# kngwyu/rogue-gym

Hardware: AMD Instinct MI355X
Metric: env-steps/sec (whole node) at 65 536 envs, 32x16 mini-dungeon (higher is better)
Workload: dtype u8/u16 integer state, f32 observation; 1 GPU; config-mini.json 32x16, 65536 envs per GPU (65536 total), gray-image obs [N,1,16,32] f32, max_steps 1000, auto-reset; envs_per_gpu=65536, parallelism=env-sharded x1, no data-path collective

## Files before the change

### include/rogue_gym_hip.h

```cpp
#ifndef ROGUE_GYM_HIP_H
#define ROGUE_GYM_HIP_H
#include <stddef.h>
#include <stdint.h>

#ifdef __cplusplus
extern "C" {
#endif

typedef struct rg_handle rg_t;

#define RG_FLAG_TERMINAL   0x00000001u
#define RG_FLAG_DEAD       0x00000002u
#define RG_FLAG_REDRAW     0x00000004u
#define RG_FLAG_HIST_STALE 0x00000008u
#define RG_FLAG_HIST_LAG   0x00000010u
#define RG_FLAG_HIST_DIRTY 0x00000020u
#define RG_FLAG_SCR_CHANGED 0x00000040u
#define RG_FLAG_MSG_SHIFT  8
#define RG_FLAG_MSG_MASK   0x00007f00u
#define RG_FLAG_ERR_KEY    0x00010000u
#define RG_FLAG_ERR_DEAD   0x00020000u
#define RG_FLAG_ERR_TILE   0x00040000u
#define RG_FLAG_ERR_INTERNAL 0x00080000u
#define RG_FLAG_ERR_STATE  0x00100000u
#define RG_FLAG_ERR_MASK   0x00ff0000u

int rg_create(const char *const *cfg_json, int n_env, uint64_t max_steps, int device, int auto_reset, rg_t **out);
void rg_destroy(rg_t *h);
const char *rg_last_error(const rg_t *h);

const char *rg_build_id(void);

int rg_dims(const rg_t *h, int *height, int *width, int *symbols, int *n_env);
int rg_env_dims(const rg_t *h, int32_t *heights, int32_t *widths);
int rg_env_symbols(const rg_t *h, int32_t *out_host);
int rg_set_stream(rg_t *h, void *hip_stream);

int rg_seed(rg_t *h, const uint64_t *seed_lo, const uint64_t *seed_hi, int n);
int rg_reset(rg_t *h);
int rg_reset_envs(rg_t *h, const int32_t *env_ids, int k, int ids_on_device);
int rg_reset_mask(rg_t *h, const uint8_t *mask_dev);
int rg_seed_envs(rg_t *h, const int32_t *env_ids, const uint64_t *seed_lo, const uint64_t *seed_hi, int k);
int rg_step(rg_t *h, const uint8_t *keys, int keys_on_device);
int rg_step_prefix(rg_t *h, const uint8_t *keys, int n_keys, int keys_on_device);
int rg_step_obs_gray(rg_t *h, const uint8_t *keys, int keys_on_device, uint32_t status_flag, int with_hist, float *out_dev);
int rg_obs_bind(rg_t *h, int kind, uint32_t status_flag, int with_hist, float *out_dev);
int rg_sync(rg_t *h);

int rg_screen(rg_t *h, uint8_t **dev);
int rg_hist(rg_t *h, uint8_t **dev);
int rg_status(rg_t *h, int32_t **dev);
int rg_flags(rg_t *h, uint32_t **dev);
int rg_reward(rg_t *h, float **dev);
int rg_done(rg_t *h, uint8_t **dev);

int rg_set_stair_reward(rg_t *h, float bonus);

int rg_obs_gray(rg_t *h, uint32_t status_flag, int with_hist, float *out_dev);
int rg_obs_symbol(rg_t *h, uint32_t status_flag, int with_hist, float *out_dev);
int rg_obs_channels(const rg_t *h, int symbol, uint32_t status_flag, int with_hist);

int rg_obs_crop(rg_t *h, int kind, int radius_y, int radius_x, uint32_t status_flag, int with_hist, float *out_dev, int32_t *centers_dev);

#define RG_OBS_F32  0
#define RG_OBS_F16  1
#define RG_OBS_BF16 2
#define RG_OBS_U8   3
int rg_obs_dtype_bytes(int dtype);
int rg_obs_typed(rg_t *h, int kind, int dtype, uint32_t status_flag, int with_hist, void *out_dev);
int rg_step_obs_typed(rg_t *h, const uint8_t *keys, int keys_on_device, int kind, int dtype, uint32_t status_flag, int with_hist, void *out_dev);

int rg_status_vec(rg_t *h, uint32_t status_flag, int32_t *out_host);

int rg_fetch_states(rg_t *h, uint8_t *screen, uint8_t *hist, int32_t *status, uint32_t *flags);
int rg_step_fetch(rg_t *h, const uint8_t *keys_host, int n_keys, uint8_t *screen, uint8_t *hist, int32_t *status, uint32_t *flags);

int rg_dev_alloc(int device, size_t bytes, void **out);
void rg_dev_free(int device, void *p);
int rg_snapshot_take(rg_t *h, void *dev);
int rg_dev_read(rg_t *h, const void *dev_src, void *host_dst, size_t bytes);
int rg_dev_read_rows(rg_t *h, const void *dev_src, size_t src_pitch, void *host_dst, size_t row_bytes, int rows);

int rg_encode_host(int device, const uint8_t *screen, const uint8_t *hist, const int32_t *status, int height, int width,
                   int symbols, uint32_t status_flag, int with_hist, int kind, float *out_host);

int rg_encode_host_batch(int device, int n, const uint8_t *screen, const uint8_t *hist, const int32_t *status, int height, int width,
                         int symbols, uint32_t status_flag, int with_hist, int kind, float *out_host);
int rg_obs_host(rg_t *h, int kind, uint32_t status_flag, int with_hist, float *out_host);
int rg_host_alloc(size_t bytes, void **out);
void rg_host_free(void *p);

#define RG_COMPACT_FIXED_BYTES 48
#define RG_COMPACT_STATUS_OFFSET(hw) (hw)
#define RG_COMPACT_REWARD_OFFSET(hw) ((hw) + 40)
#define RG_COMPACT_FLAGS_OFFSET(hw) ((hw) + 44)
#define RG_COMPACT_HIST_OFFSET(hw) ((hw) + RG_COMPACT_FIXED_BYTES)
int rg_compact_record_bytes(const rg_t *h, int with_hist);
int rg_pack_compact(rg_t *h, int with_hist, uint8_t *out_dev);
int rg_comm_unique_id(uint8_t id[128]);
int rg_comm_init(rg_t *h, const uint8_t id[128], int rank, int world);
int rg_comm_destroy(rg_t *h);
int rg_comm_count(rg_t *h, int *count, int *rank);
int rg_allgather_compact(rg_t *h, int with_hist, uint8_t *out_dev);
int rg_expand_compact(rg_t *h, const uint8_t *packed_dev, int n, int packed_has_hist, int kind, uint32_t status_flag, int with_hist, float *out_dev);

int rg_history_enable(rg_t *h, int cap_per_env);
int rg_history_keys(rg_t *h, int env, int which, uint8_t *keys, size_t cap, uint32_t *len);
int rg_dump_history(rg_t *h, int env, int which, char *buf, size_t cap, size_t *needed);

int rg_counters(rg_t *h, uint64_t out[8], int reset);
int rg_counters_ex(rg_t *h, uint64_t *out, int n_out, int reset);
int rg_probe_sclk(rg_t *h, double *mhz);

int rg_timing_enable(rg_t *h, int on);
int rg_timing_read(rg_t *h, double ms[4], uint64_t launches[4]);
int rg_timing_read_all(rg_t *h, int n, double *ms, uint64_t *sampled, uint64_t *launches);
int rg_timing_read_samples(rg_t *h, int kernel, float *ms, int cap, int *n);

int rg_dump_config(const rg_t *h, int env, char *buf, size_t cap);

int rg_config_canonical(const char *cfg_json, char *buf, size_t cap);

int rg_config_resolved(const char *cfg_json, char *buf, size_t cap);

int rg_config_schema(char *buf, size_t cap, size_t *needed);

int rg_state_record_bytes(const rg_t *h);
int rg_state_save(rg_t *h, const int32_t *env_ids, int k, int ids_on_device, uint8_t *out_dev);
int rg_state_load(rg_t *h, const uint8_t *rec_dev, size_t rec_bytes, const int32_t *env_ids, int k, int ids_on_device);

typedef struct rg_debug_state {
    int32_t px, py, dungeon_level, hp, hp_max, player_level, n_monsters, n_gold;
    uint32_t exp, food_left, quiet, pack_gold, steps;
    uint32_t rng[12];
    int32_t mon_x[384], mon_y[384], mon_type[384], mon_active[384], mon_hp[384];
    uint32_t mon_exp[384];
    int32_t gold_x[384], gold_y[384], gold_amount[384];
    int32_t n_rooms;
    uint32_t room_rect[384];
    int32_t room_meta[384];
} rg_debug_state;
int rg_debug_fetch(rg_t *h, int env, rg_debug_state *out, uint16_t *cells);
int rg_debug_descend(rg_t *h);

#ifdef __cplusplus
}
#endif
#endif
```

### rogue-gym_amd/csrc/rg_api.cpp

```cpp
#include <hip/hip_runtime.h>
#include <dlfcn.h>

#include <cstdio>
#include <cstdlib>
#include <cstring>
#include <mutex>
#include <random>
#include <string>
#include <vector>

#include "../../include/rogue_gym_hip.h"
#include "rg_state.h"
#include "rg_state_io.h"

extern "C" {
typedef struct ncclComm *ncclComm_t;
typedef struct { char internal[128]; } ncclUniqueId;
typedef int ncclResult_t;
typedef int ncclDataType_t;
}
static const ncclResult_t ncclSuccess = 0;
static const ncclDataType_t ncclUint8 = 1;

extern "C" {
void rgk_build(const RgState *S, const RgConfig *c, hipStream_t st);
int rgk_step(const RgState *S, const RgState *SP_dev, const RgConfig *c, const uint8_t *keys, int use_spares, int parity, hipStream_t st, hipEvent_t ev0, hipEvent_t ev1);
void rgk_probe_clock(unsigned long long *out, int spin, hipStream_t st);
void rgk_regen(const RgState *SP, const RgConfig *c, int bulk, int spares, const uint32_t *mark, uint32_t target, uint32_t *err_any, hipStream_t st, hipEvent_t ev0, hipEvent_t ev1);
void rgk_regen_gate(const uint32_t *mark, uint32_t target, uint32_t *err_any, hipStream_t st);
void rgk_export(const RgState *S, uint32_t *err_any, void *o_screen, void *o_hist, void *o_status, void *o_flags, uint32_t *o_err, hipStream_t st);
int rgk_regen_lanes_supported(const RgConfig *c, int maze_cap);
int rgk_step_bound_capable(const RgConfig *c);
int rgk_regen_lanes(const RgState *SP, const RgConfig *c, uint32_t *q, int32_t *list, int bulk, int waves, int slots, hipStream_t st, hipEvent_t ev0, hipEvent_t ev1);
void rgk_debug_descend(const RgState *S, const RgConfig *c, hipStream_t st);
void rgk_render(const RgState *S, const RgConfig *c, hipStream_t st);
void rgk_encode(const uint8_t *screen, const uint8_t *hist, const int32_t *status, uint32_t *flags, uint32_t *err_any, int n, int hw, size_t rs, size_t rst,
                int symbols, int planes_sym, uint32_t sflag, int with_hist, int kind, float *out, const int32_t *ext, hipStream_t st);
void rgk_pack(const RgState *S, int with_hist, uint8_t *out, hipStream_t st);
void rgk_scatter_rows(const void *src, void *dst, const int32_t *ext, int n, int row_bytes, hipStream_t st);
void rgk_gather_keys(const uint8_t *keys, const int32_t *ext, uint8_t *dst, int n, hipStream_t st);
int rgk_obs(const RgState *S, const RgConfig *c, uint32_t sflag, int with_hist, int kind, float *out, uint32_t *err_any, int planes_sym, int bound, hipStream_t st, hipEvent_t ev0, hipEvent_t ev1);
int rgk_redraw(const RgState *S, const RgConfig *c, hipStream_t st);
int rgk_obs_typed(const RgState *S, const RgConfig *c, int kind, int dtype, uint32_t sflag, int with_hist, int planes_sym, void *out, uint32_t *err_any, hipStream_t st, hipEvent_t ev0,
                  hipEvent_t ev1);
int rgk_obs_crop(const RgState *S, const RgConfig *c, int kind, int ry, int rx, uint32_t sflag, int with_hist, int planes_sym, float *out, int32_t *centers,
                 uint32_t *err_any, hipStream_t st);
void rgk_state_save(const RgState *S, const RgIoLayout *L, const uint64_t *desc, const uint32_t *guard, const int32_t *ids, int k, uint8_t *out, hipStream_t st);
void rgk_state_load(const RgState *S, const RgIoLayout *L, const uint64_t *desc, const uint32_t *guard, const int32_t *ids, int k, const uint8_t *recs, uint32_t rec_bytes, uint8_t *ok,
                    uint8_t *mark, hipStream_t st);
void rgk_state_stairs(const RgState *S, const RgIoLayout *L, uint8_t *mark, hipStream_t st);
void rgk_reset_compact(const uint8_t *mask, int n, int32_t *list, uint32_t *cnt, hipStream_t st);
void rgk_build_list(const RgState *S, const RgConfig *c, const int32_t *list, const uint32_t *cnt, uint8_t *mark, hipStream_t st);
}

#define RG_TIMED_KERNELS 5
struct rg_handle {
    RgParsed parsed;
    RgConfig cfg;
    RgState S;
    RgState SP;
    bool spares = false;
    uint32_t *lane_q = nullptr; int32_t *lane_list = nullptr;
    hipStream_t side3 = nullptr;
    hipStream_t side2 = nullptr;
    int lane_flip = 0;
    uint64_t lane_last = 0;
    uint8_t *pin_keys = nullptr;
    uint32_t *pin_err = nullptr;
    bool lane_regen = false;
    uint64_t step_count = 0;
    hipStream_t side = nullptr;
    int regen_idle_after = -1;
    int regen_bulk = 0;
    int device = 0;
    hipStream_t stream = nullptr;
    std::vector<void *> allocs;
    uint32_t *d_err = nullptr;
    uint8_t *d_keys = nullptr;
    bool render_pending = false;
    float *bound_out = nullptr; int bound_kind = 0; bool bound_valid = false;
    int32_t *obs_list_mem = nullptr; uint32_t *obs_cnt_mem = nullptr; float *gray_lut_mem = nullptr;
    int bound_steps = 0;
    int stair_gen = 0;
    float *obs_scratch = nullptr;
    size_t obs_scratch_cap = 0;
    std::vector<uint64_t> seed_lo, seed_hi;
    std::vector<uint8_t> reseed;
    std::vector<uint64_t> range_lo, range_span;
    unsigned long long *d_probe = nullptr;
    std::vector<rg_handle *> sub;
    std::vector<int> g_of, l_of;
    int32_t *d_ext = nullptr;
    std::vector<int32_t> ext;
    uint8_t *d_keys_sub = nullptr;
    int planes_sym = 0;
    bool screens_stale = true;
    bool mixed = false;
    std::vector<size_t> ragged_off;
    size_t stat_rows = 0;
    RgState *d_SP = nullptr;
    ncclComm_t comm = nullptr;
    int comm_rank = 0, comm_world = 1;
    std::string err;
    bool timing = false;
    std::vector<hipEvent_t> ev[RG_TIMED_KERNELS];
    size_t ev_used[RG_TIMED_KERNELS] = {0, 0, 0, 0, 0};
    uint64_t timing_seq[RG_TIMED_KERNELS] = {0, 0, 0, 0, 0};
    uint64_t timing_stride = 1;
    uint64_t state_fp = 0;
    uint64_t *io_desc = nullptr;
    uint32_t *io_guard = nullptr;
    uint32_t io_words = 0;
    int32_t *io_ids = nullptr; size_t io_ids_cap = 0;
    uint8_t *io_ok = nullptr; size_t io_ok_cap = 0;
    uint8_t *io_mark = nullptr;
    int32_t *reset_list = nullptr;
    uint32_t *reset_cnt = nullptr;
};

#define RG_TIMING_MAX 4096
struct TimedLaunch {
    rg_handle *h; int k; bool on, ext_;
    TimedLaunch(rg_handle *h_, int k_, bool ext = false) : h(h_), k(k_), on(false), ext_(ext) {
        if (h->timing && (h->timing_seq[k]++ % h->timing_stride) == h->timing_stride / 2 && h->ev_used[k] + 2 <= h->ev[k].size()) {
            on = true;
            if (!ext_) (void)hipEventRecord(h->ev[k][h->ev_used[k]], h->stream);
        }
    }
    hipEvent_t start_ev() const { return on && ext_ ? h->ev[k][h->ev_used[k]] : nullptr; }
    hipEvent_t stop_ev() const { return on && ext_ ? h->ev[k][h->ev_used[k] + 1] : nullptr; }
    void cancel() { on = false; }
    void stop() { if (on) { if (!ext_) (void)hipEventRecord(h->ev[k][h->ev_used[k] + 1], h->stream); h->ev_used[k] += 2; on = false; } }
    ~TimedLaunch() { stop(); }
};

static thread_local std::string g_create_err;

#ifdef RG_DEV_KNOBS
#define RG_DEV_ENV(name) getenv(name)
#else
#define RG_DEV_ENV(name) ((const char *)nullptr)
#endif

#define HIPCHK(h, call)                                                                                  \
    do {                                                                                                 \
        hipError_t e_ = (call);                                                                          \
        if (e_ != hipSuccess) {                                                                          \
            (h)->err = std::string(#call) + ": " + hipGetErrorString(e_);                                \
            return 1;                                                                                    \
        }                                                                                                \
    } while (0)

template <typename T>
static bool dev_alloc(rg_handle *h, T **p, size_t count) {
    void *q = nullptr;
    size_t bytes = count * sizeof(T);
    if (bytes == 0) bytes = 16;
    if (hipMalloc(&q, bytes) != hipSuccess) { h->err = "hipMalloc failed (" + std::to_string(bytes) + " bytes)"; return false; }
    if (hipMemset(q, 0, bytes) != hipSuccess) { h->err = "hipMemset failed"; return false; }
    h->allocs.push_back(q);
    *p = (T *)q;
    return true;
}

static void free_all(rg_handle *h) {
    for (void *p : h->allocs) (void)hipFree(p);
    h->allocs.clear();
}

static int flush_render(rg_handle *h) {
    if (h->render_pending) {
        { TimedLaunch t(h, 1); rgk_render(&h->S, &h->cfg, h->stream); }
        HIPCHK(h, hipGetLastError());
        h->render_pending = false;
        h->bound_valid = false;
    }
    return 0;
}

static int upload_seeds(rg_handle *h, size_t n) {
    HIPCHK(h, hipMemcpyAsync(h->S.seed_lo, h->seed_lo.data(), n * 8, hipMemcpyHostToDevice, h->stream));
    HIPCHK(h, hipMemcpyAsync(h->S.seed_hi, h->seed_hi.data(), n * 8, hipMemcpyHostToDevice, h->stream));
    HIPCHK(h, hipMemcpyAsync(h->S.reseed, h->reseed.data(), n, hipMemcpyHostToDevice, h->stream));
    return 0;
}

extern "C" {

const char *rg_last_error(const rg_t *h) { return h ? h->err.c_str() : g_create_err.c_str(); }

#ifndef RG_BUILD_ID
#define RG_BUILD_ID "unstamped"
#endif
const char *rg_build_id(void) { static const char id[] = "RGBUILDID:" RG_BUILD_ID; return id + 10; }

static void destroy_handle(rg_handle *h);
struct EnvSeed { bool has_seed, has_range; uint64_t lo, hi; unsigned __int128 r0, r1; };

static int create_homog(const RgParsed &parsed, const EnvSeed *seeds, int n_env, uint64_t max_steps, int device, int auto_reset, rg_handle **out) {
    *out = nullptr;
    rg_handle *h = new rg_handle();
    std::random_device rd;
    std::mt19937_64 gen(((uint64_t)rd() << 32) ^ rd());
    h->seed_lo.resize(n_env); h->seed_hi.resize(n_env); h->reseed.resize(n_env);
    h->parsed = parsed;
    for (int i = 0; i < n_env; i++) {
        const EnvSeed &p = seeds[i];
        if (p.has_seed) { h->seed_lo[i] = p.lo; h->seed_hi[i] = p.hi; h->reseed[i] = 0; }
        else { h->seed_lo[i] = gen(); h->seed_hi[i] = gen(); h->reseed[i] = 1; }
        if (p.has_range) {
            if (!(p.r1 > p.r0)) {
                if (!p.has_seed) { g_create_err = "Invalid Setting: seed_range must satisfy start < end"; delete h; return 1; }
                continue;
            }
            if (h->range_lo.empty()) { h->range_lo.assign(2 * (size_t)n_env, 0); h->range_span.assign(2 * (size_t)n_env, 0); }
            const unsigned __int128 span = p.r1 - p.r0;
            h->range_lo[i] = (uint64_t)p.r0; h->range_lo[n_env + i] = (uint64_t)(p.r0 >> 64);
            h->range_span[i] = (uint64_t)span; h->range_span[n_env + i] = (uint64_t)(span >> 64);
            if (!p.has_seed) h->reseed[i] = 2;
        }
    }
    h->cfg = h->parsed.cfg;
    {
        RgParsed q = h->parsed;
        q.has_seed_range = false;
        const std::string js = rg_dump_config_json(q, 0, 0, false);
        uint64_t f = 0xcbf29ce484222325ull;
        for (unsigned char ch : js) { f ^= ch; f *= 0x100000001b3ull; }
        h->state_fp = f;
    }
    h->planes_sym = h->cfg.symbols;
    h->cfg.max_steps = max_steps > 0xfffffff0ull ? 0xfffffff0u : (uint32_t)max_steps;
    h->cfg.auto_reset = auto_reset ? 1 : 0;
    h->device = device;
    int ndev = 0;
    if (hipGetDeviceCount(&ndev) != hipSuccess || ndev <= 0) {
        g_create_err = "no HIP device available (librogue_gym_hip has no CPU fallback)"; delete h; return 1;
    }
    if (device < 0 || device >= ndev || hipSetDevice(device) != hipSuccess) { g_create_err = "invalid HIP device " + std::to_string(device); delete h; return 1; }

    RgState &S = h->S;
    memset(&S, 0, sizeof S);
    const size_t n = (size_t)n_env, hw = (size_t)h->cfg.width * h->cfg.height;
    S.n = n_env; S.hw = (int)hw; S.n_keys = n_env;
    const int maze_cap = ((h->cfg.width / h->cfg.room_num_x + 1) / 2) * ((h->cfg.height / h->cfg.room_num_y + 1) / 2) + 1;
    S.maze_cap = maze_cap;
    const size_t nr = (size_t)h->cfg.room_num_x * h->cfg.room_num_y, ne = 2 * nr;
    h->stat_rows = 2048 + (n + 15) / 16;
    bool ok = dev_alloc(h, &S.cell, n * hw) && dev_alloc(h, &S.screen, n * hw) && dev_alloc(h, &S.hist, n * hw) &&
              dev_alloc(h, &S.p_pos, n) && dev_alloc(h, &S.p_hp, n) && dev_alloc(h, &S.p_hpmax, n) && dev_alloc(h, &S.p_lvl, n) &&
              dev_alloc(h, &S.p_exp, n) && dev_alloc(h, &S.food, n) && dev_alloc(h, &S.quiet, n) && dev_alloc(h, &S.pack_gold, n) &&
              dev_alloc(h, &S.dlevel, n) && dev_alloc(h, &S.steps, n) && dev_alloc(h, &S.flags, n) && dev_alloc(h, &S.reward, n) && dev_alloc(h, &S.done, n) &&
              dev_alloc(h, &S.rng, 12 * n) && dev_alloc(h, &S.seed_lo, n) && dev_alloc(h, &S.seed_hi, n) && dev_alloc(h, &S.reseed, n) &&
              dev_alloc(h, &S.room_rect, nr * n) && dev_alloc(h, &S.room_meta, nr * n) &&
              dev_alloc(h, &S.mon_w0, nr * n) && dev_alloc(h, &S.mon_hp, nr * n) && dev_alloc(h, &S.mon_exp, nr * n) &&
              dev_alloc(h, &S.mon_cnt, n) && dev_alloc(h, &S.gold_pos, nr * n) && dev_alloc(h, &S.gold_amt, nr * n) &&
              dev_alloc(h, &S.edge_a, ne * n) && dev_alloc(h, &S.edge_b, ne * n) &&
              dev_alloc(h, &S.maze_stack, (size_t)maze_cap * n) && dev_alloc(h, &S.build_ctr, n) && dev_alloc(h, &S.stats, RG_STAT_COLS * h->stat_rows) && dev_alloc(h, &S.stair_list, 2 * n) && dev_alloc(h, &S.stair_cnt, 8) && dev_alloc(h, &S.stair_mark, 2 * n) &&
              dev_alloc(h, &S.dc_map, h->cfg.n_enemies > 0 ? n * RG_DIST_SLOTS * hw : 16) && dev_alloc(h, &S.dc_key, RG_DIST_SLOTS * n) &&
              dev_alloc(h, &S.dc_head, n) && dev_alloc(h, &S.dc_len, n) && dev_alloc(h, &S.dc_part, n) && dev_alloc(h, &S.dc_own, n) && dev_alloc(h, &S.status, n * 10) &&
              dev_alloc(h, &h->d_err, 4) && dev_alloc(h, &h->d_keys, n);
    if (ok && nr <= RG_OBS_MAX_ROOMS) ok = dev_alloc(h, &S.obs_rec, n * (size_t)RG_OBS_REC_WORDS(nr));
    if (ok && nr <= RG_OVL_MAX && getenv("ROGUE_GYM_HIP_NO_MIRROR_UPDATE") == nullptr)
        ok = dev_alloc(h, &S.ovl, (nr + 1) * n) && hipMemset(S.ovl, 0xff, (nr + 1) * n * 2) == hipSuccess;
    h->spares = auto_reset != 0 && getenv("ROGUE_GYM_HIP_NO_SPARES") == nullptr;
    h->lane_regen = h->spares && getenv("ROGUE_GYM_HIP_WAVE_REGEN") == nullptr && rgk_regen_lanes_supported(&h->cfg, maze_cap) > 0;
    const char *slots_env = getenv("ROGUE_GYM_HIP_SP_SLOTS");
    S.sp_slots = h->lane_regen ? (slots_env ? atoi(slots_env) : 4) : 1;
    if (S.sp_slots < 1 || S.sp_slots > 8) S.sp_slots = 4;
    const size_t ns = n * (size_t)S.sp_slots;
    ok = ok && dev_alloc(h, &S.sp_ready, ns) && dev_alloc(h, &h->d_probe, 4) && dev_alloc(h, &S.launch_mark, 4);
    if (ok && h->cfg.n_enemies > 0 && RG_PARTIAL_MAPS(h->cfg.width, h->cfg.height, (int)nr))
        ok = dev_alloc(h, &S.dc_walk, n * RG_DIST_SLOTS * h->cfg.height * RG_WALK_WORDS(h->cfg.width));
    S.full_bfs = getenv("ROGUE_GYM_HIP_FULL_BFS") != nullptr;
    S.keep_spares = getenv("ROGUE_GYM_HIP_KEEP_SPARES") != nullptr;
    S.err_any = h->d_err;
    if (ok && !h->range_lo.empty()) {
        ok = dev_alloc(h, &S.range_lo, 2 * n) && dev_alloc(h, &S.range_span, 2 * n) &&
             hipMemcpy(S.range_lo, h->range_lo.data(), 2 * n * 8, hipMemcpyHostToDevice) == hipSuccess &&
             hipMemcpy(S.range_span, h->range_span.data(), 2 * n * 8, hipMemcpyHostToDevice) == hipSuccess;
        if (!ok && h->err.empty()) h->err = "hipMemcpy failed";
    }
    if (ok && !h->parsed.init_draws.empty()) {
        uint32_t *d = nullptr;
        ok = dev_alloc(h, &d, h->parsed.init_draws.size()) &&
             hipMemcpy(d, h->parsed.init_draws.data(), h->parsed.init_draws.size() * 4, hipMemcpyHostToDevice) == hipSuccess;
        if (!ok && h->err.empty()) h->err = "hipMemcpy failed";
        S.init_draws = d;
    }
    if (ok && h->spares && nr <= 64 && getenv("ROGUE_GYM_HIP_NO_NEXT_LEVELS") == nullptr) {
        RgNext nx;
        memset(&nx, 0, sizeof nx);
        RgNext *d_nx = nullptr;
        ok = dev_alloc(h, &nx.cell, n * hw) && dev_alloc(h, &nx.room_rect, nr * n) && dev_alloc(h, &nx.room_meta, nr * n) &&
             dev_alloc(h, &nx.gold_pos, nr * n) && dev_alloc(h, &nx.gold_amt, nr * n) && dev_alloc(h, &nx.level, n) &&
             dev_alloc(h, &S.nx_rng, 12 * n) && dev_alloc(h, &S.nx_state, n) && dev_alloc(h, &d_nx, 1);
        ok = ok && hipMemcpy(d_nx, &nx, sizeof nx, hipMemcpyHostToDevice) == hipSuccess;
        S.nx = d_nx;
    }
    h->SP = S;
    if (ok && h->spares) {
        RgState &P = h->SP;
        ok = dev_alloc(h, &P.cell, ns * hw) && dev_alloc(h, &P.p_pos, ns) && dev_alloc(h, &P.p_hp, ns) && dev_alloc(h, &P.p_hpmax, ns) && dev_alloc(h, &P.p_lvl, ns) &&
             dev_alloc(h, &P.p_exp, ns) && dev_alloc(h, &P.food, ns) && dev_alloc(h, &P.quiet, ns) && dev_alloc(h, &P.pack_gold, ns) && dev_alloc(h, &P.dlevel, ns) &&
             dev_alloc(h, &P.rng, 12 * ns) && dev_alloc(h, &P.room_rect, nr * ns) && dev_alloc(h, &P.room_meta, nr * ns) &&
             dev_alloc(h, &P.mon_w0, nr * ns) && dev_alloc(h, &P.mon_hp, nr * ns) && dev_alloc(h, &P.mon_exp, nr * ns) &&
             dev_alloc(h, &P.mon_cnt, ns) && dev_alloc(h, &P.gold_pos, nr * ns) && dev_alloc(h, &P.gold_amt, nr * ns) &&
             dev_alloc(h, &P.edge_a, ne * n) && dev_alloc(h, &P.edge_b, ne * n) && dev_alloc(h, &P.maze_stack, (size_t)maze_cap * n) &&
             dev_alloc(h, &P.on_stairs, ns);
        P.prof = nullptr;
        int lo = 0, hi = 0;
        if (ok && (hipDeviceGetStreamPriorityRange(&lo, &hi) != hipSuccess || hipStreamCreateWithPriority(&h->side, hipStreamNonBlocking, RG_DEV_ENV("ROGUE_GYM_HIP_SIDE_HIPRIO") ? hi : lo) != hipSuccess)) {
            h->err = "failed to create the background generation stream"; ok = false;
        }
        static const bool lanes_low = RG_DEV_ENV("ROGUE_GYM_HIP_LANES_LOWPRIO") != nullptr;
        if (ok && (hipStreamCreateWithPriority(&h->side2, hipStreamNonBlocking, lanes_low ? lo : (lo + hi) / 2) != hipSuccess || hipStreamCreateWithPriority(&h->side3, hipStreamNonBlocking, lanes_low ? lo : (lo + hi) / 2) != hipSuccess)) { h->err = "failed to create the background generation stream"; ok = false; }
    }
    ok = ok && dev_alloc(h, &h->d_SP, 1) && hipMemcpy(h->d_SP, &h->SP, sizeof(RgState), hipMemcpyHostToDevice) == hipSuccess;
    if (!ok) { g_create_err = h->err.empty() ? "device allocation failed" : h->err; destroy_handle(h); return 1; }
    if (hipMemset(S.screen, ' ', n * hw) != hipSuccess) { g_create_err = "hipMemset failed"; destroy_handle(h); return 1; }
    if (upload_seeds(h, n)) { g_create_err = h->err; destroy_handle(h); return 1; }
    h->S.stair_gen = h->stair_gen++;
    rgk_build(&h->S, &h->cfg, h->stream);
    hipError_t e = hipGetLastError();
    if (e == hipSuccess) e = hipStreamSynchronize(h->stream);
    if (e != hipSuccess) { g_create_err = std::string("k_build: ") + hipGetErrorString(e); destroy_handle(h); return 1; }
    h->render_pending = true;
    if (h->spares) {
        if (h->lane_regen && !(dev_alloc(h, &h->lane_q, 8) && dev_alloc(h, &h->lane_list, 2 * ns))) { g_create_err = h->err; destroy_handle(h); return 1; }
        if (h->lane_regen) (void)rgk_regen_lanes(&h->SP, &h->cfg, h->lane_q, h->lane_list, 1, 0, h->S.sp_slots, h->side2, nullptr, nullptr);
        else rgk_regen(&h->SP, &h->cfg, 1, 1, nullptr, 0, h->d_err, h->side, nullptr, nullptr);
        e = hipGetLastError();
        if (e == hipSuccess && !RG_DEV_ENV("ROGUE_GYM_HIP_ASYNC_FIRST_SPARES")) { e = hipStreamSynchronize(h->side); if (e == hipSuccess) e = hipStreamSynchronize(h->side2); if (e == hipSuccess) e = hipStreamSynchronize(h->side3); }
        if (e != hipSuccess) { g_create_err = std::string("k_regen: ") + hipGetErrorString(e); destroy_handle(h); return 1; }
        h->regen_bulk = 1;
        bool all_fixed = true;
        for (uint8_t m : h->reseed) all_fixed = all_fixed && m == 0;
        if (h->S.keep_spares && all_fixed && !h->S.nx_state) h->regen_idle_after = 1;
    }
    *out = h;
    return 0;
}

#define SUBCHK(h, sh, call) do { if (call) { (h)->err = (sh)->err; return 1; } } while (0)

static void destroy_handle(rg_handle *h);
static int comm_release(rg_handle *h, bool teardown);

static int assemble_small(rg_handle *h) {
    for (rg_handle *sh : h->sub) {
        const int m = sh->S.n;
        rgk_scatter_rows(sh->S.status, h->S.status, sh->d_ext, m, 40, h->stream);
        rgk_scatter_rows(sh->S.reward, h->S.reward, sh->d_ext, m, 4, h->stream);
        rgk_scatter_rows(sh->S.done, h->S.done, sh->d_ext, m, 1, h->stream);
        rgk_scatter_rows(sh->S.flags, h->S.flags, sh->d_ext, m, 4, h->stream);
    }
    HIPCHK(h, hipGetLastError());
    return 0;
}
static int assemble_screens(rg_handle *h) {
    if (!h->screens_stale) return 0;
    for (rg_handle *sh : h->sub) {
        SUBCHK(h, sh, flush_render(sh));
        const int m = sh->S.n;
        if (!h->mixed) {
            rgk_scatter_rows(sh->S.screen, h->S.screen, sh->d_ext, m, h->S.hw, h->stream);
            rgk_scatter_rows(sh->S.hist, h->S.hist, sh->d_ext, m, h->S.hw, h->stream);
        }
        rgk_scatter_rows(sh->S.flags, h->S.flags, sh->d_ext, m, 4, h->stream);
    }
    HIPCHK(h, hipGetLastError());
    h->screens_stale = false;
    return 0;
}

int rg_create(const char *const *cfg_json, int n_env, uint64_t max_steps, int device, int auto_reset, rg_t **out) {
    if (!out || n_env <= 0) { g_create_err = "rg_create: invalid arguments"; return 1; }
    *out = nullptr;
    std::vector<RgParsed> reps;
    std::vector<EnvSeed> seeds(n_env);
    std::vector<int> g_of(n_env), l_of(n_env);
    std::vector<std::vector<int>> members;
    {
        const char *prev = nullptr; int prev_g = -1;
        RgParsed p;
        for (int i = 0; i < n_env; i++) {
            const char *js = cfg_json ? cfg_json[i] : nullptr;
            const bool same_text = i > 0 && ((js == nullptr && prev == nullptr) || (js && prev && strcmp(js, prev) == 0));
            int g = prev_g;
            if (!same_text) {
                std::string e = rg_parse_config(js, &p);
                if (!e.empty()) { g_create_err = "Failed to parse config: " + e; return 1; }
                g = -1;
                for (size_t k = 0; k < reps.size(); k++) if (rg_config_equal(reps[k], p)) { g = (int)k; break; }
                if (g < 0) { g = (int)reps.size(); reps.push_back(p); members.emplace_back(); }
                prev = js; prev_g = g;
            }
            seeds[i] = EnvSeed{p.has_seed, p.has_seed_range, p.seed_lo, p.seed_hi, p.seed_range[0], p.seed_range[1]};
            g_of[i] = g; l_of[i] = (int)members[g].size(); members[g].push_back(i);
        }
    }
    if (reps.size() == 1) return create_homog(reps[0], seeds.data(), n_env, max_steps, device, auto_reset, out);
    bool mixed = false;
    for (size_t k = 1; k < reps.size(); k++) mixed = mixed || reps[k].cfg.width != reps[0].cfg.width || reps[k].cfg.height != reps[0].cfg.height;
    rg_handle *h = new rg_handle();
    h->device = device;
    h->mixed = mixed;
    h->g_of = g_of; h->l_of = l_of;
    for (size_t k = 0; k < reps.size(); k++) {
        std::vector<EnvSeed> gs(members[k].size());
        for (size_t j = 0; j < members[k].size(); j++) gs[j] = seeds[members[k][j]];
        rg_handle *sh = nullptr;
        if (create_homog(reps[k], gs.data(), (int)gs.size(), max_steps, device, auto_reset, &sh)) { destroy_handle(h); return 1; }
        h->sub.push_back(sh);
        sh->ext.assign(members[k].begin(), members[k].end());
        bool ok = dev_alloc(sh, &sh->d_ext, gs.size()) && dev_alloc(sh, &sh->d_keys_sub, gs.size()) &&
                  hipMemcpy(sh->d_ext, sh->ext.data(), gs.size() * 4, hipMemcpyHostToDevice) == hipSuccess;
        if (!ok) { g_create_err = "device allocation failed"; destroy_handle(h); return 1; }
        sh->S.ext = sh->d_ext;
    }
    if (mixed) {
        h->ragged_off.assign((size_t)n_env + 1, 0);
        for (int i = 0; i < n_env; i++) h->ragged_off[i + 1] = h->ragged_off[i] + (size_t)reps[g_of[i]].cfg.width * reps[g_of[i]].cfg.height;
    }
    rg_handle *first = h->sub[g_of[0]];
    h->parsed = first->parsed; h->cfg = first->cfg;
    h->planes_sym = first->cfg.symbols;
    for (rg_handle *sh : h->sub) sh->planes_sym = h->planes_sym;
    RgState &S = h->S;
    memset(&S, 0, sizeof S);
    const size_t n = (size_t)n_env, hw = (size_t)h->cfg.width * h->cfg.height;
    S.n = n_env; S.hw = (int)hw; S.n_keys = n_env;
    bool ok = (mixed || (dev_alloc(h, &S.screen, n * hw) && dev_alloc(h, &S.hist, n * hw))) && dev_alloc(h, &S.status, n * 10) && dev_alloc(h, &S.flags, n) &&
              dev_alloc(h, &S.reward, n) && dev_alloc(h, &S.done, n) && dev_alloc(h, &h->d_err, 4) && dev_alloc(h, &h->d_probe, 4);
    if (!ok) { g_create_err = h->err; destroy_handle(h); return 1; }
    S.err_any = h->d_err;
    if (assemble_small(h) || hipStreamSynchronize(h->stream) != hipSuccess) { g_create_err = h->err.empty() ? "assemble failed" : h->err; destroy_handle(h); return 1; }
    *out = h;
    return 0;
}

static void destroy_handle(rg_handle *h) {
    if (!h) return;
    (void)hipSetDevice(h->device);
    for (rg_handle *sh : h->sub) destroy_handle(sh);
    h->sub.clear();
    (void)hipStreamSynchronize(h->stream);
    if (h->comm) (void)comm_release(h, true);
    if (h->side) { (void)hipStreamSynchronize(h->side); (void)hipStreamDestroy(h->side); }
    if (h->side2) { (void)hipStreamSynchronize(h->side2); (void)hipStreamDestroy(h->side2); }
    if (h->side3) { (void)hipStreamSynchronize(h->side3); (void)hipStreamDestroy(h->side3); }
    for (int k = 0; k < RG_TIMED_KERNELS; k++) for (auto &e : h->ev[k]) (void)hipEventDestroy(e);
    if (h->obs_scratch) (void)hipFree(h->obs_scratch);
    if (h->pin_keys) (void)hipHostFree(h->pin_keys);
    if (h->pin_err) (void)hipHostFree(h->pin_err);
    free_all(h);
    delete h;
}

void rg_destroy(rg_t *h) { destroy_handle(h); }

int rg_dims(const rg_t *h, int *height, int *width, int *symbols, int *n_env) {
    if (height) *height = h->cfg.height;
    if (width) *width = h->cfg.width;
    if (symbols) *symbols = h->planes_sym;
    if (n_env) *n_env = h->S.n;
    return 0;
}

int rg_env_dims(const rg_t *h, int32_t *heights, int32_t *widths) {
    for (int i = 0; i < h->S.n; i++) {
        const RgConfig &c = h->sub.empty() ? h->cfg : h->sub[h->g_of[i]]->cfg;
        if (heights) heights[i] = c.height;
        if (widths) widths[i] = c.width;
    }
    return 0;
}
static bool refuse_mixed(rg_handle *h, const char *what) {
    if (!h->mixed) return false;
    h->err = std::string(what) + ": the envs of this batch differ in width / height, so there is no [n_env][H][W] tensor (per-env sizes: rg_env_dims; "
             "ragged host copies: rg_fetch_states; or one handle per size)";
    return true;
}

int rg_env_symbols(const rg_t *h, int32_t *out_host) {
    if (h->sub.empty()) { for (int i = 0; i < h->S.n; i++) out_host[i] = h->cfg.symbols; return 0; }
    for (int i = 0; i < h->S.n; i++) out_host[i] = h->sub[h->g_of[i]]->cfg.symbols;
    return 0;
}

int rg_set_stream(rg_t *h, void *hip_stream) {
    for (rg_handle *sh : h->sub) SUBCHK(h, sh, rg_set_stream(sh, hip_stream));
    HIPCHK(h, hipStreamSynchronize(h->stream));
    if (h->side) { HIPCHK(h, hipStreamSynchronize(h->side)); HIPCHK(h, hipStreamSynchronize(h->side2)); HIPCHK(h, hipStreamSynchronize(h->side3)); }
    h->stream = (hipStream_t)hip_stream;
    return 0;
}

int rg_seed(rg_t *h, const uint64_t *seed_lo, const uint64_t *seed_hi, int n) {
    if (n > h->S.n) n = h->S.n;
    if (n <= 0) return 0;
    HIPCHK(h, hipSetDevice(h->device));
    if (!h->sub.empty()) {
        for (rg_handle *sh : h->sub) {
            std::vector<uint64_t> lo, hi;
            for (int l = 0; l < sh->S.n && sh->ext[l] < n; l++) { lo.push_back(seed_lo[sh->ext[l]]); hi.push_back(seed_hi ? seed_hi[sh->ext[l]] : 0); }
            if (!lo.empty()) SUBCHK(h, sh, rg_seed(sh, lo.data(), hi.data(), (int)lo.size()));
        }
        return 0;
    }
    for (int i = 0; i < n; i++) { h->seed_lo[i] = seed_lo[i]; h->seed_hi[i] = seed_hi ? seed_hi[i] : 0; h->reseed[i] = 0; }
    if (h->spares) {
        HIPCHK(h, hipStreamSynchronize(h->side));
        HIPCHK(h, hipStreamSynchronize(h->side2));
        HIPCHK(h, hipStreamSynchronize(h->side3));
        for (int sl = 0; sl < h->S.sp_slots; sl++) HIPCHK(h, hipMemsetAsync(h->S.sp_ready + (size_t)sl * h->S.n, 0, (size_t)n * 4, h->stream));
        if (h->regen_idle_after >= 0) h->regen_idle_after = 2;
        h->regen_bulk = 2;
    }
    return upload_seeds(h, (size_t)n);
}

int rg_reset(rg_t *h) {
    HIPCHK(h, hipSetDevice(h->device));
    if (!h->sub.empty()) {
        for (rg_handle *sh : h->sub) SUBCHK(h, sh, rg_reset(sh));
        h->screens_stale = true;
        return assemble_small(h);
    }
    h->S.stair_gen = h->stair_gen++;
    { TimedLaunch t(h, 3); rgk_build(&h->S, &h->cfg, h->stream); }
    HIPCHK(h, hipGetLastError());
    h->render_pending = true;
    h->bound_valid = false;
    return 0;
}

static int obs_common(rg_t *h, uint32_t status_flag, int with_hist, int kind, float *out_dev);
int rg_step(rg_t *h, const uint8_t *keys, int keys_on_device) { return rg_step_prefix(h, keys, h->S.n, keys_on_device); }
int rg_step_obs_gray(rg_t *h, const uint8_t *keys, int keys_on_device, uint32_t status_flag, int with_hist, float *out_dev) {
    return rg_step_prefix(h, keys, h->S.n, keys_on_device) ? 1 : obs_common(h, status_flag, with_hist, 0, out_dev);
}

int rg_step_prefix(rg_t *h, const uint8_t *keys, int n_keys, int keys_on_device) {
    HIPCHK(h, hipSetDevice(h->device));
    if (n_keys < 0) { h->err = "rg_step_prefix: negative key count"; return 1; }
    if (n_keys > h->S.n) n_keys = h->S.n;
    if (!h->sub.empty()) {
        const uint8_t *dkeys = keys;
        if (!keys_on_device) {
            if (!h->d_keys && !dev_alloc(h, &h->d_keys, (size_t)h->S.n)) return 1;
            HIPCHK(h, hipMemcpyAsync(h->d_keys, keys, (size_t)n_keys, hipMemcpyHostToDevice, h->stream));
            dkeys = h->d_keys;
        }
        for (rg_handle *sh : h->sub) {
            int m = 0;
            while (m < sh->S.n && sh->ext[m] < n_keys) m++;
            if (m) rgk_gather_keys(dkeys, sh->d_ext, sh->d_keys_sub, m, h->stream);
            SUBCHK(h, sh, rg_step_prefix(sh, sh->d_keys_sub, m, 1));
        }
        HIPCHK(h, hipGetLastError());
        h->screens_stale = true;
        return assemble_small(h);
    }
    if (flush_render(h)) return 1;
    const uint8_t *dk = keys;
    if (!keys_on_device) {
        HIPCHK(h, hipMemcpyAsync(h->d_keys, keys, (size_t)n_keys, hipMemcpyHostToDevice, h->stream));
        dk = h->d_keys;
    }
    h->S.n_keys = n_keys;
    static const int regen_every = RG_DEV_ENV("ROGUE_GYM_HIP_REGEN_EVERY") ? atoi(RG_DEV_ENV("ROGUE_GYM_HIP_REGEN_EVERY")) : 1;
    h->step_count++;
    bool regen = h->spares && (regen_every <= 1 || h->step_count % (uint64_t)regen_every == 0);
    if (regen && h->regen_idle_after >= 0) { if (h->regen_idle_after == 0) regen = false; else h->regen_idle_after--; }
    static const bool no_stair_waves = getenv("ROGUE_GYM_HIP_NO_STAIR_WAVES") != nullptr;
    {
        TimedLaunch t(h, 0, true);
        h->S.stair_gen = h->stair_gen++;
        h->S.obs_par = (int32_t)(h->step_count & 1); h->bound_steps++;
        (void)rgk_step(&h->S, h->d_SP, &h->cfg, dk, h->spares ? 1 : 0, no_stair_waves ? -1 : 0, h->stream, t.start_ev(), t.stop_ev());
    }
    HIPCHK(h, hipGetLastError());
    if (regen) {
        TimedLaunch t(h, 4, true);
        if (h->lane_regen) {
            static const int lane_waves = RG_DEV_ENV("ROGUE_GYM_HIP_LANE_WAVES") ? atoi(RG_DEV_ENV("ROGUE_GYM_HIP_LANE_WAVES")) : 256;
            static const int lane_every = RG_DEV_ENV("ROGUE_GYM_HIP_LANE_EVERY") ? atoi(RG_DEV_ENV("ROGUE_GYM_HIP_LANE_EVERY")) : 16;
            static const bool time_lanes = RG_DEV_ENV("ROGUE_GYM_HIP_TIME_LANES") != nullptr;
            const bool lanes_now = h->regen_bulk > 0 || h->step_count - h->lane_last >= (uint64_t)(lane_every > 0 ? lane_every : 1);
            static const int urgent_mode = RG_DEV_ENV("ROGUE_GYM_HIP_URGENT_AT0") ? 3 : 2;
            rgk_regen(&h->SP, &h->cfg, 0, urgent_mode, h->S.launch_mark, (uint32_t)h->S.stair_gen + 1u, h->d_err, h->side, time_lanes ? nullptr : t.start_ev(), time_lanes ? nullptr : t.stop_ev());
            if (time_lanes && !lanes_now) t.cancel();
            if (lanes_now) {
                h->lane_last = h->step_count;
                h->lane_flip ^= 1;
                rgk_regen_gate(h->S.launch_mark, (uint32_t)h->S.stair_gen + 1u, h->d_err, h->lane_flip ? h->side3 : h->side2);
                (void)rgk_regen_lanes(&h->SP, &h->cfg, h->lane_q + 4 * h->lane_flip, h->lane_list + (size_t)h->S.n * h->S.sp_slots * h->lane_flip, h->regen_bulk > 0 ? 1 : 0, lane_waves, h->S.sp_slots,
                                      h->lane_flip ? h->side3 : h->side2, time_lanes ? t.start_ev() : nullptr, time_lanes ? t.stop_ev() : nullptr);
            }
        } else rgk_regen(&h->SP, &h->cfg, h->regen_bulk > 0 ? 1 : 0, 1, h->S.launch_mark, (uint32_t)h->S.stair_gen + 1u, h->d_err, h->side, t.start_ev(), t.stop_ev());
        if (h->regen_bulk > 0) h->regen_bulk--;
    }
    HIPCHK(h, hipGetLastError());
    h->render_pending = true;
    return 0;
}

int rg_sync(rg_t *h) {
    HIPCHK(h, hipSetDevice(h->device));
    if (!h->sub.empty()) {
        int rc = 0;
        for (rg_handle *sh : h->sub)
            if (rg_sync(sh) && !rc) { rc = 1; h->err = sh->err; }
        if (rc) return rc;
    }
    uint32_t err = 0;
    HIPCHK(h, hipMemcpyAsync(&err, h->d_err, 4, hipMemcpyDeviceToHost, h->stream));
    HIPCHK(h, hipStreamSynchronize(h->stream));
    if (h->side) { HIPCHK(h, hipStreamSynchronize(h->side)); HIPCHK(h, hipStreamSynchronize(h->side2)); HIPCHK(h, hipStreamSynchronize(h->side3)); }
    if (err) {
        HIPCHK(h, hipMemsetAsync(h->d_err, 0, 4, h->stream));
        if (err & RG_FLAG_ERR_INTERNAL) h->err = "internal capacity guard of the HIP stepper tripped (please report the config), or rg_reset_envs was given a device-side env id out of range";
        else if (err & RG_FLAG_ERR_STATE) h->err = "state record refused: it does not fit this env (magic / version / config fingerprint / geometry), the env is unchanged";
        else if (err & RG_FLAG_ERR_KEY) h->err = "Invalid input (key is not in the ai keymap)";
        else if (err & RG_FLAG_ERR_DEAD) h->err = "Ignored input (action while the player is dead)";
        else h->err = "Invalid tile in symbol image (symbol >= symbols - 1)";
        return 1;
    }
    return 0;
}

static int flush_mirrors(rg_handle *h) { return h->sub.empty() ? flush_render(h) : assemble_screens(h); }
int rg_screen(rg_t *h, uint8_t **dev) { if (refuse_mixed(h, "rg_screen")) return 1; HIPCHK(h, hipSetDevice(h->device)); if (flush_mirrors(h)) return 1; *dev = h->S.screen; return 0; }
int rg_hist(rg_t *h, uint8_t **dev) { if (refuse_mixed(h, "rg_hist")) return 1; HIPCHK(h, hipSetDevice(h->device)); if (flush_mirrors(h)) return 1; *dev = h->S.hist; return 0; }
int rg_status(rg_t *h, int32_t **dev) { *dev = h->S.status; return 0; }
int rg_flags(rg_t *h, uint32_t **dev) { HIPCHK(h, hipSetDevice(h->device)); if (flush_mirrors(h)) return 1; *dev = h->S.flags; return 0; }
int rg_reward(rg_t *h, float **dev) { *dev = h->S.reward; return 0; }
int rg_done(rg_t *h, uint8_t **dev) { *dev = h->S.done; return 0; }
int rg_set_stair_reward(rg_t *h, float bonus) {
    if (!(bonus == bonus) || bonus < 0.f) { h->err = "rg_set_stair_reward: the bonus must be a number >= 0"; return 1; }
    h->S.stair_reward = bonus;
    for (rg_handle *sh : h->sub) sh->S.stair_reward = bonus;
    return 0;
}

int rg_obs_channels(const rg_t *h, int symbol, uint32_t status_flag, int with_hist) {
    return (symbol ? h->planes_sym : 1) + __builtin_popcount(status_flag & 0x1ffu) + (with_hist ? 1 : 0);
}

static int obs_common(rg_t *h, uint32_t status_flag, int with_hist, int kind, float *out_dev) {
    if (refuse_mixed(h, kind ? "rg_obs_symbol" : "rg_obs_gray")) return 1;
    HIPCHK(h, hipSetDevice(h->device));
    if (!h->sub.empty()) {
        for (rg_handle *sh : h->sub) {
            if (kind && sh->cfg.symbols > h->planes_sym) {
                h->err = "symbol image: a config of the batch has more symbols (" + std::to_string(sh->cfg.symbols) + ") than env 0's (" + std::to_string(h->planes_sym) +
                         "), which sets the channel count (python/src/lib.rs:281-285)";
                return 1;
            }
            SUBCHK(h, sh, obs_common(sh, status_flag, with_hist, kind, out_dev));
        }
        return 0;
    }
    {
        TimedLaunch t(h, 2, true);
        const bool bound = h->bound_out && out_dev == h->bound_out && kind == h->bound_kind && (status_flag & 0x1ffu) == 0 && !with_hist;
        if (rgk_obs(&h->S, &h->cfg, status_flag & 0x1ffu, with_hist ? 1 : 0, kind, out_dev, h->d_err, h->planes_sym, bound && h->S.obs_list && h->bound_valid && h->bound_steps == 1, h->stream, t.start_ev(), t.stop_ev())) {
            HIPCHK(h, hipGetLastError());
            h->render_pending = false;
            h->bound_valid = bound;
            h->bound_steps = 0;
            return 0;
        }
        t.cancel();
    }
    h->bound_valid = false;
    if (flush_render(h)) return 1;
    {
        TimedLaunch t(h, 2);
        rgk_encode(h->S.screen, h->S.hist, h->S.status, h->S.flags, h->d_err, h->S.n, h->S.hw, (size_t)h->S.hw, 10, h->cfg.symbols, h->planes_sym,
                   status_flag & 0x1ffu, with_hist ? 1 : 0, kind, out_dev, h->S.ext, h->stream);
    }
    HIPCHK(h, hipGetLastError());
    return 0;
}
static uint32_t host_tile_to_sym(uint32_t t) {
    switch (t) {
    case ' ': return 0; case '@': return 1; case '#': return 2; case '.': return 3; case '-': case '|': return 4;
    case '%': return 5; case '+': return 6; case '^': return 7; case '!': return 8; case '?': return 9; case ']': return 10;
    case ')': return 11; case '/': return 12; case '*': return 13; case ':': return 14; case '=': return 15; case ',': return 16;
    default: return (t >= 'A' && t <= 'Z') ? t - 'A' + 17 : 255u;
    }
}
int rg_obs_bind(rg_t *h, int kind, uint32_t status_flag, int with_hist, float *out_dev) {
    if (!h->sub.empty()) { h->err = "rg_obs_bind: not for a handle with config groups"; return 1; }
    if (out_dev && ((status_flag & 0x1ffu) || with_hist || (kind != 0 && kind != 1))) { h->err = "rg_obs_bind: gray or symbol image without status planes and history plane"; return 1; }
    HIPCHK(h, hipSetDevice(h->device));
    const bool capable = rgk_step_bound_capable(&h->cfg) != 0;
    if (!capable) { h->S.obs_list = nullptr; h->S.obs_cnt = nullptr; h->S.bound_gray = nullptr; h->bound_out = out_dev; h->bound_kind = kind; h->bound_valid = false; h->bound_steps = 0; return 0; }
    if (out_dev && !h->obs_list_mem) {
        if (!dev_alloc(h, &h->obs_list_mem, 2 * (size_t)h->S.n) || !dev_alloc(h, &h->obs_cnt_mem, 2)) return 1;
    }
    if (out_dev) HIPCHK(h, hipMemsetAsync(h->obs_cnt_mem, 0, 8, h->stream));
    h->S.obs_list = out_dev ? h->obs_list_mem : nullptr; h->S.obs_cnt = out_dev ? h->obs_cnt_mem : nullptr;
    h->S.bound_gray = (out_dev && kind == 0) ? out_dev : nullptr;
    if (h->S.bound_gray && !h->gray_lut_mem) {
        float lut[128];
        for (uint32_t g = 0; g < 128; g++) lut[g] = (float)(uint8_t)host_tile_to_sym(g) / (float)(uint8_t)h->cfg.symbols;
        if (!dev_alloc(h, &h->gray_lut_mem, 128)) return 1;
        HIPCHK(h, hipMemcpy(h->gray_lut_mem, lut, sizeof lut, hipMemcpyHostToDevice));
    }
    h->S.gray_lut = h->gray_lut_mem;
    h->bound_out = out_dev; h->bound_kind = kind; h->bound_valid = false; h->bound_steps = 0;
    return 0;
}
int rg_obs_crop(rg_t *h, int kind, int radius_y, int radius_x, uint32_t status_flag, int with_hist, float *out_dev, int32_t *centers_dev) {
    if (kind != 0 && kind != 1) { h->err = "rg_obs_crop: kind must be 0 (gray) or 1 (symbol), got " + std::to_string(kind); return 1; }
    if (radius_y < 0 || radius_y > RG_MAX_H - 1 || radius_x < 0 || radius_x > RG_MAX_W - 1) {
        h->err = "rg_obs_crop: radii must satisfy 0 <= radius_y <= " + std::to_string(RG_MAX_H - 1) + " and 0 <= radius_x <= " + std::to_string(RG_MAX_W - 1) +
                 ", got (" + std::to_string(radius_y) + ", " + std::to_string(radius_x) + ")";
        return 1;
    }
    if (!out_dev || ((uintptr_t)out_dev & 15)) { h->err = "rg_obs_crop: out_dev must be a non-null, 16-byte aligned device pointer"; return 1; }
    HIPCHK(h, hipSetDevice(h->device));
    if (!h->sub.empty()) {
        for (rg_handle *sh : h->sub)
            if (kind && sh->cfg.symbols > h->planes_sym) {
                h->err = "symbol image: a config of the batch has more symbols (" + std::to_string(sh->cfg.symbols) + ") than env 0's (" + std::to_string(h->planes_sym) +
                         "), which sets the channel count (python/src/lib.rs:281-285)";
                return 1;
            }
        for (rg_handle *sh : h->sub) SUBCHK(h, sh, rg_obs_crop(sh, kind, radius_y, radius_x, status_flag, with_hist, out_dev, centers_dev));
        return 0;
    }
    if (flush_render(h)) return 1;
    if (!rgk_obs_crop(&h->S, &h->cfg, kind, radius_y, radius_x, status_flag & 0x1ffu, with_hist ? 1 : 0, h->planes_sym, out_dev, centers_dev, h->d_err, h->stream)) {
        h->err = "rg_obs_crop: window too large";
        return 1;
    }
    HIPCHK(h, hipGetLastError());
    return 0;
}
int rg_obs_dtype_bytes(int dtype) { return dtype == RG_OBS_F32 ? 4 : (dtype == RG_OBS_F16 || dtype == RG_OBS_BF16) ? 2 : dtype == RG_OBS_U8 ? 1 : -1; }
static int typed_check(rg_t *h, const char *what, int kind, int dtype, uint32_t status_flag, const void *out_dev) {
    const std::string w = std::string(what) + ": ";
    if (kind < 0 || kind > 2) { h->err = w + "kind must be 0 (gray), 1 (symbol) or 2 (symbol ids), got " + std::to_string(kind); return 1; }
    if (rg_obs_dtype_bytes(dtype) < 0) { h->err = w + "dtype must be RG_OBS_F32 (0), RG_OBS_F16 (1), RG_OBS_BF16 (2) or RG_OBS_U8 (3), got " + std::to_string(dtype); return 1; }
    if (kind == 2 && dtype != RG_OBS_U8) { h->err = w + "kind 2 (symbol ids) takes dtype RG_OBS_U8 only, got dtype " + std::to_string(dtype); return 1; }
    if (kind != 2 && dtype == RG_OBS_U8) { h->err = w + "dtype RG_OBS_U8 is for kind 2 (symbol ids) only, got kind " + std::to_string(kind); return 1; }
    if (kind == 2 && (status_flag & 0x1ffu)) { h->err = w + "status_flag must be 0 for kind 2 (status values do not fit a byte; read the status mirror)"; return 1; }
    if (!out_dev || ((uintptr_t)out_dev & 15)) { h->err = w + "out_dev must be a non-null, 16-byte aligned device pointer"; return 1; }
    if (dtype == RG_OBS_F32) return 0;
    if (!h->sub.empty() || h->mixed) { h->err = w + "not for a handle with config groups or mixed sizes"; return 1; }
    const int cells = dtype == RG_OBS_U8 ? 16 : 8;
    if (h->S.hw % cells) {
        h->err = w + "H*W must be a multiple of " + std::to_string(cells) + " for this dtype (a lane writes whole 16-byte pieces of a plane), got " + std::to_string(h->cfg.height) +
                 " x " + std::to_string(h->cfg.width);
        return 1;
    }
    return 0;
}
static int obs_typed_checked(rg_t *h, int kind, int dtype, uint32_t status_flag, int with_hist, void *out_dev) {
    if (dtype == RG_OBS_F32) return obs_common(h, status_flag, with_hist, kind, static_cast<float *>(out_dev));
    HIPCHK(h, hipSetDevice(h->device));
    if (h->render_pending) {
        bool swept;
        { TimedLaunch t(h, 1); swept = rgk_redraw(&h->S, &h->cfg, h->stream) != 0; if (!swept) t.cancel(); }
        if (swept) {
            HIPCHK(h, hipGetLastError());
            h->render_pending = false;
            h->bound_valid = false;
        } else if (flush_render(h)) return 1;
    }
    {
        TimedLaunch t(h, 2, true);
        if (!rgk_obs_typed(&h->S, &h->cfg, kind, dtype, status_flag & 0x1ffu, with_hist ? 1 : 0, h->planes_sym, out_dev, h->d_err, h->stream, t.start_ev(), t.stop_ev())) {
            t.cancel();
            h->err = "rg_obs_typed: grid not supported";
            return 1;
        }
    }
    HIPCHK(h, hipGetLastError());
    return 0;
}
int rg_obs_typed(rg_t *h, int kind, int dtype, uint32_t status_flag, int with_hist, void *out_dev) {
    return typed_check(h, "rg_obs_typed", kind, dtype, status_flag, out_dev) ? 1 : obs_typed_checked(h, kind, dtype, status_flag, with_hist, out_dev);
}
int rg_step_obs_typed(rg_t *h, const uint8_t *keys, int keys_on_device, int kind, int dtype, uint32_t status_flag, int with_hist, void *out_dev) {
    if (typed_check(h, "rg_step_obs_typed", kind, dtype, status_flag, out_dev)) return 1;
    return rg_step_prefix(h, keys, h->S.n, keys_on_device) ? 1 : obs_typed_checked(h, kind, dtype, status_flag, with_hist, out_dev);
}
int rg_obs_gray(rg_t *h, uint32_t status_flag, int with_hist, float *out_dev) { return obs_common(h, status_flag, with_hist, 0, out_dev); }
int rg_obs_symbol(rg_t *h, uint32_t status_flag, int with_hist, float *out_dev) { return obs_common(h, status_flag, with_hist, 1, out_dev); }

int rg_fetch_states(rg_t *h, uint8_t *screen, uint8_t *hist, int32_t *status, uint32_t *flags) {
    HIPCHK(h, hipSetDevice(h->device));
    if (flush_mirrors(h)) return 1;
    size_t n = (size_t)h->S.n, hw = (size_t)h->S.hw;
    if (h->mixed) {
        std::vector<uint8_t> tmp;
        for (rg_handle *sh : h->sub) {
            const size_t m = (size_t)sh->S.n, ghw = (size_t)sh->S.hw;
            for (int which = 0; which < 2; which++) {
                uint8_t *dst = which ? hist : screen;
                if (!dst) continue;
                tmp.resize(m * ghw);
                HIPCHK(h, hipMemcpyAsync(tmp.data(), which ? sh->S.hist : sh->S.screen, m * ghw, hipMemcpyDeviceToHost, h->stream));
                HIPCHK(h, hipStreamSynchronize(h->stream));
                for (size_t l = 0; l < m; l++) memcpy(dst + h->ragged_off[sh->ext[l]], tmp.data() + l * ghw, ghw);
            }
        }
        screen = hist = nullptr;
    }
    if (screen) HIPCHK(h, hipMemcpyAsync(screen, h->S.screen, n * hw, hipMemcpyDeviceToHost, h->stream));
    if (hist) HIPCHK(h, hipMemcpyAsync(hist, h->S.hist, n * hw, hipMemcpyDeviceToHost, h->stream));
    if (status) HIPCHK(h, hipMemcpyAsync(status, h->S.status, n * 40, hipMemcpyDeviceToHost, h->stream));
    if (flags) HIPCHK(h, hipMemcpyAsync(flags, h->S.flags, n * 4, hipMemcpyDeviceToHost, h->stream));
    HIPCHK(h, hipStreamSynchronize(h->stream));
    return 0;
}

int rg_step_fetch(rg_t *h, const uint8_t *keys_host, int n_keys, uint8_t *screen, uint8_t *hist, int32_t *status, uint32_t *flags) {
    if (refuse_mixed(h, "rg_step_fetch")) return 1;
    if (!h->sub.empty()) { h->err = "rg_step_fetch: not for a handle with config groups (rg_step_prefix + rg_fetch_states)"; return 1; }
    if (!status || !flags || (screen == nullptr) != (hist == nullptr)) { h->err = "rg_step_fetch: status and flags are required, screen and hist come together"; return 1; }
    if (h->S.hw & 3) { h->err = "rg_step_fetch needs H*W divisible by 4"; return 1; }
    HIPCHK(h, hipSetDevice(h->device));
    if (n_keys < 0) { h->err = "rg_step_fetch: negative key count"; return 1; }
    if (n_keys > h->S.n) n_keys = h->S.n;
    if (!h->pin_keys) HIPCHK(h, hipHostMalloc((void **)&h->pin_keys, (size_t)h->S.n + 16, hipHostMallocDefault));
    if (!h->pin_err) HIPCHK(h, hipHostMalloc((void **)&h->pin_err, 16, hipHostMallocDefault));
    memcpy(h->pin_keys, keys_host, (size_t)n_keys);
    if (rg_step_prefix(h, h->pin_keys, n_keys, 1)) return 1;
    if (flush_render(h)) return 1;
    rgk_export(&h->S, h->d_err, screen, hist, status, flags, h->pin_err, h->stream);
    HIPCHK(h, hipGetLastError());
    HIPCHK(h, hipStreamSynchronize(h->stream));
    const uint32_t err = h->pin_err[0];
    if (err) {
        if (err & RG_FLAG_ERR_INTERNAL) h->err = "internal capacity guard of the HIP stepper tripped (please report the config), or rg_reset_envs was given a device-side env id out of range";
        else if (err & RG_FLAG_ERR_STATE) h->err = "state record refused: it does not fit this env (magic / version / config fingerprint / geometry), the env is unchanged";
        else if (err & RG_FLAG_ERR_KEY) h->err = "Invalid input (key is not in the ai keymap)";
        else if (err & RG_FLAG_ERR_DEAD) h->err = "Ignored input (action while the player is dead)";
        else h->err = "Invalid tile in symbol image (symbol >= symbols - 1)";
        return 1;
    }
    return 0;
}

int rg_dev_alloc(int device, size_t bytes, void **out) {
    if (hipSetDevice(device) != hipSuccess || hipMalloc(out, bytes ? bytes : 16) != hipSuccess) { g_create_err = "hipMalloc failed (" + std::to_string(bytes) + " bytes)"; return 1; }
    return 0;
}
void rg_dev_free(int device, void *p) { if (p && hipSetDevice(device) == hipSuccess) (void)hipFree(p); }
int rg_snapshot_take(rg_t *h, void *dev) {
    if (refuse_mixed(h, "rg_snapshot_take")) return 1;
    HIPCHK(h, hipSetDevice(h->device));
    if (flush_mirrors(h)) return 1;
    const size_t bytes = (size_t)h->S.n * (size_t)h->S.hw;
    HIPCHK(h, hipMemcpyAsync(dev, h->S.screen, bytes, hipMemcpyDeviceToDevice, h->stream));
    HIPCHK(h, hipMemcpyAsync(static_cast<uint8_t *>(dev) + bytes, h->S.hist, bytes, hipMemcpyDeviceToDevice, h->stream));
    return 0;
}
int rg_dev_read_rows(rg_t *h, const void *dev_src, size_t src_pitch, void *host_dst, size_t row_bytes, int rows) {
    HIPCHK(h, hipSetDevice(h->device));
// ... 746 lines not shown
```

### rogue-gym_amd/csrc/rg_kernels.hip

```cpp


#include "rg_device.h"


#include "rg_gen.h"


#ifdef RG_FINE_PROF
#define PFM(id) pf.mark(id)
#else
#define PFM(id) ((void)0)
#endif
struct Prof {
    unsigned long long *p; unsigned long long t, t0, r0; int k;
    __device__ __forceinline__ void start(unsigned long long *pp) { p = pp ? pp + (size_t)blockIdx.x * 64 : nullptr; k = 0; if (p) { r0 = __builtin_amdgcn_s_memrealtime(); t = t0 = __builtin_amdgcn_s_memtime(); } }
    __device__ __forceinline__ void rec(int phase, unsigned long long v) {
        if (p && threadIdx.x == 0 && k < 61) p[1 + k++] = ((unsigned long long)phase << 48) | (v & 0xffffffffffffull);
    }
    __device__ __forceinline__ void mark(int phase) {
        if (!p) return;
        unsigned long long now = __builtin_amdgcn_s_memtime();
        rec(phase, now - t);
        t = now;
    }
// ... 2073 lines not shown
    const __attribute__((address_space(3))) uint8_t *mt = (const __attribute__((address_space(3))) uint8_t *)(ovl_l - ln + (RG_OVL_MAX + 6) * WAVE);
    uint32_t actp = 0;
    bool far = false;
#pragma nounroll
    for (int s0 = 0; s0 < nrooms; s0++) {
        const uint32_t p = ovl_l[(1 + s0) * WAVE], m = mc[s0 * WAVE];
        const bool alive = (m >> 24) & MF_ALIVE, had = p != OVL_NONE;
        const uint32_t pp = p & 0xff3fu, pn = m & 0xffffu;
        bool show = false;
        if (alive) {
            const int x = POS_X(pn), y = POS_Y(pn), dx = px - x, dy = py - y;
            show = dx * dx + dy * dy <= 2;
            if (!show && rid >= 0 && room_id_of(c, x, y) == rid) {
                if ((r_meta & RM_KIND_MASK) == RK_EMPTY) show = true;
                else {
                    int x0, y0, x1, y1;
                    unpack_rect(r_rect, x0, y0, x1, y1);
                    const bool ina = px >= x0 && px < x1 && py >= y0 && py < y1, inb = x >= x0 && x < x1 && y >= y0 && y < y1;
                    show = ina == inb;
                }
            }
        }
        const bool unknown = had && (p & OVL_UNKNOWN), showed = had && (p & OVL_SHOW);
        const bool same = had && alive && pp == pn && !unknown && !dirty_at(POS_X(pn), POS_Y(pn));
        uint32_t a = 0;
        if (same) { if (showed && !show) a = 1u; else if (!showed && show) a = 2u; }
        else { if (had && (showed || unknown)) a |= 1u; if (show) a |= 2u; }
        a |= show ? 4u : 0u;
        actp |= a << (3 * s0);
        if (((a & 1u) && !in_win(POS_X(pp), POS_Y(pp))) || ((a & 2u) && !in_win(POS_X(pn), POS_Y(pn)))) far = true;
        const uint32_t now = alive ? (pn | (show ? OVL_SHOW : 0u)) : OVL_NONE;
        if (now != p) S.ovl[(size_t)s0 * n + e] = (uint16_t)now;
    }
    const uint32_t pl = ovl_l[(1 + nrooms) * WAVE];
    const uint32_t plp = pl & 0xff3fu;
    const bool pl_moved = pl == OVL_NONE || (pl & OVL_UNKNOWN) || plp != POS(px, py) || dirty_at(px, py);
    if (pl_moved) S.ovl[(size_t)nrooms * n + e] = (uint16_t)POS(px, py);
    if (far || (pl_moved && pl != OVL_NONE && !in_win(POS_X(plp), POS_Y(plp)))) return false;
    for (uint32_t d = ds; d;) {
        const int k = __ffs((int)d) - 1;
        d &= d - 1;
        const int j = k / 5, i = k - j * 5, x = w.ox + i - 2, y = w.oy + j - 2;
        put(y * W + x, base_glyph(c, WV(w, k), y) & 0x7fu);
    }
    if (react & R_HIST_CHANGED) S.hist[(size_t)e * S.hw + py * W + px] = 1;
    if (pl_moved && pl != OVL_NONE) {
        const int x = POS_X(plp), y = POS_Y(plp);
        put(y * W + x, base_glyph(c, WV(w, WIN_K(x - w.ox, y - w.oy)), y) & 0x7fu);
    }
#pragma nounroll
    for (int s0 = 0; s0 < nrooms; s0++)
        if ((actp >> (3 * s0)) & 1u) {
            const uint32_t pp = ovl_l[(1 + s0) * WAVE] & 0xff3fu;
            const int x = POS_X(pp), y = POS_Y(pp);
            put(y * W + x, base_glyph(c, WV(w, WIN_K(x - w.ox, y - w.oy)), y) & 0x7fu);
        }
#pragma nounroll
    for (int s0 = 0; s0 < nrooms; s0++)
        if ((actp >> (3 * s0)) & 2u) {
            const uint32_t m = mc[s0 * WAVE];
            const int x = POS_X(m), y = POS_Y(m);
            const uint32_t under = base_glyph(c, WV(w, WIN_K(x - w.ox, y - w.oy)), y);
            if ((under & 0x80u) && under != (0x80u | '*')) put(y * W + x, mt[(m >> 16) & 0xff]);
        }
    if (pl_moved && (base_glyph(c, WV(w, WIN_K(px - w.ox, py - w.oy)), py) & 0x80u)) put(py * W + px, '@');
    return true;
}

__device__ __forceinline__ void take_spares(const RgState &S, const RgState *__restrict__ SPd, const RgConfig &c, int lane, int e, bool taken, bool &on_stairs) {
    const uint64_t tm = __ballot(taken);
    if (!tm) return;
    const RgState &SP = *SPd;
    const int HW = S.hw, n = S.n, nrooms = c.room_num_x * c.room_num_y;
    const size_t ns = (size_t)n * S.sp_slots;
    int es = e;
    if (taken)
        for (int sl = S.sp_slots - 1; sl >= 0; sl--)
            if (__hip_atomic_load(&S.sp_ready[(size_t)sl * n + e], __ATOMIC_RELAXED, __HIP_MEMORY_SCOPE_AGENT) == 1u) es = sl * n + e;
    __builtin_amdgcn_fence(__ATOMIC_ACQUIRE, "agent");
    if ((HW & 7) == 0) {
        const int q = HW / 8;
        uint64_t mm = tm;
        while (mm) {
            const int s0 = __ffsll((long long)mm) - 1; mm &= mm - 1;
            const int s1 = mm ? __ffsll((long long)mm) - 1 : -1; if (mm) mm &= mm - 1;
            const int s2 = mm ? __ffsll((long long)mm) - 1 : -1; if (mm) mm &= mm - 1;
            const int s3 = mm ? __ffsll((long long)mm) - 1 : -1; if (mm) mm &= mm - 1;
            const int e0 = __shfl(e, s0), e1 = __shfl(e, s1 >= 0 ? s1 : s0), e2 = __shfl(e, s2 >= 0 ? s2 : s0), e3 = __shfl(e, s3 >= 0 ? s3 : s0);
            const int q0 = __shfl(es, s0), q1 = __shfl(es, s1 >= 0 ? s1 : s0), q2 = __shfl(es, s2 >= 0 ? s2 : s0), q3 = __shfl(es, s3 >= 0 ? s3 : s0);
            const uint4 *a0 = reinterpret_cast<const uint4 *>(SP.cell + (size_t)q0 * HW), *a1 = reinterpret_cast<const uint4 *>(SP.cell + (size_t)q1 * HW);
            const uint4 *a2 = reinterpret_cast<const uint4 *>(SP.cell + (size_t)q2 * HW), *a3 = reinterpret_cast<const uint4 *>(SP.cell + (size_t)q3 * HW);
            uint4 *d0 = reinterpret_cast<uint4 *>(S.cell + (size_t)e0 * HW), *d1 = reinterpret_cast<uint4 *>(S.cell + (size_t)e1 * HW);
            uint4 *d2 = reinterpret_cast<uint4 *>(S.cell + (size_t)e2 * HW), *d3 = reinterpret_cast<uint4 *>(S.cell + (size_t)e3 * HW);
            for (int i = lane; i < q; i += WAVE) {
                const uint4 v0 = a0[i];
                uint4 v1 = v0, v2 = v0, v3 = v0;
                if (s1 >= 0) v1 = a1[i];
                if (s2 >= 0) v2 = a2[i];
                if (s3 >= 0) v3 = a3[i];
                d0[i] = v0;
                if (s1 >= 0) d1[i] = v1;
                if (s2 >= 0) d2[i] = v2;
                if (s3 >= 0) d3[i] = v3;
            }
        }
    } else {
        uint64_t mm = tm;
        while (mm) {
            const int src = __ffsll((long long)mm) - 1; mm &= mm - 1;
            const int env_s = __shfl(e, src);
            const uint16_t *sp = SP.cell + (size_t)__shfl(es, src) * HW;
            uint16_t *dp = S.cell + (size_t)env_s * HW;
            for (int i = lane; i < HW; i += WAVE) dp[i] = sp[i];
        }
    }
    if (taken) {
        uint32_t r[12];
#pragma unroll
        for (int k = 0; k < 12; k++) r[k] = SP.rng[k * ns + es];
        const uint16_t pp = SP.p_pos[es];
        const int32_t hp = SP.p_hp[es], hpm = SP.p_hpmax[es], lv = SP.p_lvl[es];
        const uint32_t ex = SP.p_exp[es], fd = SP.food[es], qu = SP.quiet[es], pg = SP.pack_gold[es], dl = SP.dlevel[es], mc = SP.mon_cnt[es];
        on_stairs = SP.on_stairs[es] != 0;
#pragma unroll
        for (int k = 0; k < 12; k++) S.rng[k * n + e] = r[k];
        S.p_pos[e] = pp; S.p_hp[e] = hp; S.p_hpmax[e] = hpm; S.p_lvl[e] = lv;
        if (S.obs_rec) S.obs_rec[(size_t)e * RG_OBS_REC_WORDS(nrooms) + nrooms] = pp;
        if (S.ovl) S.ovl[(size_t)nrooms * n + e] = (uint16_t)(pp | 0x40u);
        S.p_exp[e] = ex; S.food[e] = fd; S.quiet[e] = qu; S.pack_gold[e] = pg; S.dlevel[e] = dl; S.mon_cnt[e] = mc;
        for (int s0 = 0; s0 < nrooms; s0 += 4) {
            uint32_t rr[4], mw[4], me[4], gp[4], ga[4]; int32_t mh[4]; uint8_t rm[4];
#pragma unroll
            for (int k = 0; k < 4; k++) {
                const size_t g = (size_t)(s0 + k < nrooms ? s0 + k : s0) * ns + es;
                rr[k] = SP.room_rect[g]; rm[k] = SP.room_meta[g]; mw[k] = SP.mon_w0[g]; mh[k] = SP.mon_hp[g]; me[k] = SP.mon_exp[g]; gp[k] = SP.gold_pos[g]; ga[k] = SP.gold_amt[g];
            }
#pragma unroll
            for (int k = 0; k < 4; k++)
                if (s0 + k < nrooms) {
                    const size_t g = (size_t)(s0 + k) * n + e;
                    S.room_rect[g] = rr[k]; S.room_meta[g] = rm[k]; S.mon_w0[g] = mw[k]; S.mon_hp[g] = mh[k]; S.mon_exp[g] = me[k]; S.gold_pos[g] = gp[k]; S.gold_amt[g] = ga[k];
                    if (S.obs_rec) {
                        uint32_t *rec = S.obs_rec + (size_t)e * RG_OBS_REC_WORDS(nrooms);
                        rec[s0 + k] = mw[k]; rec[nrooms + 1 + s0 + k] = rr[k]; reinterpret_cast<uint8_t *>(&rec[2 * nrooms + 1])[s0 + k] = rm[k];
                    }
                    if (S.ovl) S.ovl[(size_t)(s0 + k) * n + e] = (uint16_t)(((mw[k] >> 24) & MF_ALIVE) ? ((mw[k] & 0xffffu) | 0x40u) : 0xffffu);
                }
        }
    }
    __syncthreads();
    if (taken && !(S.keep_spares && S.reseed[e] == 0)) __hip_atomic_store(&S.sp_ready[es], 0u, __ATOMIC_RELAXED, __HIP_MEMORY_SCOPE_AGENT);
}

template <int BW, int GM, bool BND = false>
__device__ __forceinline__ void step_wave(const RgState &S, const RgState *__restrict__ SPd, const RgConfig &c, const uint8_t *__restrict__ keys, int use_spares, int stage_off,
                                          const int e, const bool valid_in, const int stair_role) {
    uint16_t *lds_grid = reinterpret_cast<uint16_t *>(g_smem + stage_off);
    const int lane = threadIdx.x;
    Prof pf; pf.start(S.prof);
    Env E;
    E.err = 0; E.on_stairs = 0;
    uint32_t react = 0, err = 0, old_flags = 0, steps = 0, flags = 0;
    int act = ACT_NOOP, dir = 0;
    int gold0 = 0;
    bool live = false;
    bool ui_dead = false, terminal = false;
    bool inc_done = false;
    bool taken = false;
    uint32_t n_bfs = 0, n_inline = 0, n_taken = 0, n_cont = 0;
    uint32_t key = 0, nxs = RG_NX_NONE;
    bool listed = false;
    const int nrooms_k = c.room_num_x * c.room_num_y;
    E.mc = (lds_u32 *)(g_smem + STEP_LDS_MC) + lane;
    const uint32_t glyph_r = S.ovl ? c.mon[lane & 31].tile : 0u;
    if (valid_in) {
        listed = S.stair_mark[(size_t)(S.stair_gen & 1) * S.n + e] != 0;
        uint32_t nxk = 0;
        if (S.nx_state) {
            nxs = __hip_atomic_load(&S.nx_state[e], __ATOMIC_RELAXED, __HIP_MEMORY_SCOPE_AGENT);
            nxk = __hip_atomic_load(&S.nx_rng[(size_t)3 * S.n + e], __ATOMIC_RELAXED, __HIP_MEMORY_SCOPE_AGENT);
        }
        old_flags = S.flags[e];
        steps = S.steps[e];
        gold0 = S.status[(size_t)e * 10 + 1];
        if (e < S.n_keys) key = keys[e];
        load_env(S, E, e);
        if (nxs == RG_NX_READY && nxk != E.rd.w) nxs = RG_NX_STALE;
        for (int s0 = 0; s0 < nrooms_k; s0 += 4) {
            uint32_t m4[4];
#pragma unroll
            for (int k = 0; k < 4; k++) m4[k] = S.mon_w0[(size_t)(s0 + k < nrooms_k ? s0 + k : s0) * S.n + e];
#pragma unroll
            for (int k = 0; k < 4; k++)
                if (s0 + k < nrooms_k) E.mc[(s0 + k) * WAVE] = m4[k];
        }
    }
    const bool to_stair_wave = listed && key == '>';
    const bool valid = valid_in && (stair_role == 0 || (stair_role == 1) == to_stair_wave);
    const bool has_key = valid && e < S.n_keys;
    if (valid) {
        if (has_key && !(steps > c.max_steps)) {
            act = decode_key(key, dir);
            if (act == ACT_INVALID) err = RG_FLAG_ERR_KEY;
            else {
                klog_push(S, e, key);
                if (old_flags & RG_FLAG_DEAD) err = RG_FLAG_ERR_DEAD;
                else live = true;
            }
        }
    }
    pf.mark(0);
    bool need_gen = false, descends = false;
    Win w;
    w.v = (lds_u16 *)(g_smem + STEP_LDS_WIN) + lane;
    lds_u32 *ovl_l = (lds_u32 *)(g_smem + STEP_LDS_OVL) + lane;
    ovl_l[0] = 0;
    if (BND && S.bound_gray) {
        typedef const __attribute__((address_space(1))) void *gptr;
        typedef __attribute__((address_space(3))) void *lptr;
        __builtin_amdgcn_global_load_lds((gptr)(S.gray_lut + lane), (lptr)(g_smem + STEP_LDS_LUT), 4, 0, 0);
        __builtin_amdgcn_global_load_lds((gptr)(S.gray_lut + 64 + lane), (lptr)(g_smem + STEP_LDS_LUT + 256), 4, 0, 0);
    }
    if (S.ovl && lane < RG_MAX_ENEMY_KINDS + 6)
        ((__attribute__((address_space(3))) uint8_t *)(g_smem + STEP_LDS_OVL + (RG_OVL_MAX + 6) * WAVE * 4))[lane] = (uint8_t)glyph_r;
    if (S.ovl) {
        typedef const __attribute__((address_space(1))) void *gptr;
        typedef __attribute__((address_space(3))) void *lptr;
        lds_u32 *base = (lds_u32 *)(g_smem + STEP_LDS_OVL);
        const size_t es = valid_in ? (size_t)e : 0;
#pragma unroll
        for (int s0 = 0; s0 <= RG_OVL_MAX; s0++)
            __builtin_amdgcn_global_load_lds((gptr)(S.ovl + (size_t)(s0 <= nrooms_k ? s0 : 0) * S.n + es), (lptr)(base + (1 + s0) * WAVE), 2, 0, 0);
    }
    w.inb = 0;
    if (S.ovl) {
        typedef const __attribute__((address_space(1))) void *gptr;
        typedef __attribute__((address_space(3))) void *lptr;
        lds_u32 *base = (lds_u32 *)(g_smem + STEP_LDS_OVL);
        const size_t es = valid_in ? (size_t)e : 0;
        const bool mv = live && (act == ACT_MOVE || act == ACT_MOVE_UNTIL);
        const int ra = room_id_of(c, E.px, E.py), rb = mv ? room_id_of(c, E.px + dir_dx(dir), E.py + dir_dy(dir)) : ra;
        const size_t aa = (size_t)(ra >= 0 ? ra : 0) * S.n + es, ab = (size_t)(rb >= 0 ? rb : 0) * S.n + es;
        __builtin_amdgcn_global_load_lds((gptr)(S.room_rect + aa), (lptr)(base + (RG_OVL_MAX + 2) * WAVE), 4, 0, 0);
        __builtin_amdgcn_global_load_lds((gptr)(S.room_meta + aa), (lptr)(base + (RG_OVL_MAX + 3) * WAVE), 1, 0, 0);
        __builtin_amdgcn_global_load_lds((gptr)(S.room_rect + ab), (lptr)(base + (RG_OVL_MAX + 4) * WAVE), 4, 0, 0);
        __builtin_amdgcn_global_load_lds((gptr)(S.room_meta + ab), (lptr)(base + (RG_OVL_MAX + 5) * WAVE), 1, 0, 0);
    }
    if (live && stair_role != 1) win_load(c, E.cell, w, E.px, E.py);
    else { w.inb = 0; w.dirty = 0; w.ox = w.oy = 0; }
    pf.mark(26);
    if (live && act == ACT_DOWNSTAIR) {
        if (stair_role == 1 || (WV(w, WIN_K(0, 0)) & C_SURF_MASK) == S_STAIR) {
            need_gen = descends = true;
            react |= R_REDRAW | R_STATUS | R_HIST_STALE;
        } else react |= MSG_NO_DOWNSTAIR;
    }
    if (S.nx_state) {
        if (descends && nxs == RG_NX_READY) {
            const uint32_t *q = S.nx_rng + e;
            const size_t n = (size_t)S.n;
            const uint32_t k0 = q[0], k1 = q[n], k2 = q[2 * n], kl = S.nx->level[e];
            if (k0 == E.rd.x && k1 == E.rd.y && k2 == E.rd.z && kl == E.dlevel) nxs = RG_NX_HIT;
        }
        if (__any(nxs == RG_NX_HIT)) __builtin_amdgcn_fence(__ATOMIC_ACQUIRE, "agent");
    }
    {
        uint64_t lag = __ballot(descends && ((old_flags & RG_FLAG_HIST_LAG) || ((old_flags & RG_FLAG_REDRAW) && (old_flags & RG_FLAG_HIST_STALE))));
        while (lag) {
            const int src = __ffsll((long long)lag) - 1;
            lag &= lag - 1;
            const int env_s = __shfl(e, src);
            const uint16_t *cp = S.cell + (size_t)env_s * S.hw;
            uint8_t *hp = S.hist + (size_t)env_s * S.hw;
            for (int i = lane; i < S.hw; i += WAVE) hp[i] = (cp[i] & C_VISITED) ? 1 : 0;
        }
    }
#pragma nounroll
    for (int pass = 0; pass < 2; ++pass) {
        pf.mark(1);
        if (pass == 1 && use_spares) {
            if (need_gen) {
                bool rdy = false;
                for (int sl = 0; sl < S.sp_slots; sl++) rdy = rdy || __hip_atomic_load(&S.sp_ready[(size_t)sl * S.n + e], __ATOMIC_RELAXED, __HIP_MEMORY_SCOPE_AGENT) == 1u;
                if (rdy) { taken = true; need_gen = false; n_taken++; }
            }
        }
        const bool regenerated = descends && pass == 0;
        if constexpr (BW == 1 || BW == 2) { if (pass == 0 && S.dc_walk) snapshot_walk_service(S, c, lane, e, descends); }
        const uint64_t nx_now = pass == 0 ? __ballot(need_gen && nxs == RG_NX_HIT) : 0ull;
        if (need_gen) n_inline++;
        gen_service<GM>(S, c, E, lane, e, need_gen, pass == 1, lds_grid, pf, nx_now);
        (void)regenerated;
        pf.mark(2);
        need_gen = false;
        if (pass == 1) break;

        bool running = live && act != ACT_NOOP;
        int iter = 0;
        while (__any(running)) {
            bool do_turn = false, need_bfs = false, opened = false, own_req = false;
            int map_slot = -1;
            FillReq fr; fr.leave = fr.enter = 0;
            if (running) {
                switch (act) {
                case ACT_DOWNSTAIR:
                    do_turn = true; running = false;
                    break;
                case ACT_MOVE:
                case ACT_MOVE_UNTIL: {
                    bool done = move_player(S, c, E, w, dir, react, fr, (S.ovl && iter == 0) ? (const lds_u32 *)ovl_l : nullptr);
                    if (act == ACT_MOVE) { do_turn = true; running = false; break; }
                    uint32_t v = win_get(w, WIN_K(E.px - w.ox, E.py - w.oy));
                    uint32_t tile = (v & C_VISIBLE) ? glyph_of(v) : ' ';
                    if (done || (tile != '.' && tile != '#')) running = false;
                    else do_turn = true;
                    break;
                }
                case ACT_SEARCH:
                    opened = do_search(c, E, w, react);
                    do_turn = true; running = false;
                    break;
                }
            }
            if constexpr (BW == 1 || BW == 2) { if (__any(opened) && S.dc_walk) snapshot_walk_service(S, c, lane, e, opened); }
            pf.mark(28);
            if (do_turn) turn_passed(c, E, react);
            pf.mark(29);
            bool need_map = false;
            if (do_turn && E.mon_active > 0) need_map = monsters_prepass(S, c, E);
            pf.mark(30);
            if (need_map) {
                uint32_t part_bits = 0, own_bits = 0;
                if constexpr (BW == 1 || BW == 2) { part_bits = S.dc_part[e]; own_bits = S.dc_own[e]; }
                need_bfs = !dist_cache_lookup(S, E, POS(E.px, E.py), map_slot);
                if constexpr (BW == 1 || BW == 2) {
                    if (!need_bfs && ((part_bits >> map_slot) & 1u) && !dist_map_sufficient(S, c, E, map_slot)) {
                        need_bfs = true;
                        own_req = (own_bits >> map_slot) & 1u;
                        if (own_req) n_cont++;
                    }
                }
            }
            pf.mark(3);
            if (iter == 0) ovl_l[0] = w.dirty | ((fr.leave | fr.enter) ? 0x80000000u : 0u);
            fill_service(S, c, lane, e, fr);
            win_flush(c, E.cell, w);
            pf.mark(27);
#ifdef RG_EXP_NO_BFS
            need_bfs = false;
#endif
            uint64_t m = __ballot(need_bfs);
            if (need_bfs) n_bfs++;
            if (m) {
                unsigned long long tb0 = pf.p ? __builtin_amdgcn_s_memtime() : 0;
                const bool complete = bfs_service<BW>(S, c, reinterpret_cast<uint64_t *>(lds_grid), m, e, E.px, E.py, map_slot, lane, E.mc - lane, __ballot(own_req));
                if constexpr (BW == 1 || BW == 2) {
                    if (need_bfs) {
                        const uint32_t bit = 1u << map_slot;
                        const uint32_t part = S.dc_part[e], own = S.dc_own[e];
                        S.dc_part[e] = (uint16_t)(complete ? part & ~bit : part | bit);
                        S.dc_own[e] = (uint16_t)((own_req && !complete) ? own : own & ~bit);
                    }
                } else (void)complete;
                if (pf.p) { pf.rec(24, __builtin_amdgcn_s_memtime() - tb0); pf.rec(25, (unsigned long long)__popcll(m)); }
            }
            pf.mark(4);
            if (do_turn && E.mon_active > 0) ui_dead = monsters_move(S, c, E, map_slot, react);
            else if (do_turn) ui_dead = false;
            pf.mark(5);
            if (++iter > RG_MAX_W + RG_MAX_H && running) { running = false; E.err |= RG_FLAG_ERR_INTERNAL; }
            if (running) win_load(c, E.cell, w, E.px, E.py);
        }
        if (live) {
            flags = (react & 0x7f00u);
            if (react & R_REDRAW) flags |= RG_FLAG_REDRAW | ((react & R_HIST_STALE) ? RG_FLAG_HIST_STALE : 0);
            else flags |= old_flags & (RG_FLAG_REDRAW | RG_FLAG_HIST_STALE);
            flags |= old_flags & (RG_FLAG_HIST_LAG | RG_FLAG_HIST_DIRTY | (BND ? RG_FLAG_SCR_CHANGED : 0u));
            if ((react & R_HIST_CHANGED) || descends) flags |= RG_FLAG_HIST_DIRTY;
            if (react & R_STATUS) write_status(S, c, E);
            if (ui_dead) flags |= RG_FLAG_DEAD;
            steps += 1;
            terminal = (react & R_GRAVE) || steps >= c.max_steps;
            need_gen = terminal && c.auto_reset;
            if (S.ovl && (react & R_REDRAW) && !descends && !need_gen && act != ACT_MOVE_UNTIL &&
                !(old_flags & (RG_FLAG_REDRAW | RG_FLAG_HIST_STALE | RG_FLAG_HIST_LAG | RG_FLAG_HIST_DIRTY)) && !(ovl_l[0] >> 31)) {
                if (mirror_update<BND>(S, c, E, w, react, room_id_of(c, w.ox, w.oy))) flags = (flags & ~(RG_FLAG_REDRAW | RG_FLAG_HIST_DIRTY)) | ((!BND || S.bound_gray) ? 0u : RG_FLAG_SCR_CHANGED);
                inc_done = true;
            }
        }
    }
    pf.mark(6);
    int et = e;
    asm volatile("" : "+v"(et));
    E.e = et;
    bool pend = false; uint64_t pm = 0; uint32_t lbase = 0;
    if (BND && S.obs_list) {
        const uint32_t fw = (live ? ((terminal && c.auto_reset) ? RG_FLAG_REDRAW : flags) : old_flags);
        pend = valid && (fw & (RG_FLAG_REDRAW | RG_FLAG_SCR_CHANGED));
        pm = __ballot(pend);
        if (pm && lane == 0) lbase = atomicAdd(&S.obs_cnt[S.obs_par], (uint32_t)__popcll(pm));
    }
    if (S.stats) {
        const uint32_t cnt[8] = {(uint32_t)__popcll(__ballot(live && terminal && c.auto_reset)), (uint32_t)__popcll(__ballot(descends)),
                                 wave_sum(n_bfs), wave_sum(n_inline), wave_sum(n_taken), (uint32_t)__popcll(__ballot(live && (react & R_REDRAW))),
                                 (uint32_t)__popcll(__ballot(live)), (BW == 1 || BW == 2) ? wave_sum(n_cont) : 0u};
        const uint32_t n_nx = (uint32_t)__popcll(__ballot(descends && nxs == RG_NX_HIT));
        int ln = threadIdx.x;
        asm volatile("" : "+v"(ln));
        if (ln < RG_STAT_COLS) {
            uint32_t mine = ln == 8 ? n_nx : 0u;
#pragma unroll
            for (int k = 0; k < 8; k++) mine = ln == k ? cnt[k] : mine;
            if (mine) atomicAdd(&S.stats[(size_t)blockIdx.x * RG_STAT_COLS + ln], (unsigned long long)mine);
        }
    }
    if (valid && err) {
        S.flags[et] = (old_flags & ~RG_FLAG_ERR_MASK) | err;
        S.reward[et] = 0.f;
        S.done[et] = (old_flags & RG_FLAG_TERMINAL) ? 1 : 0;
        atomicOr(S.err_any, err);
    } else if (valid && !live) {
        S.reward[et] = 0.f; S.done[et] = (old_flags & RG_FLAG_TERMINAL) ? 1 : 0;
    } else if (valid) {
        if (terminal && c.auto_reset) {
            if (taken) {
                E.dlevel = 1; E.gold = c.init_gold; E.hp = E.hpmax = c.init_hp; E.plvl = 1; E.exp = 0; E.food = c.hunger_time;
            }
            write_status(S, c, E);
            S.dc_len[et] = 0; S.dc_head[et] = 0; S.dc_part[et] = 0; S.dc_own[et] = 0;
            steps = 0;
            flags = RG_FLAG_REDRAW | RG_FLAG_HIST_DIRTY;
            klog_new_episode(S, et);
        }
        if (E.err) { flags |= E.err; atomicOr(S.err_any, E.err); }
        if (terminal) flags |= RG_FLAG_TERMINAL;
        if (!taken) store_env(S, E);
        S.steps[et] = steps;
        S.flags[et] = flags;
        S.done[et] = terminal ? 1 : 0;
        if (S.ovl && !taken && !inc_done && ((react & R_REDRAW) || descends || (terminal && c.auto_reset))) {
            for (int s0 = 0; s0 < nrooms_k; s0++) {
                const uint32_t mw = E.mc[s0 * WAVE];
                S.ovl[(size_t)s0 * S.n + et] = (uint16_t)(((mw >> 24) & MF_ALIVE) ? ((mw & 0xffffu) | OVL_UNKNOWN) : OVL_NONE);
            }
            S.ovl[(size_t)nrooms_k * S.n + et] = (uint16_t)(POS(E.px, E.py) | OVL_UNKNOWN);
        }
        if (S.obs_rec && (flags & RG_FLAG_REDRAW) && !taken) {
            uint32_t *rec = S.obs_rec + (size_t)et * RG_OBS_REC_WORDS(nrooms_k);
            for (int s0 = 0; s0 < nrooms_k; s0 += 4) {
                uint32_t m4[4];
#pragma unroll
                for (int k = 0; k < 4; k++) m4[k] = E.mc[(s0 + k < nrooms_k ? s0 + k : s0) * WAVE];
                if (s0 + 4 <= nrooms_k) *reinterpret_cast<uint4 *>(rec + s0) = make_uint4(m4[0], m4[1], m4[2], m4[3]);
                else
                    for (int k = 0; k < 4 && s0 + k < nrooms_k; k++) rec[s0 + k] = m4[k];
            }
            rec[nrooms_k] = POS(E.px, E.py);
        }
        const int gold_before = gold0;
        const int gold_after = ((terminal && c.auto_reset) || (react & R_STATUS)) ? (int)E.gold : gold_before;
        const float bonus = (descends && !(terminal && c.auto_reset)) ? S.stair_reward : 0.f;
        S.reward[et] = (float)(gold_after - gold_before > 0 ? gold_after - gold_before : 0) + bonus;
    }
    bool on_next = false;
    if (valid && !live) on_next = S.stair_mark[(size_t)(S.stair_gen & 1) * S.n + et] != 0;
    if (live) on_next = ((descends || (terminal && c.auto_reset && !taken)) ? E.on_stairs != 0
                                                                              : (win_get(w, WIN_K(E.px - w.ox, E.py - w.oy)) & C_SURF_MASK) == S_STAIR);
    if (S.nx_state) {
        const bool fresh = live && (descends || (terminal && c.auto_reset));
        const bool ask = live && !fresh && (w.inb & WIN_STAIR) && (nxs == RG_NX_NONE || nxs == RG_NX_STALE);
        if (fresh && nxs != RG_NX_NONE) (void)__hip_atomic_fetch_and(&S.nx_state[et], RG_NX_DROP, __ATOMIC_RELAXED, __HIP_MEMORY_SCOPE_AGENT);
        if (__any(ask)) {
            if (ask) {
                uint32_t *q = S.nx_rng + et;
                const size_t n = (size_t)S.n;
                st_pub<true>(&q[0], E.rd.x); st_pub<true>(&q[n], E.rd.y); st_pub<true>(&q[2 * n], E.rd.z); st_pub<true>(&q[3 * n], E.rd.w);
                st_pub<true>(&q[8 * n], E.ri.x); st_pub<true>(&q[9 * n], E.ri.y); st_pub<true>(&q[10 * n], E.ri.z); st_pub<true>(&q[11 * n], E.ri.w);
                st_pub<true>(&S.nx->level[et], E.dlevel);
            }
            asm volatile("s_waitcnt vmcnt(0)" ::: "memory");
            if (ask) __hip_atomic_store(&S.nx_state[et], RG_NX_ASKED, __ATOMIC_RELAXED, __HIP_MEMORY_SCOPE_AGENT);
        }
    }
    if (BND && pm) {
        const uint32_t lb = uni(lbase);
        if (pend) S.obs_list[(size_t)S.obs_par * S.n + lb + lanes_below(pm)] = et;
    }
    take_spares(S, SPd, c, lane, et, taken, on_next);
    stair_publish(S, lane, et, valid, on_next);
    pf.mark(7);
    pf.finish();
}

#define STAIR_BLOCKS 256

#define RG_STEP_BLOCK_BODY(BWV, GMV, BNDV) \
    __builtin_amdgcn_s_setprio(3); \
    const int lane = threadIdx.x; \
    if (blockIdx.x == 0 && lane == 0) { \
        stair_recycle(S); \
        if (BNDV && S.obs_cnt) S.obs_cnt[S.obs_par ^ 1] = 0;   \
        __hip_atomic_store(S.launch_mark, (uint32_t)S.stair_gen + 1u, __ATOMIC_RELAXED, __HIP_MEMORY_SCOPE_AGENT);   \
    } \
    const bool stair = parity >= 0 && (int)blockIdx.x < STAIR_BLOCKS; \
    const int32_t *list = S.stair_list + (size_t)(S.stair_gen & 1) * S.n; \
    const int items = stair ? (int)S.stair_cnt[S.stair_gen % 3] : S.n; \
    const int first = stair ? (int)blockIdx.x : ((int)blockIdx.x - (parity >= 0 ? STAIR_BLOCKS : 0)) * epw; \
    uint32_t *next = S.stair_cnt + 4 + S.stair_gen % 3; \
    for (int i0 = first; i0 < items;) { \
        bool v; int e; \
        if (stair) { e = list[i0]; v = lane == 0 && e < S.n_keys && keys[e] == '>'; } \
        else { v = lane < epw && i0 + lane < items; e = v ? i0 + lane : 0; } \
        if (!stair || __any(v)) step_wave<BWV, GMV, BNDV>(S, SPd, c, keys, use_spares, stage_off, e, v, parity >= 0 ? (stair ? 1 : 2) : 0); \
        if (!stair || items <= STAIR_BLOCKS) break; \
        __syncthreads(); \
        uint32_t t = 0; \
        if (lane == 0) t = atomicAdd(next, 1u); \
        i0 = STAIR_BLOCKS + (int)uni(t); \
    }
template <int BW, bool BND = false>
__global__ void __launch_bounds__(WAVE) k_step(RgState S, const RgState *__restrict__ SPd, RgConfig c, const uint8_t *__restrict__ keys, int use_spares, int stage_off, int epw,
                                               int parity) {
    RG_STEP_BLOCK_BODY(BW, (BW != 0 ? 1 : 0), BND)
}
template <bool BND>
__global__ void __launch_bounds__(WAVE) __attribute__((amdgpu_waves_per_eu(2, 2)))
k_step_w32(RgState S, const RgState *__restrict__ SPd, RgConfig c, const uint8_t *__restrict__ keys, int use_spares, int stage_off, int epw, int parity) {
    RG_STEP_BLOCK_BODY(0, 0, BND)
}
__global__ void __launch_bounds__(WAVE) k_step_huge(RgState S, const RgState *__restrict__ SPd, RgConfig c, const uint8_t *__restrict__ keys, int use_spares, int stage_off,
                                                    int epw, int parity) {
    RG_STEP_BLOCK_BODY(4, 2, false)
}
#undef RG_STEP_BLOCK_BODY

static int gen_mode_of(const RgConfig *c) { const int nr = c->room_num_x * c->room_num_y; return nr <= 32 ? 0 : (nr <= 64 ? 1 : 2); }
extern "C" {
void rgk_build(const RgState *S, const RgConfig *c, hipStream_t st) {
    int hw = c->width * c->height;
    size_t smem = GEN_SLOT_BYTES(hw, c->room_num_x * c->room_num_y);
    const dim3 grid((S->n + BUILD_EPB - 1) / BUILD_EPB);
    switch (gen_mode_of(c)) {
    case 0: hipLaunchKernelGGL(k_build<0>, grid, dim3(WAVE), smem, st, *S, *c); break;
    case 1: hipLaunchKernelGGL(k_build<1>, grid, dim3(WAVE), smem, st, *S, *c); break;
    default: hipLaunchKernelGGL(k_build<2>, grid, dim3(WAVE), smem, st, *S, *c);
    }
}
void rgk_reset_compact(const uint8_t *mask, int n, int32_t *list, uint32_t *cnt, hipStream_t st) {
    (void)hipMemsetAsync(cnt, 0, 4, st);
    hipLaunchKernelGGL(k_reset_compact, dim3((n + COMPACT_THREADS - 1) / COMPACT_THREADS), dim3(COMPACT_THREADS), 0, st, mask, n, list, cnt);
}
void rgk_build_list(const RgState *S, const RgConfig *c, const int32_t *list, const uint32_t *cnt, uint8_t *mark, hipStream_t st) {
    int hw = c->width * c->height;
    size_t smem = GEN_SLOT_BYTES(hw, c->room_num_x * c->room_num_y);
    const dim3 grid((S->n + BUILD_EPB - 1) / BUILD_EPB);
    switch (gen_mode_of(c)) {
    case 0: hipLaunchKernelGGL(k_build_list<0>, grid, dim3(WAVE), smem, st, *S, *c, list, cnt, mark); break;
    case 1: hipLaunchKernelGGL(k_build_list<1>, grid, dim3(WAVE), smem, st, *S, *c, list, cnt, mark); break;
    default: hipLaunchKernelGGL(k_build_list<2>, grid, dim3(WAVE), smem, st, *S, *c, list, cnt, mark);
    }
}
int rgk_step_epw(int n, int slots_per_simd) {
    static const int epw_env = getenv("ROGUE_GYM_HIP_EPW") ? atoi(getenv("ROGUE_GYM_HIP_EPW")) : 0;
    int epw = WAVE;
    while (epw > 16 && (n + epw - 1) / epw < 1024) epw >>= 1;
    if (slots_per_simd < 2 && epw < WAVE && (n + epw - 1) / epw > 1008) { epw = (n + 1007) / 1008; if (epw > WAVE) epw = WAVE; }
    if (epw_env >= 16 && epw_env <= 64) epw = epw_env;
    return epw;
}
static size_t step_lds(const RgConfig *c, int *stage_off_out) {
    const int hw = c->width * c->height;
    size_t stage = GEN_SLOT_BYTES(hw, c->room_num_x * c->room_num_y);
    const bool n32 = c->width <= 96 && hw <= 4096;
    const size_t bfs_hi = n32 ? 0 : (size_t)10 * ((c->width + 63) / 64) * WAVE * 8;
    if (bfs_hi > stage) stage = bfs_hi;
    stage = (stage + 15) & ~(size_t)15;
    const int stage_off = STEP_LDS_MC + c->room_num_x * c->room_num_y * WAVE * 4;
    if (stage_off_out) *stage_off_out = stage_off;
    return (size_t)stage_off + stage;
}
size_t rgk_step_lds_per_cu(const RgConfig *c) { return step_lds(c, nullptr) * ((c->width <= 32 && gen_mode_of(c) == 0) ? 8 : 4); }
int rgk_step_bound_capable(const RgConfig *c) {
    const int hw = c->width * c->height;
    if (gen_mode_of(c) == 2) return 0;
    if (c->width <= 32 && gen_mode_of(c) == 0) return 1;
    return (c->width <= 96 && hw <= 4096 && c->width > 64) ? 1 : 0;
}
int rgk_step(const RgState *S, const RgState *SP_dev, const RgConfig *c, const uint8_t *keys, int use_spares, int parity, hipStream_t st, hipEvent_t ev0, hipEvent_t ev1) {
    const bool bnd = S->obs_list != nullptr && rgk_step_bound_capable(c);
    int hw = c->width * c->height;
    const bool n32 = c->width <= 96 && hw <= 4096;
    int stage_off = 0;
    const size_t smem = step_lds(c, &stage_off);
    const int epw = rgk_step_epw(S->n, (c->width <= 32 && gen_mode_of(c) == 0) ? 2 : 1);
    const int nb = (S->n + epw - 1) / epw;
    const dim3 grid(parity >= 0 ? STAIR_BLOCKS + nb : nb), block(WAVE);
#define RG_LAUNCH_STEP(K) do { if (ev0 || ev1) hipExtLaunchKernelGGL(K, grid, block, (uint32_t)smem, st, ev0, ev1, 0, *S, SP_dev, *c, keys, use_spares, stage_off, epw, parity); \
                               else hipLaunchKernelGGL(K, grid, block, smem, st, *S, SP_dev, *c, keys, use_spares, stage_off, epw, parity); } while (0)
    if (gen_mode_of(c) == 2) {
        static size_t raised[64] = {0};
        int dev = 0;
        (void)hipGetDevice(&dev);
        if (dev < 0 || dev >= 64 || smem > raised[dev]) {
            if (hipFuncSetAttribute(reinterpret_cast<const void *>(k_step_huge), hipFuncAttributeMaxDynamicSharedMemorySize, (int)smem) == hipSuccess && dev >= 0 && dev < 64) raised[dev] = smem;
        }
        RG_LAUNCH_STEP(k_step_huge);
    } else if (c->width <= 32 && gen_mode_of(c) == 0) { if (bnd) RG_LAUNCH_STEP(k_step_w32<true>); else RG_LAUNCH_STEP(k_step_w32<false>); }
    else if (n32 && c->width <= 64) RG_LAUNCH_STEP(k_step<1>);
    else if (n32) { if (bnd) RG_LAUNCH_STEP((k_step<2, true>)); else RG_LAUNCH_STEP(k_step<2>); }
    else if (c->width <= 128) RG_LAUNCH_STEP(k_step<3>);
    else RG_LAUNCH_STEP(k_step<4>);
#undef RG_LAUNCH_STEP
    return (int)grid.x;
}
void rgk_debug_descend(const RgState *S, const RgConfig *c, hipStream_t st) {
    int hw = c->width * c->height;
    const size_t smem = GEN_SLOT_BYTES(hw, c->room_num_x * c->room_num_y);
    const dim3 grid((S->n + BUILD_EPB - 1) / BUILD_EPB);
    switch (gen_mode_of(c)) {
    case 0: hipLaunchKernelGGL(k_debug_descend<0>, grid, dim3(WAVE), smem, st, *S, *c); break;
    case 1: hipLaunchKernelGGL(k_debug_descend<1>, grid, dim3(WAVE), smem, st, *S, *c); break;
    default: hipLaunchKernelGGL(k_debug_descend<2>, grid, dim3(WAVE), smem, st, *S, *c);
    }
}
void rgk_regen_gate(const uint32_t *mark, uint32_t target, uint32_t *err_any, hipStream_t st) { hipLaunchKernelGGL(k_regen_gate, dim3(1), dim3(WAVE), 0, st, mark, target, err_any); }
void rgk_regen(const RgState *SP, const RgConfig *c, int bulk, int spares, const uint32_t *mark, uint32_t target, uint32_t *err_any, hipStream_t st, hipEvent_t ev0, hipEvent_t ev1) {
    if (mark) rgk_regen_gate(mark, target, err_any, st);
    int hw = c->width * c->height;
    size_t smem = GEN_SLOT_BYTES(hw, c->room_num_x * c->room_num_y);
#ifdef RG_DEV_KNOBS
    static const int epb_env = getenv("ROGUE_GYM_HIP_REGEN_EPB") ? atoi(getenv("ROGUE_GYM_HIP_REGEN_EPB")) : 0;
    const int epb = (epb_env >= 4 && epb_env <= WAVE) ? epb_env : (spares == 1 ? 8 : WAVE);
    static const int claims_env = getenv("ROGUE_GYM_HIP_REGEN_CLAIMS") ? atoi(getenv("ROGUE_GYM_HIP_REGEN_CLAIMS")) : 1;
    const int max_claims = bulk ? WAVE : claims_env;
#else
    const int epb = spares == 1 ? 8 : WAVE, max_claims = bulk ? WAVE : 1;
#endif
    const dim3 grid((SP->n + epb - 1) / epb);
#define RG_LAUNCH_REGEN(K) do { if (ev0 || ev1) hipExtLaunchKernelGGL(K, grid, dim3(WAVE), (uint32_t)smem, st, ev0, ev1, 0, *SP, *c, epb, max_claims, spares); \
                                else hipLaunchKernelGGL(K, grid, dim3(WAVE), smem, st, *SP, *c, epb, max_claims, spares); } while (0)
    switch (gen_mode_of(c)) {
    case 0: RG_LAUNCH_REGEN(k_regen<0>); break;
    case 1: RG_LAUNCH_REGEN(k_regen<1>); break;
    default: RG_LAUNCH_REGEN(k_regen_huge);
    }
#undef RG_LAUNCH_REGEN
}
}
```

### rogue-gym_amd/csrc/rg_obs.hip

```cpp
#include <cstdlib>
#include "rg_device.h"

#define RENDER_THREADS 256
__device__ __forceinline__ bool in_same_room(const RgState &S, const RgConfig &c, int e, int ax, int ay, int bx, int by) {
    int id = room_id_of(c, ax, ay);
    if (id < 0 || room_id_of(c, bx, by) != id) return false;
    uint8_t meta = S.room_meta[id * S.n + e];
    if ((meta & RM_KIND_MASK) == RK_EMPTY) return true;
    int x0, y0, x1, y1;
    unpack_rect(S.room_rect[id * S.n + e], x0, y0, x1, y1);
    bool ina = ax >= x0 && ax < x1 && ay >= y0 && ay < y1, inb = bx >= x0 && bx < x1 && by >= y0 && by < y1;
    return ina == inb;
}

__global__ void __launch_bounds__(RENDER_THREADS) k_render(RgState S, RgConfig c) {
    __shared__ uint8_t s_scr[RG_MAX_W * RG_MAX_H];
    const int tid = threadIdx.x, W = c.width, H = c.height, HW = W * H, n = S.n;
    const int nrooms = c.room_num_x * c.room_num_y;
    for (int e = blockIdx.x; e < n; e += gridDim.x) {
        const uint32_t fl = S.flags[e];
        if (!(fl & RG_FLAG_REDRAW)) continue;
        const uint16_t *cell = S.cell + (size_t)e * HW;
        const bool upd_hist = !(fl & RG_FLAG_HIST_STALE);
        uint8_t *hist = S.hist + (size_t)e * HW;
// ... 206 lines not shown
    auto load_flag = [&](int base, int e) -> uint32_t {
        return (le < epb && base + le < n) ? S.flags[e] : 0u;
    };
    auto prefetch = [&](int base, int e, uint32_t fl) {
        Pre p; p.v0 = make_uint4(0, 0, 0, 0); p.rec = 0;
        if (le < epb && base + le < n) {
            if (fl & RG_FLAG_REDRAW) {
                if (lt < Q8) p.v0 = reinterpret_cast<const uint4 *>(S.cell + (size_t)e * HW)[lt];
                if (lt < rec_words) p.rec = rec_all[(size_t)e * rec_words + lt];
            } else if (fast_ok) {
                const uint32_t *m4 = reinterpret_cast<const uint32_t *>(S.screen + (size_t)e * HW);
                if (lt < Q4) p.v0.x = m4[lt];
                if (lt + tpe < Q4) p.v0.y = m4[lt + tpe];
                if (lt + 2 * tpe < Q4) p.v0.z = m4[lt + 2 * tpe];
                if (lt + 3 * tpe < Q4) p.v0.w = m4[lt + 3 * tpe];
            } else if (lt < Q8) {
                const uint2 m = reinterpret_cast<const uint2 *>(S.screen + (size_t)e * HW)[lt];
                p.v0.x = m.x; p.v0.y = m.y;
            }
        }
        return p;
    };
    const uint32_t smax = (uint32_t)symbols - 1;
    auto emit_glyphs = [&](float4 *o, int q, uint32_t g, bool &bad) {
        const int q4 = Q4;
        const uint32_t b0 = g & 0x7f, b1 = (g >> 8) & 0x7f, b2 = (g >> 16) & 0x7f, b3 = g >> 24;
        if (KIND == 0) {
            float4 v; v.x = lutf[b0]; v.y = lutf[b1]; v.z = lutf[b2]; v.w = lutf[b3];
            store_obs(&o[q], v);
        } else {
            const uint32_t s0 = luts[b0], s1 = luts[b1], s2 = luts[b2], s3 = luts[b3];
            bad = bad || s0 >= smax || s1 >= smax || s2 >= smax || s3 >= smax;
            for (uint32_t ch = 0; ch < smax; ch++) {
                float4 v;
                v.x = s0 == ch ? 1.f : 0.f; v.y = s1 == ch ? 1.f : 0.f; v.z = s2 == ch ? 1.f : 0.f; v.w = s3 == ch ? 1.f : 0.f;
                store_obs(&o[(size_t)ch * q4 + q], v);
            }
            float4 z; z.x = z.y = z.z = z.w = 0.f;
            for (uint32_t ch = smax; ch < (uint32_t)base_planes; ch++) store_obs(&o[(size_t)ch * q4 + q], z);
        }
    };
    auto emit = [&](float4 *o, int q, uint32_t g, const float *stf, int nst, const uint32_t *hist4, bool &bad) {
        const int q4 = Q4;
        emit_glyphs(o, q, g, bad);
        int p = base_planes;
        for (int b = 0; b < nst; b++, p++) {
            float4 sv; sv.x = sv.y = sv.z = sv.w = stf[b];
            store_obs(&o[(size_t)p * q4 + q], sv);
        }
        if (with_hist) {
            const uint32_t h4 = hist4[q];
            float4 a;
            a.x = (h4 & 0xff) ? 1.f : 0.f; a.y = (h4 & 0xff00) ? 1.f : 0.f; a.z = (h4 & 0xff0000) ? 1.f : 0.f; a.w = (h4 >> 24) ? 1.f : 0.f;
            store_obs(&o[(size_t)p * q4 + q], a);
        }
    };
    lds_barrier();
    const int base0 = blockIdx.x * epb;
    int e_cur = load_env(base0), e_nxt = load_env(base0 + stride), e_nn = load_env(base0 + 2 * stride);
    uint32_t fl_cur = load_flag(base0, e_cur), fl_nxt = load_flag(base0 + stride, e_nxt);
    Pre nxt = prefetch(base0, e_cur, fl_cur);
    for (int base = base0; base < n; base += stride) {
        const int e = e_cur;
        const bool valid = le < epb && base + le < n;
        const Pre cur = nxt;
        const uint32_t fl = fl_cur;
        e_cur = e_nxt; e_nxt = e_nn;
        fl_cur = fl_nxt;
        fl_nxt = load_flag(base + 2 * stride, e_nxt);
        e_nn = load_env(base + 3 * stride);
        if (base + stride < n) nxt = prefetch(base + stride, e_cur, fl_cur);
        const uint4 *cell4 = reinterpret_cast<const uint4 *>(S.cell + (size_t)e * HW);
        const uint4 v0 = cur.v0;
        const uint32_t t_rec = cur.rec;
        const bool my_fast = fast_ok && valid && !(fl & RG_FLAG_REDRAW);
        if (my_fast) {
            const int xe = GROUPS ? __builtin_amdgcn_readfirstlane(S.ext[e]) : e;
            float4 *o = reinterpret_cast<float4 *>(out + (size_t)xe * nplanes * HW);
            bool bad = false;
            if (lt < Q4) emit_glyphs(o, lt, v0.x & 0x7f7f7f7fu, bad);
            if (lt + tpe < Q4) emit_glyphs(o, lt + tpe, v0.y & 0x7f7f7f7fu, bad);
            if (lt + 2 * tpe < Q4) emit_glyphs(o, lt + 2 * tpe, v0.z & 0x7f7f7f7fu, bad);
            if (lt + 3 * tpe < Q4) emit_glyphs(o, lt + 3 * tpe, v0.w & 0x7f7f7f7fu, bad);
            if (KIND == 1 && bad) { atomicOr(&S.flags[e], RG_FLAG_ERR_TILE); atomicOr(err_any, RG_FLAG_ERR_TILE); }
            if (BOUND && lt == 0) atomicAnd(&S.flags[e], ~RG_FLAG_SCR_CHANGED);
        }
        const bool staged = valid && !my_fast;
        if (fast_ok && !(one_wave ? __any(staged) : staged)) continue;
        const bool redraw = staged && (fl & RG_FLAG_REDRAW);
        lds_barrier();
        if (staged) {
            if (redraw) {
                if (lt < rec_words) tb->w[lt] = t_rec;
                const bool upd_hist = !(fl & RG_FLAG_HIST_STALE) && (fl & RG_FLAG_HIST_DIRTY);
                uint2 *hist8 = reinterpret_cast<uint2 *>(S.hist + (size_t)e * HW);
                for (int i = lt; i < Q8; i += tpe) {
                    uint4 v = i == lt ? v0 : cell4[i];
                    uint32_t g[2], hb[2];
                    draw_cells8(v, i, W, HW, g, hb);
                    reinterpret_cast<uint2 *>(scr)[i] = make_uint2(g[0], g[1]);
                    if (upd_hist) hist8[i] = make_uint2(hb[0], hb[1]);
                }
            } else {
                const uint2 *m8 = reinterpret_cast<const uint2 *>(S.screen + (size_t)e * HW);
                for (int i = lt; i < Q8; i += tpe) reinterpret_cast<uint2 *>(scr)[i] = i == lt ? make_uint2(v0.x, v0.y) : m8[i];
            }
        }
        lds_barrier();
        const uint32_t ppos = redraw ? tb->w[nrooms] : 0;
        const int px = POS_X(ppos), py = POS_Y(ppos);
        if (redraw && lt < nrooms) {
            uint32_t w = tb->w[lt];
            if ((w >> 24) & MF_ALIVE) {
                int x = POS_X(w), y = POS_Y(w);
                const bool show = monster_shown(c, tb, nrooms, px, py, x, y);
                const uint32_t under = scr[y * W + x];
                if (show && (under & 0x80u) && under != (0x80u | '*')) scr[y * W + x] = (uint8_t)(0x80u | mtile[(w >> 16) & 0xff]);
            }
        }
        lds_barrier();
        if (redraw && lt == 0 && (scr[py * W + px] & 0x80u)) scr[py * W + px] = (uint8_t)(0x80u | '@');
        lds_barrier();
        if (with_hist) __syncthreads();
        if (staged) {
            uint32_t *m4 = reinterpret_cast<uint32_t *>(S.screen + (size_t)e * HW);
            const uint32_t *scr4 = reinterpret_cast<const uint32_t *>(scr);
            const uint32_t *hist4 = reinterpret_cast<const uint32_t *>(S.hist + (size_t)e * HW);
            const int xe = GROUPS ? __builtin_amdgcn_readfirstlane(S.ext[e]) : e;
            float4 *o = reinterpret_cast<float4 *>(out + (size_t)xe * nplanes * HW);
            float stf[9];
            int nst = 0;
            for (int b = 0; b < 9; b++)
                if (sflag & (1u << b)) stf[nst++] = (float)S.status[(size_t)e * 10 + kStatusIdx[b]];
            bool bad = false;
            for (int q = lt; q < Q4; q += tpe) {
                const uint32_t g = scr4[q] & 0x7f7f7f7fu;
                if (redraw) m4[q] = g;
                emit(o, q, g, stf, nst, hist4, bad);
            }
            if (KIND == 1 && bad) { atomicOr(&S.flags[e], RG_FLAG_ERR_TILE); atomicOr(err_any, RG_FLAG_ERR_TILE); }
            const uint32_t seen = BOUND ? RG_FLAG_SCR_CHANGED : 0u;
            if (redraw && lt == 0) {
                const uint32_t clr = seen | RG_FLAG_REDRAW | RG_FLAG_HIST_STALE | RG_FLAG_HIST_LAG | ((fl & RG_FLAG_HIST_STALE) ? 0u : RG_FLAG_HIST_DIRTY);
                const uint32_t set = (fl & RG_FLAG_HIST_STALE) ? RG_FLAG_HIST_LAG : 0u;
                if (KIND == 1) {
                    atomicAnd(&S.flags[e], ~clr);
                    if (set) atomicOr(&S.flags[e], set);
                } else S.flags[e] = (fl & ~clr) | set;
            } else if (BOUND && !redraw && lt == 0) atomicAnd(&S.flags[e], ~RG_FLAG_SCR_CHANGED);
        }
    }
}

#ifndef OBS_RUN
#define OBS_RUN 4
#endif
#ifndef OBS_STREAM_WAVES
#define OBS_STREAM_WAVES 16384
#endif
__global__ void __launch_bounds__(WAVE) k_obs_stream(RgState S, RgConfig c, float *__restrict__ out, int hi_prio) {
    if (hi_prio) __builtin_amdgcn_s_setprio(3);
    __shared__ float lutf[128];
    __shared__ uint8_t mtile[RG_MAX_ENEMY_KINDS + 6];
    __shared__ __align__(16) uint8_t scr[512];
    __shared__ ObsTabs tb;
    const int lane = threadIdx.x, W = c.width, HW = W * c.height, Q4 = HW >> 2, Q8 = HW >> 3, n = S.n;
    const int nrooms = c.room_num_x * c.room_num_y, rec_words = RG_OBS_REC_WORDS(nrooms);
    for (int g = lane; g < 128; g += WAVE) lutf[g] = (float)(uint8_t)tile_to_sym((uint32_t)g) / (float)(uint8_t)c.symbols;
    for (int g = lane; g < RG_MAX_ENEMY_KINDS + 6; g += WAVE) mtile[g] = c.mon[g].tile;
    lds_barrier();
    auto gray4 = [&](uint32_t w) {
        w &= 0x7f7f7f7fu;
        float4 v; v.x = lutf[w & 0xff]; v.y = lutf[(w >> 8) & 0xff]; v.z = lutf[(w >> 16) & 0xff]; v.w = lutf[w >> 24];
        return v;
    };
    struct Run { uint32_t fl, w0[OBS_RUN], w1[OBS_RUN]; };
    auto load_run = [&](int r, Run &R) {
        const int base = r * OBS_RUN, cnt = n - base;
        R.fl = lane < cnt && lane < OBS_RUN ? S.flags[base + lane] : 0u;
        const uint32_t *m = reinterpret_cast<const uint32_t *>(S.screen) + (size_t)base * Q4;
#pragma unroll
        for (int i = 0; i < OBS_RUN; i++) {
            R.w0[i] = i < cnt && lane < Q4 ? m[i * Q4 + lane] : 0u;
            R.w1[i] = i < cnt && lane + WAVE < Q4 ? m[i * Q4 + lane + WAVE] : 0u;
        }
    };
    const int nruns = (n + OBS_RUN - 1) / OBS_RUN;
    Run cur;
    load_run(blockIdx.x, cur);
    for (int r = blockIdx.x; r < nruns; r += gridDim.x) {
        const int base = r * OBS_RUN, cnt = n - base < OBS_RUN ? n - base : OBS_RUN;
        Run nxt;
        load_run(r + gridDim.x, nxt);
        const uint32_t fl = cur.fl;
#ifdef RG_EXP_OBS_STREAM_BOUND
        uint64_t rmask = 0;
#else
        uint64_t rmask = __ballot(fl & RG_FLAG_REDRAW);
#endif
        auto load_tiles = [&](int e, uint4 &v, uint32_t &rec) {
            v = lane < Q8 ? reinterpret_cast<const uint4 *>(S.cell + (size_t)e * HW)[lane] : make_uint4(0, 0, 0, 0);
            rec = lane < rec_words ? S.obs_rec[(size_t)e * rec_words + lane] : 0u;
        };
        uint4 tv = make_uint4(0, 0, 0, 0);
        uint32_t trec = 0;
        if (rmask) load_tiles(base + __builtin_ctzll(rmask), tv, trec);
        float4 *o = reinterpret_cast<float4 *>(out) + (size_t)base * Q4;
#pragma unroll
        for (int i = 0; i < OBS_RUN; i++) {
            if (i >= cnt || ((rmask >> i) & 1)) continue;
            if (lane < Q4) store_obs(&o[i * Q4 + lane], gray4(cur.w0[i]));
            if (lane + WAVE < Q4) store_obs(&o[i * Q4 + lane + WAVE], gray4(cur.w1[i]));
        }
        while (rmask) {
            const int i = __builtin_ctzll(rmask);
            rmask &= rmask - 1;
            const int e = base + i;
            const uint32_t fle = __builtin_amdgcn_readlane(fl, i);
            const uint4 v = tv;
            const uint32_t t_rec = trec;
            if (rmask) load_tiles(base + __builtin_ctzll(rmask), tv, trec);
            lds_barrier();
            if (lane < rec_words) tb.w[lane] = t_rec;
            const bool upd_hist = !(fle & RG_FLAG_HIST_STALE) && (fle & RG_FLAG_HIST_DIRTY);
            if (lane < Q8) {
                uint32_t g[2], hb[2];
                draw_cells8(v, lane, W, HW, g, hb);
                reinterpret_cast<uint2 *>(scr)[lane] = make_uint2(g[0], g[1]);
                if (upd_hist) reinterpret_cast<uint2 *>(S.hist + (size_t)e * HW)[lane] = make_uint2(hb[0], hb[1]);
            }
            lds_barrier();
            const uint32_t ppos = tb.w[nrooms];
            const int px = POS_X(ppos), py = POS_Y(ppos);
            if (lane < nrooms) {
                const uint32_t mw = tb.w[lane];
                if ((mw >> 24) & MF_ALIVE) {
                    const int x = POS_X(mw), y = POS_Y(mw);
                    const uint32_t under = scr[y * W + x];
                    if (monster_shown(c, &tb, nrooms, px, py, x, y) && (under & 0x80u) && under != (0x80u | '*')) scr[y * W + x] = (uint8_t)(0x80u | mtile[(mw >> 16) & 0xff]);
                }
            }
            lds_barrier();
            if (lane == 0 && (scr[py * W + px] & 0x80u)) scr[py * W + px] = (uint8_t)(0x80u | '@');
            lds_barrier();
            uint32_t *m4 = reinterpret_cast<uint32_t *>(S.screen + (size_t)e * HW);
            float4 *oe = reinterpret_cast<float4 *>(out) + (size_t)e * Q4;
            for (int q = lane; q < Q4; q += WAVE) {
                const uint32_t g = reinterpret_cast<const uint32_t *>(scr)[q] & 0x7f7f7f7fu;
                m4[q] = g;
                store_obs(&oe[q], gray4(g));
            }
            if (lane == 0)
                S.flags[e] = (fle & ~(RG_FLAG_REDRAW | RG_FLAG_HIST_STALE | RG_FLAG_HIST_LAG | ((fle & RG_FLAG_HIST_STALE) ? 0u : RG_FLAG_HIST_DIRTY))) |
                             ((fle & RG_FLAG_HIST_STALE) ? RG_FLAG_HIST_LAG : 0u);
        }
        cur = nxt;
    }
}

#define RG_PUBLIC_FLAGS (RG_FLAG_TERMINAL | RG_FLAG_DEAD | RG_FLAG_MSG_MASK | RG_FLAG_ERR_MASK)
__global__ void __launch_bounds__(256) k_pack(const uint8_t *__restrict__ screen, const uint8_t *__restrict__ hist, const int32_t *__restrict__ status,
                                              const float *__restrict__ reward, const uint32_t *__restrict__ flags, int n, int hw, int with_hist, uint32_t *__restrict__ out) {
    const int qs = hw >> 2, qr = qs + 12 + (with_hist ? qs : 0);
    const size_t total = (size_t)n * qr;
    for (size_t g = (size_t)blockIdx.x * blockDim.x + threadIdx.x; g < total; g += (size_t)gridDim.x * blockDim.x) {
        const int e = (int)(g / qr), i = (int)(g - (size_t)e * qr);
        uint32_t v;
        if (i < qs) v = reinterpret_cast<const uint32_t *>(screen + (size_t)e * hw)[i];
        else if (i < qs + 10) v = (uint32_t)status[(size_t)e * 10 + (i - qs)];
        else if (i == qs + 10) v = __float_as_uint(reward[e]);
        else if (i == qs + 11) v = flags[e] & RG_PUBLIC_FLAGS;
        else v = reinterpret_cast<const uint32_t *>(hist + (size_t)e * hw)[i - qs - 12];
        out[g] = v;
    }
}

__global__ void __launch_bounds__(256) k_export(const uint32_t *__restrict__ screen, const uint32_t *__restrict__ hist, const uint32_t *__restrict__ status,
                                                const uint32_t *__restrict__ flags, uint32_t *__restrict__ err_any, size_t w_scr, size_t w_status, size_t w_flags,
                                                uint32_t *__restrict__ o_screen, uint32_t *__restrict__ o_hist, uint32_t *__restrict__ o_status,
                                                uint32_t *__restrict__ o_flags, uint32_t *__restrict__ o_err) {
    const size_t total = (o_screen ? 2 * w_scr : 0) + w_status + w_flags;
    const size_t base = o_screen ? 2 * w_scr : 0;
    for (size_t g = (size_t)blockIdx.x * blockDim.x + threadIdx.x; g < total; g += (size_t)gridDim.x * blockDim.x) {
        if (g < base) { if (g < w_scr) o_screen[g] = screen[g]; else o_hist[g - w_scr] = hist[g - w_scr]; }
        else if (g < base + w_status) o_status[g - base] = status[g - base];
        else o_flags[g - base - w_status] = flags[g - base - w_status];
    }
    if (blockIdx.x == 0 && threadIdx.x == 0) {
        const uint32_t e = atomicExch(err_any, 0u);
        *o_err = e;
    }
}
__global__ void __launch_bounds__(256) k_scatter_rows(const uint8_t *__restrict__ src, uint8_t *__restrict__ dst, const int32_t *__restrict__ ext, int n, int row_bytes) {
    if ((row_bytes & 3) == 0) {
        const int rw = row_bytes >> 2;
        const size_t total = (size_t)n * rw;
        for (size_t g = (size_t)blockIdx.x * blockDim.x + threadIdx.x; g < total; g += (size_t)gridDim.x * blockDim.x) {
            const int e = (int)(g / rw), i = (int)(g - (size_t)e * rw);
            reinterpret_cast<uint32_t *>(dst)[(size_t)ext[e] * rw + i] = reinterpret_cast<const uint32_t *>(src)[g];
        }
    } else {
        const size_t total = (size_t)n * row_bytes;
        for (size_t g = (size_t)blockIdx.x * blockDim.x + threadIdx.x; g < total; g += (size_t)gridDim.x * blockDim.x) {
            const int e = (int)(g / row_bytes), i = (int)(g - (size_t)e * row_bytes);
            dst[(size_t)ext[e] * row_bytes + i] = src[g];
        }
    }
}
__global__ void __launch_bounds__(256) k_gather_keys(const uint8_t *__restrict__ keys, const int32_t *__restrict__ ext, uint8_t *__restrict__ dst, int n) {
    const int e = blockIdx.x * 256 + threadIdx.x;
    if (e < n) dst[e] = keys[ext[e]];
}

__global__ void k_probe_clock(unsigned long long *out, int spin) {
    const unsigned long long c0 = __builtin_amdgcn_s_memtime(), r0 = __builtin_amdgcn_s_memrealtime();
    uint32_t x = threadIdx.x + 1u;
    for (int i = 0; i < spin; i++) x = x * 1664525u + 1013904223u;
    const unsigned long long c1 = __builtin_amdgcn_s_memtime(), r1 = __builtin_amdgcn_s_memrealtime();
    if (threadIdx.x == 0) { out[0] = c1 - c0; out[1] = r1 - r0; out[2] = x; out[3] = (unsigned long long)spin; }
}

__global__ void __launch_bounds__(256) k_encode_scalar(const uint8_t *__restrict__ screen, const uint8_t *__restrict__ hist, const int32_t *__restrict__ status,
                                                       uint32_t *__restrict__ flags, uint32_t *__restrict__ err_any, int n, int hw, size_t rs, size_t rst, int symbols,
                                                       int planes_sym, uint32_t sflag, int with_hist, int kind, float *__restrict__ out, const int32_t *__restrict__ ext) {
    const size_t total = (size_t)n * hw;
    const int base = kind ? planes_sym : 1;
    const int nplanes = base + __popc(sflag) + (with_hist ? 1 : 0);
    for (size_t g = (size_t)blockIdx.x * blockDim.x + threadIdx.x; g < total; g += (size_t)gridDim.x * blockDim.x) {
        int e = (int)(g / hw), i = (int)(g - (size_t)e * hw);
        uint32_t sym = tile_to_sym(screen[(size_t)e * rs + i]);
        float *o = out + (size_t)(ext ? ext[e] : e) * nplanes * hw + i;
        if (!kind) o[0] = (float)(uint8_t)sym / (float)(uint8_t)symbols;
        else {
            if (sym >= (uint32_t)symbols - 1) { if (flags) atomicOr(&flags[e], RG_FLAG_ERR_TILE); atomicOr(err_any, RG_FLAG_ERR_TILE); }
            for (int ch = 0; ch < planes_sym; ch++) o[(size_t)ch * hw] = (sym == (uint32_t)ch && ch < symbols - 1) ? 1.f : 0.f;
        }
        int p = base;
        for (int b = 0; b < 9; b++)
            if (sflag & (1u << b)) { o[(size_t)p * hw] = (float)status[(size_t)e * rst + kStatusIdx[b]]; p++; }
        if (with_hist) o[(size_t)p * hw] = hist[(size_t)e * rs + i] ? 1.f : 0.f;
    }
}

enum { CROP_D_CA, CROP_D_AREA, CROP_D_WC, CROP_D_BB, CROP_D_BW };
__device__ __forceinline__ uint32_t mdiv(uint32_t x, uint32_t m, uint32_t shifts, int which) {
    return (uint32_t)(((uint64_t)x * m) >> ((shifts >> (6 * which)) & 63));
}
struct RgCropArgs {
    int ry, rx, hc, wc, area, ca;
    int run, bh, bw, bb;
    int planes, nst, with_hist, nplanes;
    uint32_t sflag;
    uint32_t m[5], shifts;
};
#define CROP_UNROLL 8
template <int KIND>
__global__ void __launch_bounds__(WAVE) k_obs_crop(const uint16_t *__restrict__ p_pos, const int32_t *__restrict__ status, const uint8_t *__restrict__ screen,
                                                  const uint8_t *__restrict__ hist, uint32_t *__restrict__ flags, const int32_t *__restrict__ ext, int n, int W, int H,
                                                  int symbols, RgCropArgs a, float *__restrict__ out, int32_t *__restrict__ centers, uint32_t *__restrict__ err_any) {
    extern __shared__ __align__(16) uint8_t smem[];
    float *lutf = reinterpret_cast<float *>(smem);
    uint8_t *luts = smem + 512;
    int4 *geo = reinterpret_cast<int4 *>(smem + 640);
    float *stf = reinterpret_cast<float *>(smem + 640 + 16 * a.run);
    uint8_t *box = smem + 640 + 52 * a.run;
    uint8_t *hbox = box + (size_t)a.run * a.bb;
    const int lane = threadIdx.x, HW = W * H, R = a.run;
    for (int g = lane; g < 128; g += WAVE) {
        const uint32_t sy = tile_to_sym((uint32_t)g);
        luts[g] = (uint8_t)sy;
        lutf[g] = (float)(uint8_t)sy / (float)(uint8_t)symbols;
    }
    const uint32_t smax = (uint32_t)symbols - 1;
    const int nruns = (n + R - 1) / R;
    for (int run = blockIdx.x; run < nruns; run += gridDim.x) {
        const int base = run * R, cnt = n - base < R ? n - base : R;
        lds_barrier();
        if (lane < cnt) {
            const int e = base + lane;
            const uint32_t pos = p_pos[e];
            const int cx = POS_X(pos), cy = POS_Y(pos);
            const int oy = min(max(cy - a.ry, 0), H - a.bh), ox = min(max(cx - a.rx, 0), W - a.bw);
            geo[lane] = make_int4(cy, cx, oy, ox);
            int p = 0;
            for (int b = 0; b < 9; b++)
                if (a.sflag & (1u << b)) stf[lane * 9 + p++] = (float)status[(size_t)e * 10 + kStatusIdx[b]];
            if (centers) {
                const int xe = ext ? ext[e] : e;
                centers[2 * (size_t)xe] = cy;
                centers[2 * (size_t)xe + 1] = cx;
            }
        }
        lds_barrier();
        const int tot = cnt * a.bb;
        auto box_cell = [&](int k, int &r, int &y, int &x) {
            r = (int)mdiv((uint32_t)k, a.m[CROP_D_BB], a.shifts, CROP_D_BB);
            const int t = k - r * a.bb, j = (int)mdiv((uint32_t)t, a.m[CROP_D_BW], a.shifts, CROP_D_BW);
            const int4 gg = geo[r];
            y = gg.z + j; x = gg.w + (t - j * a.bw);
        };
        for (int k0 = 0; k0 < tot; k0 += WAVE * CROP_UNROLL) {
            uint32_t gv[CROP_UNROLL], hv[CROP_UNROLL];
#pragma unroll
            for (int u = 0; u < CROP_UNROLL; u++) {
                const int kk = k0 + u * WAVE + lane;
                gv[u] = hv[u] = 0;
                if (KIND == 0 || kk < tot) {
                    int r, y, x;
                    box_cell(min(kk, tot - 1), r, y, x);
// ... 157 lines not shown
    typedef uint32_t wv __attribute__((ext_vector_type(CW)));
    constexpr uint32_t ONE = DT == RG_OBS_F16 ? 0x3C00u : 0x3F80u;
    __shared__ uint16_t lut16[128];
    __shared__ uint8_t luts[128];
    const int tid = threadIdx.x, B = blockDim.x, Q = hw / (4 * CW);
    for (int g = tid; g < 128; g += B) {
        const uint32_t sy = tile_to_sym((uint32_t)g);
        luts[g] = (uint8_t)sy;
        if (KIND == 0) lut16[g] = (uint16_t)cvt16<DT>((float)(uint8_t)sy / (float)(uint8_t)symbols);
    }
    const int nplanes = planes + __popc(sflag) + (with_hist ? 1 : 0);
    const uint32_t smax = (uint32_t)symbols - 1;
    const int per_run = run * Q;
    int el[OBS_T_ITEMS], ql[OBS_T_ITEMS];
#pragma unroll
    for (int k = 0; k < OBS_T_ITEMS; k++) {
        const int j = tid + k * B;
        el[k] = j < per_run ? j / Q : -1;
        ql[k] = el[k] < 0 ? 0 : j - el[k] * Q;
    }
    struct Run { wv w[OBS_T_ITEMS], h[OBS_T_ITEMS]; };
    auto load_run = [&](int r, Run &R) {
        const int base = r * run;
        const wv *m = reinterpret_cast<const wv *>(screen + (size_t)base * hw), *hm = reinterpret_cast<const wv *>(hist + (size_t)base * hw);
#pragma unroll
        for (int k = 0; k < OBS_T_ITEMS; k++) {
            const bool ok = el[k] >= 0 && base + el[k] < n;
            R.w[k] = ok ? m[tid + k * B] : (wv)0u;
            R.h[k] = ok && with_hist ? hm[tid + k * B] : (wv)0u;
        }
    };
    auto gray2 = [&](uint32_t w, int hi) -> uint32_t {
        return (uint32_t)lut16[(w >> (16 * hi)) & 0x7f] | ((uint32_t)lut16[(w >> (16 * hi + 8)) & 0x7f] << 16);
    };
    auto one2 = [&](bool a, bool b) -> uint32_t { return (a ? ONE : 0u) | (b ? ONE << 16 : 0u); };
    lds_barrier();
    const int nruns = (n + run - 1) / run;
    Run cur;
    load_run(blockIdx.x, cur);
    for (int r = blockIdx.x; r < nruns; r += gridDim.x) {
        Run nxt;
        load_run(r + gridDim.x, nxt);
        const int base = r * run;
#pragma unroll
        for (int k = 0; k < OBS_T_ITEMS; k++) {
            const int e = base + el[k];
            if (el[k] < 0 || e >= n) continue;
            u4v *o = out + (size_t)e * nplanes * Q + ql[k];
            uint32_t w[CW], h[CW];
#pragma unroll
            for (int t = 0; t < CW; t++) { w[t] = cur.w[k][t]; h[t] = cur.h[k][t]; }
            bool bad = false;
            if (KIND == 0) {
                store_obs16(o, gray2(w[0], 0), gray2(w[0], 1), gray2(w[1], 0), gray2(w[1], 1));
            } else if (KIND == 1) {
                uint32_t s[8];
#pragma unroll
                for (int t = 0; t < 8; t++) {
                    s[t] = luts[(w[t >> 2] >> ((t & 3) * 8)) & 0x7f];
                    bad = bad || s[t] >= smax;
                }
                for (uint32_t ch = 0; ch < smax; ch++)
                    store_obs16(o + (size_t)ch * Q, one2(s[0] == ch, s[1] == ch), one2(s[2] == ch, s[3] == ch), one2(s[4] == ch, s[5] == ch), one2(s[6] == ch, s[7] == ch));
                for (uint32_t ch = smax; ch < (uint32_t)planes; ch++) store_obs16(o + (size_t)ch * Q, 0u, 0u, 0u, 0u);
            } else {
                uint32_t id[CW];
#pragma unroll
                for (int t = 0; t < CW; t++) {
                    const uint32_t a = luts[w[t] & 0x7f], b = luts[(w[t] >> 8) & 0x7f], c = luts[(w[t] >> 16) & 0x7f], d = luts[(w[t] >> 24) & 0x7f];
                    bad = bad || a >= smax || b >= smax || c >= smax || d >= smax;
                    id[t] = a | (b << 8) | (c << 16) | (d << 24);
                }
                store_obs16(o, id[0], id[1], id[CW - 2], id[CW - 1]);
            }
            int p = planes;
            if (KIND != 2 && sflag) {
                const int eu = __builtin_amdgcn_readfirstlane(e);
                for (int b = 0; b < 9; b++)
                    if (sflag & (1u << b)) {
                        const uint32_t v = cvt16<DT>((float)status[(size_t)eu * 10 + kStatusIdx[b]]) * 0x10001u;
                        store_obs16(o + (size_t)p * Q, v, v, v, v);
                        p++;
                    }
            }
            if (with_hist) {
                if (KIND == 2) store_obs16(o + (size_t)p * Q, nonzero_bytes(h[0]), nonzero_bytes(h[1]), nonzero_bytes(h[CW - 2]), nonzero_bytes(h[CW - 1]));
                else
                    store_obs16(o + (size_t)p * Q, one2(h[0] & 0xffu, h[0] & 0xff00u), one2(h[0] & 0xff0000u, h[0] >> 24), one2(h[1] & 0xffu, h[1] & 0xff00u),
                                one2(h[1] & 0xff0000u, h[1] >> 24));
            }
            if (KIND != 0 && bad) { atomicOr(&flags[e], RG_FLAG_ERR_TILE); atomicOr(err_any, RG_FLAG_ERR_TILE); }
        }
        cur = nxt;
    }
}

static void host_magic(RgCropArgs &a, int which, uint32_t d) {
    uint32_t l = 0;
    while ((1u << l) < d) l++;
    const uint32_t s = 30 + l;
    a.m[which] = (uint32_t)(((1ull << s) + d - 1) / d);
    a.shifts |= s << (6 * which);
}
extern "C" {
void rgk_render(const RgState *S, const RgConfig *c, hipStream_t st) {
    int blocks = S->n < 8192 ? S->n : 8192;
    hipLaunchKernelGGL(k_render, dim3(blocks), dim3(RENDER_THREADS), 0, st, *S, *c);
}
int rgk_obs(const RgState *S, const RgConfig *c, uint32_t sflag, int with_hist, int kind, float *out, uint32_t *err_any, int planes_sym, int bound, hipStream_t st, hipEvent_t ev0, hipEvent_t ev1) {
    int hw = c->width * c->height;
    if (hw & 7) return 0;
    if (c->room_num_x * c->room_num_y > RG_OBS_MAX_ROOMS || !S->obs_rec) return 0;
    int q8 = hw / 8;
    int tpe = q8 >= OBS_THREADS ? OBS_THREADS : ((q8 + 63) / 64) * 64;
    if (tpe > OBS_THREADS) tpe = OBS_THREADS;
    if (RG_OBS_REC_WORDS(c->room_num_x * c->room_num_y) > tpe) return 0;
    const int bthreads = tpe, epb = 1;
    const bool groups = S->ext != nullptr;
    size_t smem = 512 + 128 + 64 + (size_t)epb * OBS_ENV_BYTES(hw);
    int blocks = (S->n + epb - 1) / epb;
    {
        int cap = bthreads <= 64 ? 16384 : 8192;
#ifdef RG_DEV_KNOBS
        if (const char *ev = getenv("RG_OBS_BLOCKS")) cap = atoi(ev);
#endif
        if (blocks > cap) blocks = cap;
    }
    const int hi_prio = !(c->width <= 32 && c->room_num_x * c->room_num_y <= 32);
    bool stream = !kind && !groups && !bound && sflag == 0 && !with_hist && tpe == WAVE;
#ifdef RG_DEV_KNOBS
    if (const char *ev = getenv("RG_OBS_STREAM")) stream = stream && atoi(ev) != 0;
#endif
    if (stream) {
        int sblocks = (S->n + OBS_RUN - 1) / OBS_RUN, cap = OBS_STREAM_WAVES;
#ifdef RG_DEV_KNOBS
        if (const char *ev = getenv("RG_OBS_BLOCKS")) if (atoi(ev) > 0) cap = atoi(ev);
#endif
        if (sblocks > cap) sblocks = cap;
        if (ev0 || ev1) hipExtLaunchKernelGGL(k_obs_stream, dim3(sblocks), dim3(WAVE), 0, st, ev0, ev1, 0, *S, *c, out, hi_prio);
        else hipLaunchKernelGGL(k_obs_stream, dim3(sblocks), dim3(WAVE), 0, st, *S, *c, out, hi_prio);
        return 1;
    }
#define RG_LAUNCH_OBS(...) do { if (ev0 || ev1) hipExtLaunchKernelGGL((__VA_ARGS__), dim3(blocks), dim3(bthreads), (uint32_t)smem, st, ev0, ev1, 0, *S, *c, sflag, with_hist, out, err_any, tpe, epb, planes_sym, hi_prio); \
                               else hipLaunchKernelGGL((__VA_ARGS__), dim3(blocks), dim3(bthreads), smem, st, *S, *c, sflag, with_hist, out, err_any, tpe, epb, planes_sym, hi_prio); } while (0)
    if (bound && !groups && !kind) RG_LAUNCH_OBS(k_obs<0, false, true>);
    else if (bound && !groups) RG_LAUNCH_OBS(k_obs<1, false, true>);
    else if (!kind && !groups) RG_LAUNCH_OBS(k_obs<0, false>);
    else if (!kind) RG_LAUNCH_OBS(k_obs<0, true>);
    else if (!groups) RG_LAUNCH_OBS(k_obs<1, false>);
    else RG_LAUNCH_OBS(k_obs<1, true>);
#undef RG_LAUNCH_OBS
    return 1;
}
void rgk_encode(const uint8_t *screen, const uint8_t *hist, const int32_t *status, uint32_t *flags, uint32_t *err_any, int n, int hw, size_t rs, size_t rst,
                int symbols, int planes_sym, uint32_t sflag, int with_hist, int kind, float *out, const int32_t *ext, hipStream_t st) {
    if ((hw & 3) == 0 && (rs & 3) == 0) {
        size_t total = (size_t)n * (hw >> 2);
        int blocks = (int)((total + 255) / 256 < 16384 ? (total + 255) / 256 : 16384);
        if (blocks < 1) blocks = 1;
        if (!kind) hipLaunchKernelGGL(k_gray, dim3(blocks), dim3(256), 0, st, screen, hist, status, n, hw, rs, rst, symbols, sflag, with_hist, out, ext);
        else hipLaunchKernelGGL(k_symbol, dim3(blocks), dim3(256), 0, st, screen, hist, status, flags, err_any, n, hw, rs, rst, symbols, planes_sym, sflag, with_hist, out, ext);
    } else {
        size_t total = (size_t)n * hw;
        int blocks = (int)((total + 255) / 256 < 16384 ? (total + 255) / 256 : 16384);
        hipLaunchKernelGGL(k_encode_scalar, dim3(blocks), dim3(256), 0, st, screen, hist, status, flags, err_any, n, hw, rs, rst, symbols, planes_sym, sflag, with_hist, kind, out, ext);
    }
}
void rgk_export(const RgState *S, uint32_t *err_any, void *o_screen, void *o_hist, void *o_status, void *o_flags, uint32_t *o_err, hipStream_t st) {
    const size_t n = (size_t)S->n, w_scr = n * (size_t)S->hw / 4, w_status = n * 10, w_flags = n;
    const size_t total = (o_screen ? 2 * w_scr : 0) + w_status + w_flags;
    int blocks = (int)((total + 255) / 256 < 1024 ? (total + 255) / 256 : 1024);
    hipLaunchKernelGGL(k_export, dim3(blocks < 1 ? 1 : blocks), dim3(256), 0, st, reinterpret_cast<const uint32_t *>(S->screen), reinterpret_cast<const uint32_t *>(S->hist),
                       reinterpret_cast<const uint32_t *>(S->status), S->flags, err_any, w_scr, w_status, w_flags, static_cast<uint32_t *>(o_screen), static_cast<uint32_t *>(o_hist),
                       static_cast<uint32_t *>(o_status), static_cast<uint32_t *>(o_flags), o_err);
}
void rgk_pack(const RgState *S, int with_hist, uint8_t *out, hipStream_t st) {
    const int hw = S->hw;
    const size_t rec = (size_t)hw + RG_COMPACT_FIXED_BYTES + (with_hist ? hw : 0);
    const size_t total = (size_t)S->n * (rec / 4);
    int blocks = (int)((total + 255) / 256 < 16384 ? (total + 255) / 256 : 16384);
    if (blocks < 1) blocks = 1;
    hipLaunchKernelGGL(k_pack, dim3(blocks), dim3(256), 0, st, S->screen, S->hist, S->status, S->reward, S->flags, S->n, hw, with_hist, reinterpret_cast<uint32_t *>(out));
}
void rgk_scatter_rows(const void *src, void *dst, const int32_t *ext, int n, int row_bytes, hipStream_t st) {
    const size_t total = (size_t)n * row_bytes;
    int blocks = (int)((total + 255) / 256 < 8192 ? (total + 255) / 256 : 8192);
    if (blocks < 1) blocks = 1;
    hipLaunchKernelGGL(k_scatter_rows, dim3(blocks), dim3(256), 0, st, (const uint8_t *)src, (uint8_t *)dst, ext, n, row_bytes);
}
void rgk_gather_keys(const uint8_t *keys, const int32_t *ext, uint8_t *dst, int n, hipStream_t st) {
    hipLaunchKernelGGL(k_gather_keys, dim3((n + 255) / 256), dim3(256), 0, st, keys, ext, dst, n);
}
int rgk_obs_crop(const RgState *S, const RgConfig *c, int kind, int ry, int rx, uint32_t sflag, int with_hist, int planes_sym, float *out, int32_t *centers,
                 uint32_t *err_any, hipStream_t st) {
    RgCropArgs a;
    const int hc = 2 * ry + 1;
    a.ry = ry; a.rx = rx; a.hc = hc; a.wc = 2 * rx + 1; a.area = hc * a.wc;
    a.planes = kind ? planes_sym : 1; a.nst = __builtin_popcount(sflag); a.with_hist = with_hist ? 1 : 0; a.sflag = sflag;
    a.nplanes = a.planes + a.nst + a.with_hist;
    a.ca = a.nplanes * a.area;
    a.bh = hc < c->height ? hc : c->height; a.bw = a.wc < c->width ? a.wc : c->width; a.bb = a.bh * a.bw;
    a.run = 4;
    const size_t stage = (size_t)a.bb * (1 + a.with_hist);
    while (a.run < 64 && (size_t)a.run * a.ca * 4 < 4096 && (size_t)a.run * 2 * stage <= 16384) a.run *= 2;
    if ((uint64_t)a.run * a.ca >= (1ull << 30) || (uint64_t)a.run * a.bb >= (1ull << 30)) return 0;
    a.shifts = 0;
    host_magic(a, CROP_D_CA, (uint32_t)a.ca); host_magic(a, CROP_D_AREA, (uint32_t)a.area); host_magic(a, CROP_D_WC, (uint32_t)a.wc);
    host_magic(a, CROP_D_BB, (uint32_t)a.bb); host_magic(a, CROP_D_BW, (uint32_t)a.bw);
    const size_t smem = 640 + 52 * (size_t)a.run + (size_t)a.run * stage;
    const int nruns = (S->n + a.run - 1) / a.run;
    const int blocks = nruns < OBS_STREAM_WAVES ? nruns : OBS_STREAM_WAVES;
    if (kind) hipLaunchKernelGGL(k_obs_crop<1>, dim3(blocks), dim3(WAVE), smem, st, S->p_pos, S->status, S->screen, S->hist, S->flags, S->ext, S->n, c->width, c->height,
                                 c->symbols, a, out, centers, err_any);
    else hipLaunchKernelGGL(k_obs_crop<0>, dim3(blocks), dim3(WAVE), smem, st, S->p_pos, S->status, S->screen, S->hist, S->flags, S->ext, S->n, c->width, c->height,
                            c->symbols, a, out, centers, err_any);
    return 1;
}
int rgk_redraw(const RgState *S, const RgConfig *c, hipStream_t st) {
    const int hw = c->width * c->height;
    if ((hw & 7) || c->room_num_x * c->room_num_y > RG_OBS_MAX_ROOMS || !S->obs_rec) return 0;
    int B = ((hw / 8 + WAVE - 1) / WAVE) * WAVE;
    if (B > OBS_THREADS) B = OBS_THREADS;
    const int nruns = (S->n + REDRAW_RUN - 1) / REDRAW_RUN;
    hipLaunchKernelGGL(k_redraw, dim3(nruns < 8192 ? nruns : 8192), dim3(B), (size_t)hw, st, *S, *c);
    return 1;
}
int rgk_obs_typed(const RgState *S, const RgConfig *c, int kind, int dtype, uint32_t sflag, int with_hist, int planes_sym, void *out, uint32_t *err_any,
                  hipStream_t st, hipEvent_t ev0, hipEvent_t ev1) {
    const int hw = c->width * c->height, cells = dtype == RG_OBS_U8 ? 16 : 8;
    if (hw % cells) return 0;
    const int Q = hw / cells;
    int B = ((Q + WAVE - 1) / WAVE) * WAVE;
    if (B > OBS_THREADS) B = OBS_THREADS;
    if (Q > OBS_T_ITEMS * B) return 0;
    int run = sflag ? 1 : OBS_T_ITEMS * B / Q;
    if (run < 1) run = 1;
    const int nruns = (S->n + run - 1) / run, cap = B <= WAVE ? OBS_STREAM_WAVES : 4096;
    const int blocks = nruns < cap ? nruns : cap;
    const int planes = kind == 1 ? planes_sym : 1;
#define RG_LAUNCH_TYPED(...) do { if (ev0 || ev1) hipExtLaunchKernelGGL((__VA_ARGS__), dim3(blocks), dim3(B), 0, st, ev0, ev1, 0, S->screen, S->hist, S->status, S->flags, err_any, S->n, hw, \
                                                                        (int)c->symbols, planes, sflag, with_hist, run, static_cast<u4v *>(out)); \
                                  else hipLaunchKernelGGL((__VA_ARGS__), dim3(blocks), dim3(B), 0, st, S->screen, S->hist, S->status, S->flags, err_any, S->n, hw, (int)c->symbols, planes, sflag, \
                                                          with_hist, run, static_cast<u4v *>(out)); } while (0)
    if (kind == 2) RG_LAUNCH_TYPED(k_obs_typed<2, RG_OBS_U8>);
    else if (kind == 0 && dtype == RG_OBS_F16) RG_LAUNCH_TYPED(k_obs_typed<0, RG_OBS_F16>);
    else if (kind == 0) RG_LAUNCH_TYPED(k_obs_typed<0, RG_OBS_BF16>);
    else if (dtype == RG_OBS_F16) RG_LAUNCH_TYPED(k_obs_typed<1, RG_OBS_F16>);
    else RG_LAUNCH_TYPED(k_obs_typed<1, RG_OBS_BF16>);
#undef RG_LAUNCH_TYPED
    return 1;
}
void rgk_probe_clock(unsigned long long *out, int spin, hipStream_t st) { hipLaunchKernelGGL(k_probe_clock, dim3(1), dim3(64), 0, st, out, spin); }
}
```

### rogue-gym_amd/csrc/rg_state.h

```cpp
#pragma once
#include <cstdint>

#include "rg_config.h"

#define C_SURF_MASK 0x0007u
#define C_DOOR      0x0008u
#define C_ATTR_SHIFT 4
#define C_VISITED   0x0010u
#define C_HIDDEN    0x0020u
#define C_VISIBLE   0x0040u
#define C_DRAWN     0x0080u
#define C_LOCKED    0x0100u
#define C_DARK      0x0200u
#define C_ATTR_MASK 0x03f0u
#define C_MAZE      0x0400u
#define C_GOLD      0x0800u

enum { S_PASSAGE = 0, S_FLOOR, S_WALLX, S_WALLY, S_STAIR, S_DOOR, S_TRAP, S_NONE };

#define RM_KIND_MASK 0x03u
#define RM_DARK      0x04u
#define RM_VISITED   0x08u
#define RM_HAS_GOLD  0x10u
enum { RK_NORMAL = 0, RK_MAZE = 1, RK_EMPTY = 2 };

#define MF_ALIVE   0x01u
#define MF_ACTIVE  0x02u
#define MF_PENDING 0x04u
#define MF_RANDOM 0x08u
#define MF_DIR_SHIFT 4
#define MF_REACH 0x80u
#define MF_TURN_BITS (MF_PENDING | MF_RANDOM | (7u << MF_DIR_SHIFT) | MF_REACH)

#define RG_MAX_EDGES (2 * RG_MAX_ROOMS)
#define RG_WALK_WORDS(w) ((w) <= 64 ? 2 : 3)
#define RG_PARTIAL_MAPS(w, h, rooms) ((w) <= 96 && (w) * (h) <= 4096 && (rooms) <= 64 && !((w) <= 32 && (rooms) <= 32))

#define RG_STAT_COLS 16
#define RG_NX_ASKED 1u
#define RG_NX_CLAIMED 6u
#define RG_NX_READY 3u
#define RG_NX_NONE 0u
#define RG_NX_DROP 4u
#define RG_NX_STALE 8u
#define RG_NX_HIT 9u
struct RgNext {
    uint16_t *cell;
    uint32_t *room_rect, *gold_pos, *gold_amt;
    uint8_t *room_meta;
    uint32_t *level;
};
struct RgState {
    int32_t n;
    int32_t hw;
    uint16_t *cell;
    uint8_t *screen;
    uint8_t *hist;
    uint16_t *p_pos;
    int32_t *p_hp, *p_hpmax, *p_lvl;
    uint32_t *p_exp, *food, *quiet, *pack_gold, *dlevel;
    uint32_t *steps, *flags;
    float *reward;
    uint8_t *done;
    uint32_t *rng;
    uint64_t *seed_lo, *seed_hi;
    uint8_t *reseed;
    uint32_t *build_ctr;
    const uint32_t *init_draws;
    uint64_t *range_lo, *range_span;
    uint32_t *room_rect;
    uint8_t *room_meta;
    uint32_t *mon_w0;
    int32_t *mon_hp;
    uint32_t *mon_exp;
    uint32_t *mon_cnt;
    uint32_t *gold_pos, *gold_amt;
    uint32_t *edge_a, *edge_b;
    uint16_t *maze_stack;
    int32_t maze_cap;
    uint16_t *dc_map;
    uint16_t *dc_key;
    uint8_t *dc_head, *dc_len;
    uint16_t *dc_part, *dc_own;
    uint32_t *dc_walk;
    int keep_spares;
    int full_bfs;
    unsigned long long *prof;
    uint32_t *sp_ready;
    int32_t sp_slots;
    int32_t *status;
    uint32_t *obs_rec;
    uint16_t *ovl;
    float *bound_gray;
    const float *gray_lut;
    int32_t *obs_list;
    uint32_t *obs_cnt;
    int32_t obs_par;
    uint8_t *klog;
    uint32_t *klog_len;
    uint8_t *klog_cur;
    int32_t klog_cap;
    unsigned long long *stats;
    uint8_t *stair_mark;
    int32_t *stair_list;
    uint32_t *stair_cnt;
    int32_t stair_gen;
    uint32_t *launch_mark;
    uint8_t *on_stairs;
    uint32_t *nx_state;
    uint32_t *nx_rng;
    const struct RgNext *nx;
    const int32_t *ext;
    uint32_t *err_any;
    int32_t n_keys;
    float stair_reward;
};
```

### rogue-gym_amd/rogue_gym_python/_rogue_gym.py

```python
import ctypes as C
import weakref
import json
import os

import numpy as np

_HERE = os.path.dirname(os.path.abspath(__file__))
_SO = os.environ.get("ROGUE_GYM_HIP_LIB") or os.path.join(os.path.dirname(_HERE), "librogue_gym_hip.so")

RG_FLAG_TERMINAL = 0x1
RG_FLAG_DEAD = 0x2
RG_FLAG_MSG_SHIFT = 8
RG_FLAG_MSG_MASK = 0x7F00
RG_FLAG_ERR_MASK = 0x00FF0000

STATUS_KEYS = ("dungeon_level", "gold", "hp_current", "hp_max", "str_current", "str_max", "defense", "player_level", "exp", "hunger")


class RgDebugState(C.Structure):
    _fields_ = [
        ("px", C.c_int32), ("py", C.c_int32), ("dungeon_level", C.c_int32), ("hp", C.c_int32), ("hp_max", C.c_int32),
        ("player_level", C.c_int32), ("n_monsters", C.c_int32), ("n_gold", C.c_int32),
        ("exp", C.c_uint32), ("food_left", C.c_uint32), ("quiet", C.c_uint32), ("pack_gold", C.c_uint32), ("steps", C.c_uint32),
        ("rng", C.c_uint32 * 12),
        ("mon_x", C.c_int32 * 384), ("mon_y", C.c_int32 * 384), ("mon_type", C.c_int32 * 384), ("mon_active", C.c_int32 * 384), ("mon_hp", C.c_int32 * 384),
        ("mon_exp", C.c_uint32 * 384),
        ("gold_x", C.c_int32 * 384), ("gold_y", C.c_int32 * 384), ("gold_amount", C.c_int32 * 384),
        ("n_rooms", C.c_int32), ("room_rect", C.c_uint32 * 384), ("room_meta", C.c_int32 * 384),
    ]


_lib = None

_INT_FUNCS = (
    "rg_create", "rg_dims", "rg_env_dims", "rg_env_symbols", "rg_set_stream", "rg_seed", "rg_reset", "rg_step", "rg_step_prefix", "rg_step_obs_gray", "rg_step_fetch", "rg_sync", "rg_screen", "rg_hist", "rg_status", "rg_flags",
    "rg_reward", "rg_done", "rg_set_stair_reward", "rg_obs_bind", "rg_obs_gray", "rg_obs_symbol", "rg_obs_channels", "rg_fetch_states", "rg_encode_host", "rg_encode_host_batch", "rg_obs_host",
    "rg_host_alloc", "rg_dev_alloc", "rg_snapshot_take", "rg_dev_read", "rg_dev_read_rows", "rg_compact_record_bytes", "rg_pack_compact", "rg_expand_compact", "rg_comm_unique_id", "rg_comm_init", "rg_comm_destroy", "rg_comm_count", "rg_allgather_compact", "rg_status_vec", "rg_history_enable", "rg_history_keys",
    "rg_dump_history", "rg_counters", "rg_counters_ex", "rg_probe_sclk", "rg_dump_config", "rg_config_canonical", "rg_config_resolved", "rg_config_schema", "rg_debug_fetch", "rg_debug_descend", "rg_timing_enable", "rg_timing_read", "rg_timing_read_all", "rg_timing_read_samples",
    "rg_state_record_bytes", "rg_state_save", "rg_state_load", "rg_obs_crop", "rg_obs_dtype_bytes", "rg_obs_typed", "rg_step_obs_typed",
    "rg_reset_envs", "rg_reset_mask", "rg_seed_envs",
)


def load_library():
    global _lib
    if _lib is not None:
        return _lib
    if not os.path.exists(_SO):
        raise RuntimeError(
            "librogue_gym_hip.so is not built (%s). Run `python -c 'import __graft_entry__ as g; g.build()'` "
            "or rogue-gym_amd/csrc/build.sh -- there is no CPU fallback." % _SO
        )
    try:
        import torch
    except ImportError:
        pass
    L = C.CDLL(_SO)
    vp, i32, u32, sz = C.c_void_p, C.c_int, C.c_uint32, C.c_size_t
    sig = {
        "rg_create": [C.POINTER(C.c_char_p), i32, C.c_uint64, i32, i32, C.POINTER(vp)],
        "rg_destroy": [vp],
        "rg_last_error": [vp],
        "rg_dims": [vp] + [C.POINTER(i32)] * 4,
        "rg_env_symbols": [vp, vp], "rg_env_dims": [vp, vp, vp],
        "rg_set_stream": [vp, vp],
        "rg_seed": [vp, C.POINTER(C.c_uint64), C.POINTER(C.c_uint64), i32],
        "rg_reset": [vp],
        "rg_step": [vp, vp, i32],
        "rg_step_prefix": [vp, vp, i32, i32],
        "rg_step_obs_gray": [vp, vp, i32, u32, i32, vp],
        "rg_step_fetch": [vp, vp, i32, vp, vp, vp, vp],
        "rg_sync": [vp],
        "rg_screen": [vp, C.POINTER(vp)], "rg_hist": [vp, C.POINTER(vp)], "rg_status": [vp, C.POINTER(vp)], "rg_flags": [vp, C.POINTER(vp)],
        "rg_reward": [vp, C.POINTER(vp)], "rg_done": [vp, C.POINTER(vp)], "rg_set_stair_reward": [vp, C.c_float],
        "rg_obs_bind": [vp, i32, u32, i32, vp], "rg_obs_gray": [vp, u32, i32, vp], "rg_obs_symbol": [vp, u32, i32, vp], "rg_obs_channels": [vp, i32, u32, i32],
        "rg_fetch_states": [vp, vp, vp, vp, vp],
        "rg_encode_host": [i32, vp, vp, vp, i32, i32, i32, u32, i32, i32, vp],
        "rg_encode_host_batch": [i32, i32, vp, vp, vp, i32, i32, i32, u32, i32, i32, vp],
        "rg_obs_host": [vp, i32, u32, i32, vp],
        "rg_host_alloc": [sz, C.POINTER(vp)], "rg_host_free": [vp],
        "rg_dev_alloc": [i32, sz, C.POINTER(vp)], "rg_dev_free": [i32, vp], "rg_snapshot_take": [vp, vp], "rg_dev_read": [vp, vp, vp, sz], "rg_dev_read_rows": [vp, vp, sz, vp, sz, i32],
        "rg_compact_record_bytes": [vp, i32], "rg_pack_compact": [vp, i32, vp], "rg_expand_compact": [vp, vp, i32, i32, i32, u32, i32, vp],
        "rg_comm_unique_id": [vp], "rg_comm_init": [vp, vp, i32, i32], "rg_comm_destroy": [vp], "rg_comm_count": [vp, vp, vp], "rg_allgather_compact": [vp, i32, vp],
        "rg_status_vec": [vp, u32, vp],
        "rg_history_enable": [vp, i32], "rg_history_keys": [vp, i32, i32, vp, sz, C.POINTER(u32)],
        "rg_dump_history": [vp, i32, i32, C.c_char_p, sz, C.POINTER(sz)],
        "rg_counters": [vp, C.POINTER(C.c_uint64), i32], "rg_counters_ex": [vp, C.POINTER(C.c_uint64), i32, i32], "rg_probe_sclk": [vp, C.POINTER(C.c_double)],
        "rg_timing_enable": [vp, i32], "rg_timing_read": [vp, C.POINTER(C.c_double), C.POINTER(C.c_uint64)],
        "rg_timing_read_all": [vp, i32, C.POINTER(C.c_double), C.POINTER(C.c_uint64), C.POINTER(C.c_uint64)],
        "rg_timing_read_samples": [vp, i32, C.POINTER(C.c_float), i32, C.POINTER(i32)],
        "rg_dump_config": [vp, i32, C.c_char_p, sz], "rg_config_canonical": [C.c_char_p, C.c_char_p, sz],
        "rg_config_resolved": [C.c_char_p, C.c_char_p, sz], "rg_config_schema": [C.c_char_p, sz, C.POINTER(sz)],
        "rg_debug_fetch": [vp, i32, C.POINTER(RgDebugState), vp], "rg_debug_descend": [vp],
        "rg_state_record_bytes": [vp], "rg_state_save": [vp, vp, i32, i32, vp], "rg_state_load": [vp, vp, sz, vp, i32, i32],
        "rg_obs_crop": [vp, i32, i32, i32, u32, i32, vp, vp],
        "rg_obs_dtype_bytes": [i32], "rg_obs_typed": [vp, i32, i32, u32, i32, vp], "rg_step_obs_typed": [vp, vp, i32, i32, i32, u32, i32, vp],
        "rg_reset_envs": [vp, vp, i32, i32], "rg_reset_mask": [vp, vp], "rg_seed_envs": [vp, vp, C.POINTER(C.c_uint64), C.POINTER(C.c_uint64), i32],
    }
    optional = {"rg_timing_read_samples", "rg_obs_bind", "rg_state_record_bytes", "rg_state_save", "rg_state_load", "rg_obs_crop", "rg_obs_dtype_bytes", "rg_obs_typed",
                "rg_step_obs_typed", "rg_reset_envs", "rg_reset_mask", "rg_seed_envs"} if os.environ.get("ROGUE_GYM_HIP_LIB") else set()
    for name, argtypes in sig.items():
        if name in optional and not hasattr(L, name):
            continue
        getattr(L, name).argtypes = argtypes
    L.rg_destroy.restype = None
    L.rg_host_free.restype = None
    L.rg_dev_free.restype = None
    L.rg_last_error.restype = C.c_char_p
    L.rg_build_id.restype = C.c_char_p
    L.rg_build_id.argtypes = []
    for name in _INT_FUNCS:
        if name in optional and not hasattr(L, name):
            continue
        getattr(L, name).restype = C.c_int
    _lib = L
    return L


def _default_device():
    return int(os.environ.get("ROGUE_GYM_HIP_DEVICE", os.environ.get("LOCAL_RANK", "0")))


class _PinnedPool:

    def __init__(self, L):
        self.L, self.free, self.closed = L, {}, False

    def take(self, nbytes):
        lst = self.free.get(nbytes)
        if lst:
            return lst.pop()
        p = C.c_void_p()
        if self.L.rg_host_alloc(nbytes, C.byref(p)):
            raise RuntimeError("Error in rogue-gym: " + self.L.rg_last_error(None).decode())
        return p.value

    def give(self, ptr, nbytes):
        if self.closed:
            self.L.rg_host_free(C.c_void_p(ptr))
        else:
            self.free.setdefault(nbytes, []).append(ptr)

    def close(self):
        self.closed = True
        for lst in self.free.values():
            for ptr in lst:
                self.L.rg_host_free(C.c_void_p(ptr))
        self.free = {}


class _DevPool:

    def __init__(self, L, device):
        self.L, self.device, self.free, self.closed = L, device, {}, False

    def take(self, nbytes):
        lst = self.free.get(nbytes)
        if lst:
            return lst.pop()
        p = C.c_void_p()
        if self.L.rg_dev_alloc(self.device, nbytes, C.byref(p)):
            raise RuntimeError("Error in rogue-gym: " + self.L.rg_last_error(None).decode())
        return p.value

    def give(self, ptr, nbytes):
        if self.closed:
            self.L.rg_dev_free(self.device, C.c_void_p(ptr))
        else:
            self.free.setdefault(nbytes, []).append(ptr)

    def close(self):
        self.closed = True
        for lst in self.free.values():
            for ptr in lst:
                self.L.rg_dev_free(self.device, C.c_void_p(ptr))
        self.free = {}


class _Lease:
    __slots__ = ("pool", "ptr", "nbytes")

    def __init__(self, pool, nbytes):
        self.pool, self.nbytes = pool, nbytes
        self.ptr = pool.take(nbytes)

    def __del__(self):
        try:
            self.pool.give(self.ptr, self.nbytes)
        except Exception:
            pass


class _DevLease:
    __slots__ = ("pool", "ptr", "nbytes")

    def __init__(self, pool, nbytes):
        self.pool, self.nbytes = pool, nbytes
        self.ptr = pool.take(nbytes)

    def __del__(self):
        try:
            self.pool.give(self.ptr, self.nbytes)
        except Exception:
            pass


def _leased(pool, shape, dtype):
    nbytes = int(np.prod(shape)) * np.dtype(dtype).itemsize
    lease = _Lease(pool, nbytes)
    raw = (C.c_uint8 * nbytes).from_address(lease.ptr)
    raw._lease = lease
    return np.frombuffer(raw, dtype=dtype).reshape(shape)


def _leased_many(pool, specs):
    sizes = [(int(np.prod(sh)) * np.dtype(dt).itemsize + 15) & ~15 for sh, dt in specs]
    lease = _Lease(pool, sum(sizes))
    raw = (C.c_uint8 * sum(sizes)).from_address(lease.ptr)
    raw._lease = lease
    whole, out, off = np.frombuffer(raw, dtype=np.uint8), [], 0
    for (sh, dt), sz in zip(specs, sizes):
        out.append(whole[off:off + int(np.prod(sh)) * np.dtype(dt).itemsize].view(dt).reshape(sh))
        off += sz
    return out


class _Handle:

    def __init__(self, configs, max_steps, auto_reset, device=None):
        L = load_library()
        self.L = L
        self.device = _default_device() if device is None else device
        n = len(configs)
        arr = (C.c_char_p * n)()
        for i, cfg in enumerate(configs):
            arr[i] = None if cfg is None else cfg.encode("utf-8")
        h = C.c_void_p()
        rc = L.rg_create(arr, n, int(max_steps), self.device, int(auto_reset), C.byref(h))
        if rc:
            msg = L.rg_last_error(None).decode()
            if msg.startswith("Failed to parse config"):
                raise RuntimeError(msg)
            raise RuntimeError("Error in rogue-gym: " + msg)
        self.h = h
        hh, ww, ss, nn = C.c_int(), C.c_int(), C.c_int(), C.c_int()
        L.rg_dims(h, C.byref(hh), C.byref(ww), C.byref(ss), C.byref(nn))
        self.height, self.width, self.symbols, self.n = hh.value, ww.value, ss.value, nn.value
        self.env_symbols = np.empty(self.n, np.int32)
        L.rg_env_symbols(h, self.env_symbols.ctypes.data)
        self.uniform_symbols = bool((self.env_symbols == self.symbols).all())
        self.env_heights, self.env_widths = np.empty(self.n, np.int32), np.empty(self.n, np.int32)
        L.rg_env_dims(h, self.env_heights.ctypes.data, self.env_widths.ctypes.data)
        self.mixed_sizes = bool((self.env_heights != self.height).any() or (self.env_widths != self.width).any())
        self.pool = _PinnedPool(L)
        self.dev_pool = _DevPool(L, self.device)
        self.lazy = {}
        self.epoch = 0
        self.fast_step = True

    def check(self, rc):
        if rc:
            raise RuntimeError("Error in rogue-gym: " + self.L.rg_last_error(self.h).decode())

    def close(self):
        if getattr(self, "h", None):
            for ref in list(self.lazy.values()):
                b = ref()
                if b is not None:
                    b._materialise()
            self.L.rg_destroy(self.h)
            self.h = None
            self.pool.close()
            self.dev_pool.close()

    def __del__(self):
        try:
            self.close()
        except Exception:
            pass

    def fetch(self):
        n = self.n
        screen = np.empty((n, self.height, self.width), np.uint8)
        hist = np.empty((n, self.height, self.width), np.uint8)
        status = np.empty((n, 10), np.int32)
        flags = np.empty(n, np.uint32)
        self.check(self.L.rg_fetch_states(self.h, screen.ctypes.data, hist.ctypes.data, status.ctypes.data, flags.ctypes.data))
        return screen, hist, status, flags

    def snapshot(self):
        return StateBatch(self)

    def step_keys_host(self, keys):
        self.check(self.L.rg_step_prefix(self.h, keys.ctypes.data, int(keys.shape[0]), 0))
        self.epoch += 1
        self.check(self.L.rg_sync(self.h))

    def states(self):
        return self.snapshot()

    def debug_state(self, env):
        out = RgDebugState()
        cells = np.empty((self.height, self.width), np.uint16)
        self.check(self.L.rg_debug_fetch(self.h, env, C.byref(out), cells.ctypes.data))
        return out, cells

    def history_keys(self, env, previous=False):
        n = C.c_uint32()
        rc = self.L.rg_history_keys(self.h, env, int(previous), None, 0, C.byref(n))
        self.check(rc)
        buf = (C.c_uint8 * max(1, n.value))()
        self.check(self.L.rg_history_keys(self.h, env, int(previous), buf, len(buf), C.byref(n)))
        return bytes(buf[: n.value])

    def state_bytes(self):
        r = self.L.rg_state_record_bytes(self.h)
        if r < 0:
            self.check(1)
        return r

    def save_state_host(self, env=0):
        r = self.state_bytes()
        ptr = self.dev_pool.take(r)
        try:
            ids = (C.c_int32 * 1)(int(env))
            self.check(self.L.rg_state_save(self.h, ids, 1, 0, C.c_void_p(ptr)))
            buf = (C.c_uint8 * r)()
            self.check(self.L.rg_dev_read(self.h, C.c_void_p(ptr), buf, r))
            self.check(self.L.rg_sync(self.h))
        finally:
            self.dev_pool.give(ptr, r)
        return bytes(buf)

    def load_state_host(self, record, env=0):
        import torch

        data = bytes(record)
        if len(data) < 64 or len(data) % 16:
            raise ValueError("not a state record (%d bytes)" % len(data))
        dev = torch.frombuffer(bytearray(data), dtype=torch.uint8).to(torch.device("cuda", self.device))
        torch.cuda.synchronize(dev.device)
        ids = (C.c_int32 * 1)(int(env))
        self.check(self.L.rg_state_load(self.h, C.c_void_p(dev.data_ptr()), len(data), ids, 1, 0))
        self.epoch += 1
        self.check(self.L.rg_sync(self.h))

    def dump_history(self, env, previous=False):
        need = C.c_size_t()
        self.check(self.L.rg_dump_history(self.h, env, int(previous), None, 0, C.byref(need)))
        buf = C.create_string_buffer(need.value)
        self.check(self.L.rg_dump_history(self.h, env, int(previous), buf, need.value, None))
        return buf.value.decode()


_EAGER_MAX_BYTES = 1 << 16
_LAZY_MIN_BYTES = 1 << 20
_LAZY_MAX_BYTES = 1 << 30
_IMAGE_BATCH_LIMIT = 1 << 28


class StateBatch:

    def __init__(self, handle, keys=None):
        self._hd = handle
        n, h, w = handle.n, handle.height, handle.width
        self.n, self.symbols = n, handle.symbols
        self.mixed_sizes = handle.mixed_sizes
        eager = keys is not None and handle.fast_step and not self.mixed_sizes and (h * w) % 4 == 0 and n * h * w <= _EAGER_MAX_BYTES
        if eager:
            self.status, self.flags, self._screen, self._hist = _leased_many(handle.pool, [((n, 10), np.int32), ((n,), np.uint32), ((n, h, w), np.uint8), ((n, h, w), np.uint8)])
        else:
            self.status = _leased(handle.pool, (n, 10), np.int32)
            self.flags = _leased(handle.pool, (n,), np.uint32)
        self._snap = None
        if keys is not None and not (handle.fast_step and not self.mixed_sizes and (h * w) % 4 == 0):
            handle.step_keys_host(keys)
            keys = None
        if keys is not None:
            L = handle.L
            if eager:
                scr, hst = self._screen.ctypes.data, self._hist.ctypes.data
            else:
                self._screen = self._hist = None
                self._snap = _DevLease(handle.dev_pool, 2 * n * h * w)
                scr, hst = self._snap.ptr, self._snap.ptr + n * h * w
            rc = L.rg_step_fetch(handle.h, keys.ctypes.data, int(keys.shape[0]), C.c_void_p(scr), C.c_void_p(hst), self.status.ctypes.data, self.flags.ctypes.data)
            if rc and b"config groups" in L.rg_last_error(handle.h):
                handle.fast_step = False
                self._snap = None
                handle.step_keys_host(keys)
                keys = None
            else:
                handle.epoch += 1
                handle.check(rc)
                if self._snap is not None:
                    self._register_lazy()
        if keys is not None:
# ... 350 lines not shown
```

Measured before the change: 756.4 million env-steps/s.

## Fuse gray observation encoding into step kernel tail with residual obs pass

For the 32x16 mini-dungeon path, the step kernel now writes the gray observation for each env directly from the screen mirror at the end of its wave, using an LDS lookup table and nontemporal stores. It stamps each encoded env. A new residual kernel then encodes only envs that were not stamped: redraws, and waves that ran past a time cutoff measured with s_memrealtime. This is meant to avoid a separate full pass that rereads the screen and writes all observations, at the cost of longer step-kernel waves, extra register pressure, a per-env stamp write and a time-dependent split of the work.

```diff
diff --git a/include/rogue_gym_hip.h b/include/rogue_gym_hip.h
--- a/include/rogue_gym_hip.h
+++ b/include/rogue_gym_hip.h
@@ -55,6 +55,8 @@
 int rg_done(rg_t *h, uint8_t **dev);
 
 int rg_set_stair_reward(rg_t *h, float bonus);
+
+int rg_tail_encode(rg_t *h, int on);
 
 int rg_obs_gray(rg_t *h, uint32_t status_flag, int with_hist, float *out_dev);
 int rg_obs_symbol(rg_t *h, uint32_t status_flag, int with_hist, float *out_dev);
diff --git a/rogue-gym_amd/csrc/rg_api.cpp b/rogue-gym_amd/csrc/rg_api.cpp
--- a/rogue-gym_amd/csrc/rg_api.cpp
+++ b/rogue-gym_amd/csrc/rg_api.cpp
@@ -41,6 +41,9 @@
 void rgk_gather_keys(const uint8_t *keys, const int32_t *ext, uint8_t *dst, int n, hipStream_t st);
 int rgk_obs(const RgState *S, const RgConfig *c, uint32_t sflag, int with_hist, int kind, float *out, uint32_t *err_any, int planes_sym, int bound, hipStream_t st, hipEvent_t ev0, hipEvent_t ev1);
 int rgk_redraw(const RgState *S, const RgConfig *c, hipStream_t st);
+int rgk_obs_tail_capable(const RgState *S, const RgConfig *c);
+int rgk_step_tail_capable(const RgConfig *c);
+void rgk_obs_resid(const RgState *S, const RgConfig *c, float *out, hipStream_t st, hipEvent_t ev0, hipEvent_t ev1);
 int rgk_obs_typed(const RgState *S, const RgConfig *c, int kind, int dtype, uint32_t sflag, int with_hist, int planes_sym, void *out, uint32_t *err_any, hipStream_t st, hipEvent_t ev0,
                   hipEvent_t ev1);
 int rgk_obs_crop(const RgState *S, const RgConfig *c, int kind, int ry, int rx, uint32_t sflag, int with_hist, int planes_sym, float *out, int32_t *centers,
@@ -53,6 +56,7 @@
 void rgk_build_list(const RgState *S, const RgConfig *c, const int32_t *list, const uint32_t *cnt, uint8_t *mark, hipStream_t st);
 }
 
+#define RG_ENC_CUT_TICKS 4000u
 #define RG_TIMED_KERNELS 5
 struct rg_handle {
     RgParsed parsed;
@@ -80,6 +84,7 @@
     bool render_pending = false;
     float *bound_out = nullptr; int bound_kind = 0; bool bound_valid = false;
     int32_t *obs_list_mem = nullptr; uint32_t *obs_cnt_mem = nullptr; float *gray_lut_mem = nullptr;
+    bool tail_enc = false, tail_enc_off = false;
     int bound_steps = 0;
     int stair_gen = 0;
     float *obs_scratch = nullptr;
@@ -197,6 +202,7 @@
 static void destroy_handle(rg_handle *h);
 struct EnvSeed { bool has_seed, has_range; uint64_t lo, hi; unsigned __int128 r0, r1; };
 
+static int ensure_gray_lut(rg_handle *h);
 static int create_homog(const RgParsed &parsed, const EnvSeed *seeds, int n_env, uint64_t max_steps, int device, int auto_reset, rg_handle **out) {
     *out = nullptr;
     rg_handle *h = new rg_handle();
@@ -263,6 +269,14 @@
     if (ok && nr <= RG_OBS_MAX_ROOMS) ok = dev_alloc(h, &S.obs_rec, n * (size_t)RG_OBS_REC_WORDS(nr));
     if (ok && nr <= RG_OVL_MAX && getenv("ROGUE_GYM_HIP_NO_MIRROR_UPDATE") == nullptr)
         ok = dev_alloc(h, &S.ovl, (nr + 1) * n) && hipMemset(S.ovl, 0xff, (nr + 1) * n * 2) == hipSuccess;
+    {
+        if (ok && rgk_step_tail_capable(&h->cfg) && S.ovl && S.obs_rec) {
+            ok = dev_alloc(h, &S.enc_stamp, n) && ensure_gray_lut(h) == 0;
+            h->tail_enc = ok;
+            S.enc_cut = RG_ENC_CUT_TICKS;
+            if (const char *ev = RG_DEV_ENV("ROGUE_GYM_HIP_ENC_CUT")) S.enc_cut = (uint32_t)atoi(ev);
+        }
+    }
     h->spares = auto_reset != 0 && getenv("ROGUE_GYM_HIP_NO_SPARES") == nullptr;
     h->lane_regen = h->spares && getenv("ROGUE_GYM_HIP_WAVE_REGEN") == nullptr && rgk_regen_lanes_supported(&h->cfg, maze_cap) > 0;
     const char *slots_env = getenv("ROGUE_GYM_HIP_SP_SLOTS");
@@ -539,7 +553,24 @@
 static int obs_common(rg_t *h, uint32_t status_flag, int with_hist, int kind, float *out_dev);
 int rg_step(rg_t *h, const uint8_t *keys, int keys_on_device) { return rg_step_prefix(h, keys, h->S.n, keys_on_device); }
 int rg_step_obs_gray(rg_t *h, const uint8_t *keys, int keys_on_device, uint32_t status_flag, int with_hist, float *out_dev) {
-    return rg_step_prefix(h, keys, h->S.n, keys_on_device) ? 1 : obs_common(h, status_flag, with_hist, 0, out_dev);
+    const bool enc = h->tail_enc && !h->tail_enc_off && h->sub.empty() && (status_flag & 0x1ffu) == 0 && !with_hist && !h->bound_out && out_dev && rgk_obs_tail_capable(&h->S, &h->cfg);
+    if (enc) {
+        h->S.enc_out = out_dev;
+        h->S.enc_step = (uint32_t)(h->step_count % 0xffffffffull) + 1u;
+    }
+    const int rc = rg_step_prefix(h, keys, h->S.n, keys_on_device);
+    h->S.enc_out = nullptr;
+    if (rc) return 1;
+    if (!enc) return obs_common(h, status_flag, with_hist, 0, out_dev);
+    {
+        TimedLaunch t(h, 2, true);
+        rgk_obs_resid(&h->S, &h->cfg, out_dev, h->stream, t.start_ev(), t.stop_ev());
+    }
+    HIPCHK(h, hipGetLastError());
+    h->render_pending = false;
+    h->bound_valid = false;
+    h->bound_steps = 0;
+    return 0;
 }
 
 int rg_step_prefix(rg_t *h, const uint8_t *keys, int n_keys, int keys_on_device) {
@@ -645,6 +676,12 @@
     return 0;
 }
 
+int rg_tail_encode(rg_t *h, int on) {
+    h->tail_enc_off = on == 0;
+    for (rg_handle *sh : h->sub) sh->tail_enc_off = on == 0;
+    return 0;
+}
+
 int rg_obs_channels(const rg_t *h, int symbol, uint32_t status_flag, int with_hist) {
     return (symbol ? h->planes_sym : 1) + __builtin_popcount(status_flag & 0x1ffu) + (with_hist ? 1 : 0);
 }
@@ -693,6 +730,16 @@
     default: return (t >= 'A' && t <= 'Z') ? t - 'A' + 17 : 255u;
     }
 }
+static int ensure_gray_lut(rg_handle *h) {
+    if (!h->gray_lut_mem) {
+        float lut[128];
+        for (uint32_t g = 0; g < 128; g++) lut[g] = (float)(uint8_t)host_tile_to_sym(g) / (float)(uint8_t)h->cfg.symbols;
+        if (!dev_alloc(h, &h->gray_lut_mem, 128)) return 1;
+        HIPCHK(h, hipMemcpy(h->gray_lut_mem, lut, sizeof lut, hipMemcpyHostToDevice));
+    }
+    h->S.gray_lut = h->gray_lut_mem;
+    return 0;
+}
 int rg_obs_bind(rg_t *h, int kind, uint32_t status_flag, int with_hist, float *out_dev) {
     if (!h->sub.empty()) { h->err = "rg_obs_bind: not for a handle with config groups"; return 1; }
     if (out_dev && ((status_flag & 0x1ffu) || with_hist || (kind != 0 && kind != 1))) { h->err = "rg_obs_bind: gray or symbol image without status planes and history plane"; return 1; }
@@ -705,13 +752,7 @@
     if (out_dev) HIPCHK(h, hipMemsetAsync(h->obs_cnt_mem, 0, 8, h->stream));
     h->S.obs_list = out_dev ? h->obs_list_mem : nullptr; h->S.obs_cnt = out_dev ? h->obs_cnt_mem : nullptr;
     h->S.bound_gray = (out_dev && kind == 0) ? out_dev : nullptr;
-    if (h->S.bound_gray && !h->gray_lut_mem) {
-        float lut[128];
-        for (uint32_t g = 0; g < 128; g++) lut[g] = (float)(uint8_t)host_tile_to_sym(g) / (float)(uint8_t)h->cfg.symbols;
-        if (!dev_alloc(h, &h->gray_lut_mem, 128)) return 1;
-        HIPCHK(h, hipMemcpy(h->gray_lut_mem, lut, sizeof lut, hipMemcpyHostToDevice));
-    }
-    h->S.gray_lut = h->gray_lut_mem;
+    if (h->S.bound_gray && ensure_gray_lut(h)) return 1;
     h->bound_out = out_dev; h->bound_kind = kind; h->bound_valid = false; h->bound_steps = 0;
     return 0;
 }
diff --git a/rogue-gym_amd/csrc/rg_kernels.hip b/rogue-gym_amd/csrc/rg_kernels.hip
--- a/rogue-gym_amd/csrc/rg_kernels.hip
+++ b/rogue-gym_amd/csrc/rg_kernels.hip
@@ -2249,12 +2249,66 @@
     if (taken && !(S.keep_spares && S.reseed[e] == 0)) __hip_atomic_store(&S.sp_ready[es], 0u, __ATOMIC_RELAXED, __HIP_MEMORY_SCOPE_AGENT);
 }
 
-template <int BW, int GM, bool BND = false>
+#ifndef ENC_BATCH
+#define ENC_BATCH 8
+#endif
+__device__ __forceinline__ void tail_encode(const RgState &S, const int lane, const int e, const bool encl) {
+    typedef float f4v __attribute__((ext_vector_type(4)));
+    const uint64_t em = __ballot(encl);
+    if (encl) S.enc_stamp[e] = S.enc_step;
+    if (!em) return;
+    const int ebase = __builtin_amdgcn_readfirstlane(e - lane);
+    asm volatile("s_waitcnt vmcnt(0)" ::: "memory");
+    const __attribute__((address_space(3))) float *lut = (const __attribute__((address_space(3))) float *)(g_smem + STEP_LDS_LUT);
+    const uint32_t *mir = reinterpret_cast<const uint32_t *>(S.screen) + lane;
+    f4v *img = reinterpret_cast<f4v *>(S.enc_out) + lane;
+    uint64_t rem = em;
+    int last = 0;
+    struct Batch { int env[ENC_BATCH]; uint32_t w0[ENC_BATCH], w1[ENC_BATCH]; };
+    auto load = [&](Batch &b) {
+#pragma unroll
+        for (int k = 0; k < ENC_BATCH; k++) {
+            last = rem ? __builtin_ctzll(rem) : last;
+            rem &= rem - (rem ? 1ull : 0ull);
+            b.env[k] = ebase + last;
+            const uint32_t *m = mir + (size_t)b.env[k] * 128;
+            b.w0[k] = __hip_atomic_load(m, __ATOMIC_RELAXED, __HIP_MEMORY_SCOPE_AGENT);
+            b.w1[k] = __hip_atomic_load(m + WAVE, __ATOMIC_RELAXED, __HIP_MEMORY_SCOPE_AGENT);
+        }
+    };
+    auto gray4 = [&](uint32_t w) {
+        w &= 0x7f7f7f7fu;
+        f4v v = {lut[w & 0xff], lut[(w >> 8) & 0xff], lut[(w >> 16) & 0xff], lut[w >> 24]};
+        return v;
+    };
+    auto store = [&](const Batch &b) {
+#pragma unroll
+        for (int k = 0; k < ENC_BATCH; k++) {
+            f4v *o = img + (size_t)b.env[k] * 128;
+            __builtin_nontemporal_store(gray4(b.w0[k]), o);
+            __builtin_nontemporal_store(gray4(b.w1[k]), o + WAVE);
+        }
+    };
+    const int nb = (__popcll(em) + ENC_BATCH - 1) / ENC_BATCH;
+    Batch cur, nxt;
+    load(cur);
+    load(nxt);
+    store(cur);
+#pragma nounroll
+    for (int b = 1; b < nb; b++) {
+        cur = nxt;
+        load(nxt);
+        store(cur);
+    }
+}
+
+template <int BW, int GM, bool BND = false, bool ENC = false>
 __device__ __forceinline__ void step_wave(const RgState &S, const RgState *__restrict__ SPd, const RgConfig &c, const uint8_t *__restrict__ keys, int use_spares, int stage_off,
                                           const int e, const bool valid_in, const int stair_role) {
     uint16_t *lds_grid = reinterpret_cast<uint16_t *>(g_smem + stage_off);
     const int lane = threadIdx.x;
     Prof pf; pf.start(S.prof);
+    const unsigned long long enc_t0 = ENC ? __builtin_amdgcn_s_memrealtime() : 0ull;
     Env E;
     E.err = 0; E.on_stairs = 0;
     uint32_t react = 0, err = 0, old_flags = 0, steps = 0, flags = 0;
@@ -2312,7 +2366,7 @@
     w.v = (lds_u16 *)(g_smem + STEP_LDS_WIN) + lane;
     lds_u32 *ovl_l = (lds_u32 *)(g_smem + STEP_LDS_OVL) + lane;
     ovl_l[0] = 0;
-    if (BND && S.bound_gray) {
+    if ((BND && S.bound_gray) || ENC) {
         typedef const __attribute__((address_space(1))) void *gptr;
         typedef __attribute__((address_space(3))) void *lptr;
         __builtin_amdgcn_global_load_lds((gptr)(S.gray_lut + lane), (lptr)(g_smem + STEP_LDS_LUT), 4, 0, 0);
@@ -2491,6 +2545,7 @@
     asm volatile("" : "+v"(et));
     E.e = et;
     bool pend = false; uint64_t pm = 0; uint32_t lbase = 0;
+    bool encl = false;
     if (BND && S.obs_list) {
         const uint32_t fw = (live ? ((terminal && c.auto_reset) ? RG_FLAG_REDRAW : flags) : old_flags);
         pend = valid && (fw & (RG_FLAG_REDRAW | RG_FLAG_SCR_CHANGED));
@@ -2534,6 +2589,7 @@
         if (!taken) store_env(S, E);
         S.steps[et] = steps;
         S.flags[et] = flags;
+        if (ENC) encl = !(flags & RG_FLAG_REDRAW);
         S.done[et] = terminal ? 1 : 0;
         if (S.ovl && !taken && !inc_done && ((react & R_REDRAW) || descends || (terminal && c.auto_reset))) {
             for (int s0 = 0; s0 < nrooms_k; s0++) {
@@ -2586,12 +2642,17 @@
     take_spares(S, SPd, c, lane, et, taken, on_next);
     stair_publish(S, lane, et, valid, on_next);
     pf.mark(7);
+    if constexpr (ENC) {
+        const bool late = __builtin_amdgcn_s_memrealtime() - enc_t0 > (unsigned long long)S.enc_cut;
+        tail_encode(S, lane, et, encl && !late);
+        pf.mark(31);
+    }
     pf.finish();
 }
 
 #define STAIR_BLOCKS 256
 
-#define RG_STEP_BLOCK_BODY(BWV, GMV, BNDV) \
+#define RG_STEP_BLOCK_BODY(BWV, GMV, BNDV, ENCV) \
     __builtin_amdgcn_s_setprio(3); \
     const int lane = threadIdx.x; \
     if (blockIdx.x == 0 && lane == 0) { \
@@ -2608,7 +2669,7 @@
         bool v; int e; \
         if (stair) { e = list[i0]; v = lane == 0 && e < S.n_keys && keys[e] == '>'; } \
         else { v = lane < epw && i0 + lane < items; e = v ? i0 + lane : 0; } \
-        if (!stair || __any(v)) step_wave<BWV, GMV, BNDV>(S, SPd, c, keys, use_spares, stage_off, e, v, parity >= 0 ? (stair ? 1 : 2) : 0); \
+        if (!stair || __any(v)) step_wave<BWV, GMV, BNDV, ENCV>(S, SPd, c, keys, use_spares, stage_off, e, v, parity >= 0 ? (stair ? 1 : 2) : 0); \
         if (!stair || items <= STAIR_BLOCKS) break; \
         __syncthreads(); \
         uint32_t t = 0; \
@@ -2618,16 +2679,16 @@
 template <int BW, bool BND = false>
 __global__ void __launch_bounds__(WAVE) k_step(RgState S, const RgState *__restrict__ SPd, RgConfig c, const uint8_t *__restrict__ keys, int use_spares, int stage_off, int epw,
                                                int parity) {
-    RG_STEP_BLOCK_BODY(BW, (BW != 0 ? 1 : 0), BND)
-}
-template <bool BND>
+    RG_STEP_BLOCK_BODY(BW, (BW != 0 ? 1 : 0), BND, false)
+}
+template <bool BND, bool ENC = false>
 __global__ void __launch_bounds__(WAVE) __attribute__((amdgpu_waves_per_eu(2, 2)))
 k_step_w32(RgState S, const RgState *__restrict__ SPd, RgConfig c, const uint8_t *__restrict__ keys, int use_spares, int stage_off, int epw, int parity) {
-    RG_STEP_BLOCK_BODY(0, 0, BND)
+    RG_STEP_BLOCK_BODY(0, 0, BND, ENC)
 }
 __global__ void __launch_bounds__(WAVE) k_step_huge(RgState S, const RgState *__restrict__ SPd, RgConfig c, const uint8_t *__restrict__ keys, int use_spares, int stage_off,
                                                     int epw, int parity) {
-    RG_STEP_BLOCK_BODY(4, 2, false)
+    RG_STEP_BLOCK_BODY(4, 2, false, false)
 }
 #undef RG_STEP_BLOCK_BODY
 
@@ -2683,6 +2744,7 @@
     if (c->width <= 32 && gen_mode_of(c) == 0) return 1;
     return (c->width <= 96 && hw <= 4096 && c->width > 64) ? 1 : 0;
 }
+int rgk_step_tail_capable(const RgConfig *c) { return (c->width <= 32 && gen_mode_of(c) == 0 && c->width * c->height == 512) ? 1 : 0; }
 int rgk_step(const RgState *S, const RgState *SP_dev, const RgConfig *c, const uint8_t *keys, int use_spares, int parity, hipStream_t st, hipEvent_t ev0, hipEvent_t ev1) {
     const bool bnd = S->obs_list != nullptr && rgk_step_bound_capable(c);
     int hw = c->width * c->height;
@@ -2702,7 +2764,7 @@
             if (hipFuncSetAttribute(reinterpret_cast<const void *>(k_step_huge), hipFuncAttributeMaxDynamicSharedMemorySize, (int)smem) == hipSuccess && dev >= 0 && dev < 64) raised[dev] = smem;
         }
         RG_LAUNCH_STEP(k_step_huge);
-    } else if (c->width <= 32 && gen_mode_of(c) == 0) { if (bnd) RG_LAUNCH_STEP(k_step_w32<true>); else RG_LAUNCH_STEP(k_step_w32<false>); }
+    } else if (c->width <= 32 && gen_mode_of(c) == 0) { if (bnd) RG_LAUNCH_STEP(k_step_w32<true>); else if (S->enc_out) RG_LAUNCH_STEP((k_step_w32<false, true>)); else RG_LAUNCH_STEP(k_step_w32<false>); }
     else if (n32 && c->width <= 64) RG_LAUNCH_STEP(k_step<1>);
     else if (n32) { if (bnd) RG_LAUNCH_STEP((k_step<2, true>)); else RG_LAUNCH_STEP(k_step<2>); }
     else if (c->width <= 128) RG_LAUNCH_STEP(k_step<3>);
diff --git a/rogue-gym_amd/csrc/rg_obs.hip b/rogue-gym_amd/csrc/rg_obs.hip
--- a/rogue-gym_amd/csrc/rg_obs.hip
+++ b/rogue-gym_amd/csrc/rg_obs.hip
@@ -382,6 +382,43 @@
     }
 }
 
+#define RG_OBS_REDRAW_ENV() \
+    lds_barrier();                                                                                                             \
+    if (lane < rec_words) tb.w[lane] = t_rec;                                                                                                                            \
+                           \
+    const bool upd_hist = !(fle & RG_FLAG_HIST_STALE) && (fle & RG_FLAG_HIST_DIRTY);                                                                                     \
+    if (lane < Q8) {                                                                                                                                                     \
+        uint32_t g[2], hb[2];                                                                                                                                            \
+        draw_cells8(v, lane, W, HW, g, hb);                                                                                                                              \
+        reinterpret_cast<uint2 *>(scr)[lane] = make_uint2(g[0], g[1]);                                                                                                   \
+        if (upd_hist) reinterpret_cast<uint2 *>(S.hist + (size_t)e * HW)[lane] = make_uint2(hb[0], hb[1]);                                                               \
+    }                                                                                                                                                                    \
+    lds_barrier();                                                                                                                                                       \
+                                                                      \
+    const uint32_t ppos = tb.w[nrooms];                                                                                                                                  \
+    const int px = POS_X(ppos), py = POS_Y(ppos);                                                                                                                        \
+    if (lane < nrooms) {                                                                                                                                                 \
+        const uint32_t mw = tb.w[lane];                                                                                                                                  \
+        if ((mw >> 24) & MF_ALIVE) {                                                                                                                                     \
+            const int x = POS_X(mw), y = POS_Y(mw);                                                                                                                      \
+            const uint32_t under = scr[y * W + x];                                                                                                                       \
+            if (monster_shown(c, &tb, nrooms, px, py, x, y) && (under & 0x80u) && under != (0x80u | '*')) scr[y * W + x] = (uint8_t)(0x80u | mtile[(mw >> 16) & 0xff]);  \
+        }                                                                                                                                                                \
+    }                                                                                                                                                                    \
+    lds_barrier();                                                                                                                                                       \
+    if (lane == 0 && (scr[py * W + px] & 0x80u)) scr[py * W + px] = (uint8_t)(0x80u | '@');                                                                              \
+    lds_barrier();                                                                                                                                                       \
+    uint32_t *m4 = reinterpret_cast<uint32_t *>(S.screen + (size_t)e * HW);                                                                                              \
+    float4 *oe = reinterpret_cast<float4 *>(out) + (size_t)e * Q4;                                                                                                       \
+    for (int q = lane; q < Q4; q += WAVE) {                                                                                                                              \
+        const uint32_t g = reinterpret_cast<const uint32_t *>(scr)[q] & 0x7f7f7f7fu;                                                                                     \
+        m4[q] = g;                                                                                                                                                       \
+        store_obs(&oe[q], gray4(g));                                                                                                                                     \
+    }                                                                                                                                                                    \
+    if (lane == 0)                                                                    \
+        S.flags[e] = (fle & ~(RG_FLAG_REDRAW | RG_FLAG_HIST_STALE | RG_FLAG_HIST_LAG | ((fle & RG_FLAG_HIST_STALE) ? 0u : RG_FLAG_HIST_DIRTY))) |                        \
+                     ((fle & RG_FLAG_HIST_STALE) ? RG_FLAG_HIST_LAG : 0u);
+
 #ifndef OBS_RUN
 #define OBS_RUN 4
 #endif
@@ -450,41 +487,82 @@
             const uint4 v = tv;
             const uint32_t t_rec = trec;
             if (rmask) load_tiles(base + __builtin_ctzll(rmask), tv, trec);
-            lds_barrier();
-            if (lane < rec_words) tb.w[lane] = t_rec;
-            const bool upd_hist = !(fle & RG_FLAG_HIST_STALE) && (fle & RG_FLAG_HIST_DIRTY);
-            if (lane < Q8) {
-                uint32_t g[2], hb[2];
-                draw_cells8(v, lane, W, HW, g, hb);
-                reinterpret_cast<uint2 *>(scr)[lane] = make_uint2(g[0], g[1]);
-                if (upd_hist) reinterpret_cast<uint2 *>(S.hist + (size_t)e * HW)[lane] = make_uint2(hb[0], hb[1]);
-            }
-            lds_barrier();
-            const uint32_t ppos = tb.w[nrooms];
-            const int px = POS_X(ppos), py = POS_Y(ppos);
-            if (lane < nrooms) {
-                const uint32_t mw = tb.w[lane];
-                if ((mw >> 24) & MF_ALIVE) {
-                    const int x = POS_X(mw), y = POS_Y(mw);
-                    const uint32_t under = scr[y * W + x];
-                    if (monster_shown(c, &tb, nrooms, px, py, x, y) && (under & 0x80u) && under != (0x80u | '*')) scr[y * W + x] = (uint8_t)(0x80u | mtile[(mw >> 16) & 0xff]);
-                }
-            }
-            lds_barrier();
-            if (lane == 0 && (scr[py * W + px] & 0x80u)) scr[py * W + px] = (uint8_t)(0x80u | '@');
-            lds_barrier();
-            uint32_t *m4 = reinterpret_cast<uint32_t *>(S.screen + (size_t)e * HW);
-            float4 *oe = reinterpret_cast<float4 *>(out) + (size_t)e * Q4;
-            for (int q = lane; q < Q4; q += WAVE) {
-                const uint32_t g = reinterpret_cast<const uint32_t *>(scr)[q] & 0x7f7f7f7fu;
-                m4[q] = g;
-                store_obs(&oe[q], gray4(g));
-            }
-            if (lane == 0)
-                S.flags[e] = (fle & ~(RG_FLAG_REDRAW | RG_FLAG_HIST_STALE | RG_FLAG_HIST_LAG | ((fle & RG_FLAG_HIST_STALE) ? 0u : RG_FLAG_HIST_DIRTY))) |
-                             ((fle & RG_FLAG_HIST_STALE) ? RG_FLAG_HIST_LAG : 0u);
+            RG_OBS_REDRAW_ENV();
         }
         cur = nxt;
+    }
+}
+
+#ifndef OBS_RESID_RUN
+#define OBS_RESID_RUN 4
+#endif
+#ifndef OBS_RESID_WAVES
+#define OBS_RESID_WAVES 16384
+#endif
+__global__ void __launch_bounds__(WAVE) k_obs_resid(RgState S, RgConfig c, float *__restrict__ out) {
+    __shared__ float lutf[128];
+    __shared__ uint8_t mtile[RG_MAX_ENEMY_KINDS + 6];
+    __shared__ __align__(16) uint8_t scr[512];
+    __shared__ ObsTabs tb;
+    const int lane = threadIdx.x, W = c.width, HW = W * c.height, Q4 = HW >> 2, Q8 = HW >> 3, n = S.n;
+    const int nrooms = c.room_num_x * c.room_num_y, rec_words = RG_OBS_REC_WORDS(nrooms);
+    const int nruns = (n + OBS_RESID_RUN - 1) / OBS_RESID_RUN;
+    auto load_run = [&](int r, uint32_t &fl, uint32_t &stamp) {
+        const int base = r * OBS_RESID_RUN;
+        const bool in = r < nruns && lane < OBS_RESID_RUN && base + lane < n;
+        fl = in ? S.flags[base + lane] : 0u;
+        stamp = in ? S.enc_stamp[base + lane] : S.enc_step;
+    };
+    uint32_t fl_cur, st_cur;
+    load_run(blockIdx.x, fl_cur, st_cur);
+    lutf[lane] = S.gray_lut[lane];
+    lutf[lane + WAVE] = S.gray_lut[lane + WAVE];
+    for (int g = lane; g < RG_MAX_ENEMY_KINDS + 6; g += WAVE) mtile[g] = c.mon[g].tile;
+    lds_barrier();
+    auto gray4 = [&](uint32_t w) {
+        w &= 0x7f7f7f7fu;
+        float4 v; v.x = lutf[w & 0xff]; v.y = lutf[(w >> 8) & 0xff]; v.z = lutf[(w >> 16) & 0xff]; v.w = lutf[w >> 24];
+        return v;
+    };
+    auto load_tiles = [&](int e, uint4 &v, uint32_t &rec) {
+        v = lane < Q8 ? reinterpret_cast<const uint4 *>(S.cell + (size_t)e * HW)[lane] : make_uint4(0, 0, 0, 0);
+        rec = lane < rec_words ? S.obs_rec[(size_t)e * rec_words + lane] : 0u;
+    };
+    for (int r = blockIdx.x; r < nruns; r += gridDim.x) {
+        const int base = r * OBS_RESID_RUN;
+        const uint32_t fl = fl_cur;
+        const bool need = st_cur != S.enc_step;
+        load_run(r + gridDim.x, fl_cur, st_cur);
+        uint64_t rmask = __ballot(need && (fl & RG_FLAG_REDRAW));
+        const uint64_t smask = __ballot(need && !(fl & RG_FLAG_REDRAW));
+        if (!(rmask | smask)) continue;
+        uint4 tv = make_uint4(0, 0, 0, 0);
+        uint32_t trec = 0;
+        if (rmask) load_tiles(base + __builtin_ctzll(rmask), tv, trec);
+        const uint32_t *m = reinterpret_cast<const uint32_t *>(S.screen) + (size_t)base * Q4;
+        float4 *o = reinterpret_cast<float4 *>(out) + (size_t)base * Q4;
+        uint32_t w0[OBS_RESID_RUN], w1[OBS_RESID_RUN];
+#pragma unroll
+        for (int i = 0; i < OBS_RESID_RUN; i++) {
+            w0[i] = w1[i] = 0u;
+            if ((smask >> i) & 1) { w0[i] = m[i * Q4 + lane]; w1[i] = m[i * Q4 + lane + WAVE]; }
+        }
+#pragma unroll
+        for (int i = 0; i < OBS_RESID_RUN; i++) {
+            if (!((smask >> i) & 1)) continue;
+            store_obs(&o[i * Q4 + lane], gray4(w0[i]));
+            store_obs(&o[i * Q4 + lane + WAVE], gray4(w1[i]));
+        }
+        while (rmask) {
+            const int i = __builtin_ctzll(rmask);
+            rmask &= rmask - 1;
+            const int e = base + i;
+            const uint32_t fle = __builtin_amdgcn_readlane(fl, i);
+            const uint4 v = tv;
+            const uint32_t t_rec = trec;
+            if (rmask) load_tiles(base + __builtin_ctzll(rmask), tv, trec);
+            RG_OBS_REDRAW_ENV();
+        }
     }
 }
 
@@ -948,6 +1026,21 @@
 #undef RG_LAUNCH_OBS
     return 1;
 }
+int rgk_obs_tail_capable(const RgState *S, const RgConfig *c) {
+    const int hw = c->width * c->height, nr = c->room_num_x * c->room_num_y;
+    if (hw != 512 || nr > RG_OBS_MAX_ROOMS || !S->obs_rec || !S->ovl || S->ext) return 0;
+    if (RG_OBS_REC_WORDS(nr) > WAVE) return 0;
+#ifdef RG_DEV_KNOBS
+    if (const char *ev = getenv("RG_OBS_STREAM")) if (atoi(ev) == 0) return 0;
+#endif
+    return 1;
+}
+void rgk_obs_resid(const RgState *S, const RgConfig *c, float *out, hipStream_t st, hipEvent_t ev0, hipEvent_t ev1) {
+    int blocks = (S->n + OBS_RESID_RUN - 1) / OBS_RESID_RUN;
+    if (blocks > OBS_RESID_WAVES) blocks = OBS_RESID_WAVES;
+    if (ev0 || ev1) hipExtLaunchKernelGGL(k_obs_resid, dim3(blocks), dim3(WAVE), 0, st, ev0, ev1, 0, *S, *c, out);
+    else hipLaunchKernelGGL(k_obs_resid, dim3(blocks), dim3(WAVE), 0, st, *S, *c, out);
+}
 void rgk_encode(const uint8_t *screen, const uint8_t *hist, const int32_t *status, uint32_t *flags, uint32_t *err_any, int n, int hw, size_t rs, size_t rst,
                 int symbols, int planes_sym, uint32_t sflag, int with_hist, int kind, float *out, const int32_t *ext, hipStream_t st) {
     if ((hw & 3) == 0 && (rs & 3) == 0) {
diff --git a/rogue-gym_amd/csrc/rg_state.h b/rogue-gym_amd/csrc/rg_state.h
--- a/rogue-gym_amd/csrc/rg_state.h
+++ b/rogue-gym_amd/csrc/rg_state.h
@@ -93,6 +93,10 @@
     uint16_t *ovl;
     float *bound_gray;
     const float *gray_lut;
+    float *enc_out;
+    uint32_t *enc_stamp;
+    uint32_t enc_step;
+    uint32_t enc_cut;
     int32_t *obs_list;
     uint32_t *obs_cnt;
     int32_t obs_par;
diff --git a/rogue-gym_amd/rogue_gym_python/_rogue_gym.py b/rogue-gym_amd/rogue_gym_python/_rogue_gym.py
--- a/rogue-gym_amd/rogue_gym_python/_rogue_gym.py
+++ b/rogue-gym_amd/rogue_gym_python/_rogue_gym.py
@@ -38,7 +38,7 @@
     "rg_host_alloc", "rg_dev_alloc", "rg_snapshot_take", "rg_dev_read", "rg_dev_read_rows", "rg_compact_record_bytes", "rg_pack_compact", "rg_expand_compact", "rg_comm_unique_id", "rg_comm_init", "rg_comm_destroy", "rg_comm_count", "rg_allgather_compact", "rg_status_vec", "rg_history_enable", "rg_history_keys",
     "rg_dump_history", "rg_counters", "rg_counters_ex", "rg_probe_sclk", "rg_dump_config", "rg_config_canonical", "rg_config_resolved", "rg_config_schema", "rg_debug_fetch", "rg_debug_descend", "rg_timing_enable", "rg_timing_read", "rg_timing_read_all", "rg_timing_read_samples",
     "rg_state_record_bytes", "rg_state_save", "rg_state_load", "rg_obs_crop", "rg_obs_dtype_bytes", "rg_obs_typed", "rg_step_obs_typed",
-    "rg_reset_envs", "rg_reset_mask", "rg_seed_envs",
+    "rg_reset_envs", "rg_reset_mask", "rg_seed_envs", "rg_tail_encode",
 )
 
 
@@ -96,9 +96,10 @@
         "rg_obs_crop": [vp, i32, i32, i32, u32, i32, vp, vp],
         "rg_obs_dtype_bytes": [i32], "rg_obs_typed": [vp, i32, i32, u32, i32, vp], "rg_step_obs_typed": [vp, vp, i32, i32, i32, u32, i32, vp],
         "rg_reset_envs": [vp, vp, i32, i32], "rg_reset_mask": [vp, vp], "rg_seed_envs": [vp, vp, C.POINTER(C.c_uint64), C.POINTER(C.c_uint64), i32],
+        "rg_tail_encode": [vp, i32],
     }
     optional = {"rg_timing_read_samples", "rg_obs_bind", "rg_state_record_bytes", "rg_state_save", "rg_state_load", "rg_obs_crop", "rg_obs_dtype_bytes", "rg_obs_typed",
-                "rg_step_obs_typed", "rg_reset_envs", "rg_reset_mask", "rg_seed_envs"} if os.environ.get("ROGUE_GYM_HIP_LIB") else set()
+                "rg_step_obs_typed", "rg_reset_envs", "rg_reset_mask", "rg_seed_envs", "rg_tail_encode"} if os.environ.get("ROGUE_GYM_HIP_LIB") else set()
     for name, argtypes in sig.items():
         if name in optional and not hasattr(L, name):
             continue
@@ -243,6 +244,8 @@
                 raise RuntimeError(msg)
             raise RuntimeError("Error in rogue-gym: " + msg)
         self.h = h
+        if os.environ.get("ROGUE_GYM_HIP_NO_TAIL_ENCODE", "0") not in ("", "0") and hasattr(L, "rg_tail_encode"):
+            L.rg_tail_encode(h, 0)
         hh, ww, ss, nn = C.c_int(), C.c_int(), C.c_int(), C.c_int()
         L.rg_dims(h, C.byref(hh), C.byref(ww), C.byref(ss), C.byref(nn))
         self.height, self.width, self.symbols, self.n = hh.value, ww.value, ss.value, nn.value
```

After: 831.0 million env-steps/s (median of 6 runs). +9.9%, better.
